# cassiusfive/balatro-gym

Hardware: AMD Instinct MI355X
Metric: env-steps/sec at 65536 envs, random policy; achieved HBM GB/s vs peak (higher is better)
Workload: dtype int64/f64

## Files before the change

### balatro_gym_amd/csrc/bg_device.h

```cpp
#pragma once
#include <hip/hip_runtime.h>
#include <stdint.h>
#include "bg_tables.h"

#define BG_NHOT 8
#define BG_NDECK 4
#define BG_NCOLD 7
#define BG_NTMPL 2
#define BG_MT_N 624
#define BG_MT_M 397
#define BG_MTS 640
#define BG_BLOCK 64

#define BG_DEVERR_GSTREAM 1u
#define BG_DEVERR_SHOPBLK 2u
#define BG_DEVERR_DECKRING 4u
#define BG_DEVERR_SHOPRING 8u

typedef __attribute__((address_space(1))) unsigned long long g_u64;
typedef __attribute__((address_space(1))) uint32_t g_u32;
__device__ __forceinline__ unsigned long long bg_ld8a(const void* p) { return __hip_atomic_load((g_u64*)p, __ATOMIC_RELAXED, __HIP_MEMORY_SCOPE_AGENT); }
__device__ __forceinline__ uint32_t bg_ld4a(const void* p) { return __hip_atomic_load((g_u32*)p, __ATOMIC_RELAXED, __HIP_MEMORY_SCOPE_AGENT); }
__device__ __forceinline__ void bg_st8a(void* p, unsigned long long v) { __hip_atomic_store((g_u64*)p, v, __ATOMIC_RELAXED, __HIP_MEMORY_SCOPE_AGENT); }
__device__ __forceinline__ uint4 bg_ld16a(const void* p) {
  const unsigned long long a = bg_ld8a(p), b = bg_ld8a((const char*)p + 8);
  return make_uint4((uint32_t)a, (uint32_t)(a >> 32), (uint32_t)b, (uint32_t)(b >> 32));
}

struct BgDev {
  int N;
  uint32_t flags;
  int max_ante;
  int KG, KS, KD;
  uint4* hot;
  uint4* deck;
  uint4* cold;
  uint4* tmpl;
  uint4* ndeck;
  uint32_t* gblk;
  uint32_t* sblk;
  uint32_t* sovf;
  uint32_t* deckmt;
  uint32_t* shopgenmt;
  uint32_t* err;
  uint32_t* wl_count;
  uint32_t* wl;
  uint32_t* wl_shop;
  uint32_t* sseed;
  uint32_t* smeta;
  const uint32_t* prod_view;
  const uint32_t* prod_in;
  uint32_t* prod_out;
  unsigned long long* dbg;
  uint4* cstate;
  uint4* ctmpl;
  uint32_t* cardmt;
  uint32_t* sealmt;
  const uint32_t* jtab;
};

struct Env {
  int64_t chips_scored, round_chips;
  int64_t best_hand;
  int32_t chips_needed, money;
  int32_t hp_total, hp_ante, jokers_sold, shop_reroll_state, shop_reroll_base;
  int32_t ante, round, phase, hands_left, discards_left, hand_size, nhand, nsel, njokers, ncons, n_magic, n_minim,
      boss_type, boss_req, bflags, shop_n;
  uint64_t hand, sel;
  uint32_t highlighted, face_down, boss_hp, boss_types, cons0, cons1;
  uint64_t jokers;
  int32_t shop_ante, d_head, d_cons, d_ready;
  uint64_t boss_cards;
  uint64_t levels;
  int32_t g_cur, g_cons, g_valid;
  int32_t g_idx, s_idx, s_cur, s_cons, s_ready;
  int32_t ndrop, nfo;
  uint64_t excess;
  int32_t max_ante;
};

#define BG_BF_FIRST_HAND 1
#define BG_BF_SHOP_EXISTS 2

__device__ __forceinline__ uint32_t bg_b(uint32_t w, int i) { return (w >> (8 * i)) & 0xffu; }

__device__ __forceinline__ void bg_unpack(const uint4 c[BG_NHOT], Env& e) {
  e.chips_scored = (int64_t)(((uint64_t)c[0].y << 32) | c[0].x);
  e.round_chips = (int64_t)(((uint64_t)c[0].w << 32) | c[0].z);
  e.best_hand = (int64_t)(((uint64_t)c[1].y << 32) | c[1].x);
  e.chips_needed = (int32_t)c[1].z;
  e.money = (int32_t)c[1].w;
  e.hp_total = (int32_t)c[2].x;
  e.hp_ante = (int32_t)(c[2].y & 0xffffu);
  e.jokers_sold = (int32_t)(c[2].y >> 16);
  e.shop_reroll_state = (int32_t)c[2].z;
  e.shop_reroll_base = (int32_t)c[2].w;
  e.ante = bg_b(c[3].x, 0); e.round = bg_b(c[3].x, 1); e.phase = bg_b(c[3].x, 2); e.hands_left = bg_b(c[3].x, 3);
  e.discards_left = bg_b(c[3].y, 0); e.hand_size = (int)(int8_t)bg_b(c[3].y, 1);  e.nhand = bg_b(c[3].y, 2); e.nsel = bg_b(c[3].y, 3);
  e.njokers = bg_b(c[3].z, 0); e.ncons = bg_b(c[3].z, 1); e.n_magic = bg_b(c[3].z, 2); e.n_minim = bg_b(c[3].z, 3);
  e.boss_type = bg_b(c[3].w, 0); e.boss_req = bg_b(c[3].w, 1); e.bflags = bg_b(c[3].w, 2); e.shop_n = bg_b(c[3].w, 3);
  e.hand = ((uint64_t)c[4].y << 32) | c[4].x;
  e.sel = ((uint64_t)c[4].w << 32) | c[4].z;
  e.highlighted = c[5].x & 0xffffu; e.face_down = bg_b(c[5].x, 2); e.boss_hp = bg_b(c[5].x, 3);
  e.boss_types = c[5].y & 0xffffu; e.cons0 = bg_b(c[5].y, 2); e.cons1 = bg_b(c[5].y, 3);
  e.jokers = (uint64_t)c[5].z | ((uint64_t)(c[5].w & 0xffu) << 32);
  e.shop_ante = bg_b(c[5].w, 1); e.d_head = bg_b(c[5].w, 2); e.d_cons = bg_b(c[5].w, 3); e.d_ready = 0;
  e.boss_cards = ((uint64_t)c[6].y << 32) | c[6].x;
  e.levels = (uint64_t)c[6].z | ((uint64_t)(c[6].w & 0xffffu) << 32);
  e.g_cur = bg_b(c[6].w, 2); e.g_cons = bg_b(c[6].w, 3); e.g_valid = 0;
  e.g_idx = (int32_t)(c[7].x & 0xffffu); e.s_idx = (int32_t)(c[7].x >> 16);
  e.s_cur = bg_b(c[7].y, 0); e.s_cons = bg_b(c[7].y, 1); e.s_ready = 0; e.ndrop = bg_b(c[7].y, 2); e.nfo = bg_b(c[7].y, 3);
  e.excess = (uint64_t)c[7].z | ((uint64_t)(c[7].w & 0xffffu) << 32);
  e.max_ante = (int32_t)(c[7].w >> 16) & 0xff;
}

__device__ __forceinline__ uint32_t bg_p4(int a, int b, int c, int d) {
  return (uint32_t)(a & 0xff) | ((uint32_t)(b & 0xff) << 8) | ((uint32_t)(c & 0xff) << 16) | ((uint32_t)(d & 0xff) << 24);
}

__device__ __forceinline__ void bg_pack(const Env& e, uint4 c[BG_NHOT]) {
  c[0] = make_uint4((uint32_t)e.chips_scored, (uint32_t)((uint64_t)e.chips_scored >> 32), (uint32_t)e.round_chips,
                    (uint32_t)((uint64_t)e.round_chips >> 32));
  c[1] = make_uint4((uint32_t)e.best_hand, (uint32_t)((uint64_t)e.best_hand >> 32), (uint32_t)e.chips_needed, (uint32_t)e.money);
  c[2] = make_uint4((uint32_t)e.hp_total, ((uint32_t)e.hp_ante & 0xffffu) | ((uint32_t)e.jokers_sold << 16),
                    (uint32_t)e.shop_reroll_state, (uint32_t)e.shop_reroll_base);
  c[3] = make_uint4(bg_p4(e.ante, e.round, e.phase, e.hands_left), bg_p4(e.discards_left, e.hand_size, e.nhand, e.nsel),
                    bg_p4(e.njokers, e.ncons, e.n_magic, e.n_minim), bg_p4(e.boss_type, e.boss_req, e.bflags, e.shop_n));
  c[4] = make_uint4((uint32_t)e.hand, (uint32_t)(e.hand >> 32), (uint32_t)e.sel, (uint32_t)(e.sel >> 32));
  c[5] = make_uint4((e.highlighted & 0xffffu) | ((e.face_down & 0xffu) << 16) | ((e.boss_hp & 0xffu) << 24),
                    (e.boss_types & 0xffffu) | ((e.cons0 & 0xffu) << 16) | ((e.cons1 & 0xffu) << 24), (uint32_t)e.jokers,
                    bg_p4((int)(e.jokers >> 32), e.shop_ante, e.d_head, e.d_cons));
  c[6] = make_uint4((uint32_t)e.boss_cards, (uint32_t)(e.boss_cards >> 32), (uint32_t)e.levels,
                    ((uint32_t)(e.levels >> 32) & 0xffffu) | ((uint32_t)(e.g_cur & 0xff) << 16) | ((uint32_t)(e.g_cons & 0xff) << 24));
  c[7] = make_uint4(((uint32_t)e.g_idx & 0xffffu) | ((uint32_t)e.s_idx << 16), bg_p4(e.s_cur, e.s_cons, e.ndrop, e.nfo),
                    (uint32_t)e.excess, ((uint32_t)(e.excess >> 32) & 0xffffu) | ((uint32_t)(e.max_ante & 0xff) << 16));
}

__device__ __forceinline__ void bg_derive_ready(Env& e, uint32_t prod) {
  e.d_ready = (int)((prod - (uint32_t)e.d_cons) & 0xffu);
  e.s_ready = (int)(((prod >> 8) - (uint32_t)e.s_cons) & 0xffu);
  e.g_valid = (int)(((prod >> 16) - (uint32_t)e.g_cons) & 0xffu);
}
__device__ __forceinline__ void bg_load_env(const BgDev& d, int env, Env& e) {
  uint4 c[BG_NHOT];
#pragma unroll
  for (int k = 0; k < BG_NHOT; k++) c[k] = d.hot[(size_t)k * d.N + env];
  bg_unpack(c, e);
  bg_derive_ready(e, d.prod_view ? d.prod_view[env] : 0u);
}
__device__ __forceinline__ void bg_store_env(const BgDev& d, int env, const Env& e) {
  uint4 c[BG_NHOT];
  bg_pack(e, c);
#pragma unroll
  for (int k = 0; k < BG_NHOT; k++) d.hot[(size_t)k * d.N + env] = c[k];
}

__device__ __forceinline__ int bg_get8(uint64_t v, int i) { return (int)((v >> (8 * i)) & 0xffull); }
__device__ __forceinline__ uint64_t bg_set8(uint64_t v, int i, int x) {
  return (v & ~(0xffull << (8 * i))) | ((uint64_t)(x & 0xff) << (8 * i));
}
__device__ __forceinline__ uint64_t bg_del8(uint64_t v, int i) {
  uint64_t lowmask = i ? ((1ull << (8 * i)) - 1) : 0ull;
  uint64_t lo = v & lowmask;
  uint64_t hi = (i < 7) ? (v >> (8 * (i + 1))) << (8 * i) : 0ull;
  return lo | hi;
}
__device__ __forceinline__ int bg_level(const Env& e, int ht) { return (int)((e.levels >> (4 * ht)) & 0xf); }

__device__ __forceinline__ uint32_t* bg_gblock(const BgDev& d, int env, int slot) { return d.gblk + ((size_t)env * d.KG + slot) * BG_MTS; }
#define BG_SW_T 56
#define BG_SW_PK 56
#define BG_SW_SEED 62
#define BG_SLOT_WORDS 64
#define BG_S_FASTMAX (BG_SW_T - 1)
static_assert(BG_SW_T >= 28 && BG_SW_PK == BG_SW_T && BG_SW_PK % 4 == 0 && BG_SW_PK + 6 == BG_SW_SEED && BG_SW_SEED + 2 == BG_SLOT_WORDS, "shop slot");
#define BG_BF_SHOP_OVF 4
__device__ __forceinline__ uint32_t* bg_sblock(const BgDev& d, int env, int slot) { return d.sblk + ((size_t)env * d.KS + slot) * BG_SLOT_WORDS; }
__device__ __forceinline__ uint32_t* bg_sovf(const BgDev& d, int env) { return d.sovf + (size_t)env * BG_MTS; }
__device__ __forceinline__ void bg_mt_seed_rolled(uint32_t* p, uint32_t key) {
  uint32_t g = 19650218u, a = g;
#pragma unroll 1
  for (uint32_t i = 1; i < 624u; i++) {
    g = 1812433253u * (g ^ (g >> 30)) + i;
    a = (g ^ ((a ^ (a >> 30)) * 1664525u)) + key;
    p[i] = a;
  }
  __builtin_amdgcn_fence(__ATOMIC_RELEASE, "agent");
  __builtin_amdgcn_fence(__ATOMIC_ACQUIRE, "agent");
  const uint32_t m1 = (p[1] ^ ((a ^ (a >> 30)) * 1664525u)) + key;
  uint32_t b = m1;
#pragma unroll 1
  for (uint32_t i = 2; i < 624u; i++) {
    b = (p[i] ^ ((b ^ (b >> 30)) * 1566083941u)) - i;
    p[i] = b;
  }
  p[1] = (m1 ^ ((b ^ (b >> 30)) * 1566083941u)) - 1u;
  p[0] = 0x80000000u;
}
__device__ __forceinline__ uint32_t* bg_deckmt(const BgDev& d, int env) { return d.deckmt + (size_t)env * BG_MTS; }
__device__ __forceinline__ uint32_t* bg_shopgenmt(const BgDev& d, int env) { return d.shopgenmt + (size_t)env * BG_MTS; }

#ifdef BG_TIMING
__shared__ unsigned long long bg_probe_lds[32];
#define BG_PROBE_BEGIN() unsigned long long _pt = __builtin_readcyclecounter()
#define BG_PROBE(k) do { unsigned long long _n = __builtin_readcyclecounter(); \
    if ((int)threadIdx.x == __ffsll((long long)__ballot(1)) - 1 + (int)(threadIdx.x & ~63u)) atomicAdd(&bg_probe_lds[k], _n - _pt); \
    _pt = __builtin_readcyclecounter(); } while (0)
#define BG_PROBE_INIT() do { if (threadIdx.x < 32) bg_probe_lds[threadIdx.x] = 0; __syncthreads(); } while (0)
#define BG_PROBE_FLUSH(d) do { __syncthreads(); if (threadIdx.x < 32 && (d).dbg && bg_probe_lds[threadIdx.x]) atomicAdd(&(d).dbg[threadIdx.x], bg_probe_lds[threadIdx.x]); } while (0)
#else
#define BG_PROBE_BEGIN() do {} while (0)
#define BG_PROBE(k) do {} while (0)
#define BG_PROBE_INIT() do {} while (0)
#define BG_PROBE_FLUSH(d) do {} while (0)
#endif

#define BG_RB 128
typedef __attribute__((address_space(3))) uint8_t lds_u8;
typedef __attribute__((address_space(3))) uint32_t lds_u32;
struct Deck0 { uint64_t lo, hi; static constexpr bool kCards = false; };
struct DeckLds { lds_u32* col; static constexpr bool kCards = false; };
struct Deck0C : Deck0 { static constexpr bool kCards = true; };
struct DeckLdsC : DeckLds { static constexpr bool kCards = true; };
#define BG_NCST 7
__device__ __forceinline__ uint32_t bg_cstate(const BgDev& d, int env, int ci) {
  return (uint32_t)((const uint16_t*)&d.cstate[(size_t)(ci >> 3) * d.N + env])[ci & 7];
}
__device__ __forceinline__ Deck0 bg_load_deck0(const BgDev& d, int env) {
  uint4 c = d.deck[env];
  Deck0 r;
  r.lo = ((uint64_t)c.y << 32) | c.x;
  r.hi = ((uint64_t)c.w << 32) | c.z;
  return r;
}
__device__ __forceinline__ void bg_deck_set(Deck0& dk, int k, uint4 c) {
  if (k == 0) { dk.lo = ((uint64_t)c.y << 32) | c.x; dk.hi = ((uint64_t)c.w << 32) | c.z; }
}
__device__ __forceinline__ void bg_deck_set(DeckLds& dk, int k, uint4 c) {
  dk.col[(4 * k) * BG_RB] = c.x; dk.col[(4 * k + 1) * BG_RB] = c.y; dk.col[(4 * k + 2) * BG_RB] = c.z; dk.col[(4 * k + 3) * BG_RB] = c.w;
}
__device__ __forceinline__ int bg_card(const BgDev& d, int env, const Deck0& k, int idx) {
  if (idx < 16) return (int)(((idx < 8 ? k.lo : k.hi) >> (8 * (idx & 7))) & 0xffull);
  const uint32_t* p = (const uint32_t*)&d.deck[(size_t)(idx >> 4) * d.N + env];
  return (int)((bg_ld4a(p + ((idx & 15) >> 2)) >> (8 * (idx & 3))) & 0xffu);
}
template <int S, bool C> struct DeckLdsS { lds_u32* col; static constexpr bool kCards = C; };
template <int S, bool C>
__device__ __forceinline__ void bg_deck_set(DeckLdsS<S, C>& dk, int k, uint4 c) {
  dk.col[(4 * k) * S] = c.x; dk.col[(4 * k + 1) * S] = c.y; dk.col[(4 * k + 2) * S] = c.z; dk.col[(4 * k + 3) * S] = c.w;
}
template <int S, bool C>
__device__ __forceinline__ int bg_card(const BgDev& d, int env, const DeckLdsS<S, C>& k, int idx) {
  return (int)((const lds_u8*)k.col)[(idx >> 2) * (S * 4) + (idx & 3)];
}
__device__ __forceinline__ int bg_card(const BgDev& d, int env, const DeckLds& k, int idx) {
  return (int)((const lds_u8*)k.col)[(idx >> 2) * (BG_RB * 4) + (idx & 3)];
}

struct DeckHead { uint64_t lo, hi; };
__device__ __forceinline__ DeckHead bg_deck_head(const BgDev& d, int env, const Deck0& k) { return DeckHead{k.lo, k.hi}; }
template <int S, bool C>
__device__ __forceinline__ DeckHead bg_deck_head(const BgDev& d, int env, const DeckLdsS<S, C>& k) {
  const uint32_t a = k.col[0], b = k.col[S], c = k.col[2 * S], e = k.col[3 * S];
  return DeckHead{((uint64_t)b << 32) | a, ((uint64_t)e << 32) | c};
}
template <class DK>
__device__ __forceinline__ int bg_card_h(const BgDev& d, int env, const DK& k, const DeckHead& h, int idx) {
  if (idx < 16) return (int)(((idx < 8 ? h.lo : h.hi) >> (8 * (idx & 7))) & 0xffull);
  return bg_card(d, env, k, idx);
}

__device__ __forceinline__ uint32_t bg_temper(uint32_t y) {
  y ^= (y >> 11);
  y ^= (y << 7) & 0x9d2c5680u;
  y ^= (y << 15) & 0xefc60000u;
  y ^= (y >> 18);
  return y;
}
__device__ __forceinline__ uint32_t bg_twist(uint32_t a, uint32_t b, uint32_t far) {
  uint32_t y = (a & 0x80000000u) | (b & 0x7fffffffu);
  return far ^ (y >> 1) ^ ((y & 1u) ? 0x9908b0dfu : 0u);
}

__device__ __forceinline__ uint32_t bg_lazy_next(uint32_t* S) {
  uint32_t c = S[BG_MT_N] & 0x3ffu;
  const uint32_t c1 = c + 1 == BG_MT_N ? 0u : c + 1, cf = c + BG_MT_M >= BG_MT_N ? c + BG_MT_M - BG_MT_N : c + BG_MT_M;
  const uint32_t y = bg_twist(S[c], S[c1], S[cf]);
  S[c] = y;
  S[BG_MT_N] = c1 | 0x80000000u;
  return bg_temper(y);
}
__device__ __forceinline__ double bg_lazy_random(uint32_t* S) {
  const uint32_t a = bg_lazy_next(S) >> 5, b = bg_lazy_next(S) >> 6;
  return ((double)a * 67108864.0 + (double)b) * (1.0 / 9007199254740992.0);
}

#define BG_WIN 16
struct JTables {
  uint64_t jd[152];
  uint32_t jm[152];
  uint64_t jr[152];
  uint8_t jf[152];
  uint8_t cost[152];
  double pow115[101];
  double pow15[16];
  double pow08[16];
  uint32_t inv[64];
};
typedef __attribute__((address_space(3))) const JTables lds_JTables;
struct RngWin {
  lds_JTables* jt;
  lds_u32* lds;
  int g_blk, g_start, g_len;
  int s_start, s_len;
  bool defer_adv;
  bool need_inv;
};
__device__ __forceinline__ void bg_win_init(RngWin& w, uint32_t* lds_lane, const JTables* jt = nullptr) {
  w.jt = (lds_JTables*)jt; w.lds = (lds_u32*)lds_lane; w.g_blk = -1; w.g_start = 0; w.g_len = 0; w.s_start = 0; w.s_len = 0; w.defer_adv = false; w.need_inv = false;
}
__device__ __noinline__ void bg_win_fill(lds_u32* lds, const uint32_t* src, int len) {
#pragma unroll 1
  for (int base = 0; base < len; base += BG_WIN) {
    uint32_t v[BG_WIN];
#pragma unroll
    for (int j = 0; j < BG_WIN; j++) v[j] = (base + j < len) ? src[base + j] : 0u;
// ... 257 lines not shown
```

### balatro_gym_amd/csrc/bg_engine.h

```cpp
#pragma once

#define BG_Q_RUN 0
#define BG_Q_PLAY 1
#define BG_Q_OTHER 2
#define BG_ITEM_VALID 0x80000000u
#define BG_SPIN_LIMIT (1u << 24)
#define BG_DEVERR_SPIN 16u
#define BG_ENG_LNE 8
static_assert(BG_ENG_LNE == 8, "only 256 envs per workgroup are supported: items carry the env lane in 8 bits, copy-queue generations in 7, and the epilogue assumes NE = 256");
#define BG_ENG_NE (1 << BG_ENG_LNE)
#define BG_ENG_NW 7
#define BG_ENG_OCC 2
#define BG_ENG_IMG_PIECES 22
#define BG_ENG_NSV 4
#define BG_ENG_SMASK_DEFAULT (((1u << BG_ENG_NSV) - 1u) << (BG_ENG_NW - BG_ENG_NSV))

struct EngineArgs {
  int T;
  int policy;
  uint64_t policy_seed, env_index0, t0;
  ObsPtrs obs;
  int obs_stride_steps;
  double* reward; uint8_t* term; uint8_t* trunc; int32_t* actions_out;
  const int32_t* actions_in;
// ... 9 lines not shown
  uint32_t epw;
  uint8_t* const* gpeer;
  uint32_t gworld, grank;
};

__device__ __forceinline__ uint32_t bg_lds_ld(uint32_t* p) {
  uint32_t v = __hip_atomic_load(p, __ATOMIC_RELAXED, __HIP_MEMORY_SCOPE_WORKGROUP);
  asm volatile("" ::: "memory");
  return v;
}
__device__ __forceinline__ void bg_lds_st(uint32_t* p, uint32_t v) {
  asm volatile("" ::: "memory");
  __hip_atomic_store(p, v, __ATOMIC_RELAXED, __HIP_MEMORY_SCOPE_WORKGROUP);
}
__device__ __forceinline__ uint32_t bg_lds_ld(uint16_t* p) {
  uint16_t v = __hip_atomic_load(p, __ATOMIC_RELAXED, __HIP_MEMORY_SCOPE_WORKGROUP);
  asm volatile("" ::: "memory");
  return (uint32_t)v;
}
__device__ __forceinline__ void bg_lds_st(uint16_t* p, uint32_t v) {
  asm volatile("" ::: "memory");
  __hip_atomic_store(p, (uint16_t)v, __ATOMIC_RELAXED, __HIP_MEMORY_SCOPE_WORKGROUP);
}
__device__ __forceinline__ void bg_vm_drain() { asm volatile("s_waitcnt vmcnt(0)" ::: "memory"); }
#ifdef BG_ENG_TL
constexpr bool kEngTl = true;
#else
constexpr bool kEngTl = false;
#endif
#define BG_TL(k) do { if constexpr (kEngTl) __hip_atomic_fetch_add(&s_tl[k], wall_clock64() - tl_k0, __ATOMIC_RELAXED, __HIP_MEMORY_SCOPE_WORKGROUP); } while (0)


template <bool HASH, bool CARDS, bool INFO>
__global__ __launch_bounds__(BG_ENG_NW * BG_BLOCK, BG_ENG_OCC) void bg_engine_kernel(BgDev d, EngineArgs a) {
  constexpr int NE = BG_ENG_NE, NW = BG_ENG_NW, NSV = BG_ENG_NSV;
  __shared__ bg_u32x4 s_img[NE][BG_ENG_IMG_PIECES];
  __shared__ uint4 s_c34[2][NE];
  __shared__ uint32_t s_deck[16][NE];
  __shared__ unsigned long long s_mask[NE];
  __shared__ uint32_t s_t[NE], s_prod[NE];
  __shared__ uint32_t s_q[3][NE];
  __shared__ __attribute__((aligned(16))) uint32_t s_ctl[8];
  uint32_t* const s_tail = &s_ctl[0];
  uint32_t* const s_head = &s_ctl[4];
#define s_done s_ctl[3]
#define s_busy s_ctl[7]
  __shared__ uint32_t s_win[NSV][BG_WIN][BG_BLOCK];
  __shared__ uint2 s_cq[NE];
  __shared__ uint32_t s_cqt;
  __shared__ bg_u32x4 s_zero;
  __shared__ unsigned long long s_stats[6];
  __shared__ JTables jt;
  __shared__ unsigned long long s_tl[kEngTl ? 32 : 1];
  const unsigned long long tl_k0 = kEngTl ? wall_clock64() : 0ull;
  if constexpr (kEngTl) { if (threadIdx.x < 32) s_tl[threadIdx.x] = 0ull; __syncthreads(); }
  __builtin_amdgcn_s_setprio(3);
  BG_PROBE_INIT();
  const int tid = threadIdx.x, wave = tid >> 6, lane = tid & 63;
  const int env0 = blockIdx.x * NE;
  const int n_live = d.N - env0 < NE ? d.N - env0 : NE;
  const bool can_serve = ((a.serve_mask >> wave) & 1u) != 0;
  const int serve_idx = __popc(a.serve_mask & ((1u << wave) - 1u));
  using DeckT = DeckLdsS<NE, CARDS>;
  const size_t N = (size_t)d.N;
  const bool keys_at_end = !a.obs.rows && a.obs_stride_steps == 0;
  if (tid < 3) { s_tail[tid] = 0u; s_head[tid] = 0; }
  if (tid == 0) { s_done = 0; s_busy = 0; s_cqt = 0; s_zero = bg_u32x4{0u, 0u, 0u, 0u}; }
  if (tid < 6) s_stats[tid] = 0ull;
  const bool mine = tid < NE && tid < n_live;
  const int l0 = tid, envp = env0 + tid;
  if (tid < NE) { s_q[BG_Q_RUN][l0] = 0; s_q[BG_Q_PLAY][l0] = 0; s_q[BG_Q_OTHER][l0] = 0; s_cq[l0] = make_uint2(0u, 0u); s_t[l0] = 0; }
  constexpr int JW = (int)(sizeof(JTables) / 4), JPT = (JW + NW * BG_BLOCK - 1) / (NW * BG_BLOCK);
  uint32_t jv[JPT];
#pragma unroll
  for (int k = 0; k < JPT; k++) { const int i = tid + k * NW * BG_BLOCK; jv[k] = i < JW ? d.jtab[i] : 0u; }
  bool svc = false;
  {
    uint4 c[BG_NHOT];
    uint4 dw[BG_NDECK];
    uint32_t prod = 0u;
    int act0 = 0;
    if (mine) {
#pragma unroll
      for (int k = 0; k < BG_NHOT; k++) c[k] = d.hot[(size_t)k * N + envp];
#pragma unroll
      for (int k = 0; k < BG_NDECK; k++) dw[k] = d.deck[(size_t)k * N + envp];
      prod = d.prod_view ? d.prod_view[envp] : 0u;
      if (a.actions_in) act0 = a.actions_in[envp];
    }
    __syncthreads();
    if (tid == 0) BG_TL(1);
#pragma unroll
    for (int k = 0; k < JPT; k++) { const int i = tid + k * NW * BG_BLOCK; if (i < JW) ((uint32_t*)&jt)[i] = jv[k]; }
    if (mine) {
      s_c34[0][l0] = c[3]; s_c34[1][l0] = c[4];
      DeckT dk; dk.col = (lds_u32*)&s_deck[0][l0];
#pragma unroll
      for (int k = 0; k < BG_NDECK; k++) bg_deck_set(dk, k, dw[k]);
      s_prod[l0] = prod;
      Env pe;
      ShopRegs psr; psr.valid = false;
      bg_unpack(c, pe);
      bg_derive_ready(pe, prod);
      const uint64_t pmask = bg_action_mask(d, envp, pe, psr);
      s_mask[l0] = pmask;
      if (a.actions_in) {
        const bool valid = act0 >= 0 && act0 < 60 && ((pmask >> (act0 & 63)) & 1ull);
        const bool terminal = pe.ante > 100 || pe.chips_scored > 1000000000ll;
        const bool cheap = !terminal && (!valid || (pe.phase == 0 && act0 >= 2 && act0 < 10) || (pe.phase == 1 && act0 == 31 && pe.hand_size <= pe.nhand));
        svc = !cheap;
        if (svc) {
          const int q = (!terminal && pe.phase == 0 && act0 == 0) ? BG_Q_PLAY : BG_Q_OTHER;
          const uint32_t slot = __hip_atomic_fetch_add(&s_tail[q], 1u, __ATOMIC_RELAXED, __HIP_MEMORY_SCOPE_WORKGROUP);
          bg_lds_st(&s_q[q][slot & (NE - 1)], (uint32_t)l0 | (((slot >> BG_ENG_LNE) & 0xffu) << 8) | (((uint32_t)act0 & 0x7fffu) << 16) | BG_ITEM_VALID);
        }
      }
    }
  }
  if (tid == 0) BG_TL(2);
  __syncthreads();
  if (tid == 0) BG_TL(3);
  {
    if (mine && !svc) {
      __builtin_amdgcn_s_setprio(1);
      uint4 c[BG_NHOT];
#pragma unroll
      for (int k = 0; k < BG_NHOT; k++) if (k != 3 && k != 4) c[k] = d.hot[(size_t)k * N + envp];
      c[3] = s_c34[0][l0]; c[4] = s_c34[1][l0];
      Env pe;
      ShopRegs psr; psr.valid = false;
      bg_unpack(c, pe);
      bg_derive_ready(pe, s_prod[l0]);
      const uint64_t pmask = s_mask[l0];
      DeckT dk; dk.col = (lds_u32*)&s_deck[0][l0];
      const ObsPtrs none{};
      bg_write_obs_impl<false, 3>(d, envp, 0, pe, dk, none, pmask, psr, RowExtra{0.0, 0, 0u}, RowStage{(lds_u4*)&s_img[l0][0], nullptr});
      const uint32_t slot = __hip_atomic_fetch_add(&s_tail[BG_Q_RUN], 1u, __ATOMIC_RELAXED, __HIP_MEMORY_SCOPE_WORKGROUP);
      bg_lds_st(&s_q[BG_Q_RUN][slot & (NE - 1)], (uint32_t)l0 | (((slot >> BG_ENG_LNE) & 0xffu) << 8) | BG_ITEM_VALID);
    }
  }
  if (tid == 0) BG_TL(4);
  if (wave >= (int)(a.n_waves + a.copier)) return;
  if (a.copier && wave >= (int)a.n_waves) {
    __builtin_amdgcn_s_setprio(2);
    const uint32_t cid = (uint32_t)wave - a.n_waves, two = a.copier > 1u ? 1u : 0u;
    uint32_t head = two ? 32u * cid : 0u, cpolls = 0;
    const bool whole = a.obs.row_stride == 384u;
    const uint32_t PR = 22u, rcp = 2979u;
    for (;;) {
      const uint32_t tail = __builtin_amdgcn_readfirstlane(bg_lds_ld(&s_cqt));
      uint32_t navail = (int32_t)(tail - head) > 0 ? tail - head : 0u;
      if (two) { const uint32_t left = 32u - (head & 31u); navail = navail > left ? left : navail; }
      if (navail == 0u) {
        if (__builtin_amdgcn_readfirstlane(bg_lds_ld(&s_done)) >= (uint32_t)n_live) break;
        __builtin_amdgcn_s_sleep(2);
        if (++cpolls > BG_SPIN_LIMIT) { if (lane == 0) atomicOr(d.err, BG_DEVERR_SPIN); break; }
        continue;
      }
      cpolls = 0;
      const uint32_t nb = navail > BG_BLOCK ? BG_BLOCK : navail;
      uint2 ent = make_uint2(0u, 0u);
      if ((uint32_t)lane < nb) {
        const uint32_t pos = head + (uint32_t)lane, want = BG_ITEM_VALID | (((pos >> BG_ENG_LNE) & 0x7fu) << 16);
        lds_u32* ep = (lds_u32*)&s_cq[pos & (NE - 1)];
        uint32_t spin = 0, y = ep[1];
        while ((y & (BG_ITEM_VALID | 0x7f0000u)) != want && ++spin < BG_SPIN_LIMIT) { __builtin_amdgcn_s_sleep(1); asm volatile("" ::: "memory"); y = ep[1]; }
        asm volatile("" ::: "memory");
        if ((y & (BG_ITEM_VALID | 0x7f0000u)) != want) atomicOr(d.err, BG_DEVERR_SPIN);
        else ent = make_uint2(ep[0], y);
      }
      BG_WAVE_SYNC();
      typedef __attribute__((address_space(3))) const char lds_cc;
      typedef uint32_t bg_u32x2 __attribute__((ext_vector_type(2)));
      if (whole) {
        uint32_t rsel[3], mul[3], ib[3], gl[3];
        lds_cc* const imgb = (lds_cc*)&s_img[0][0];
        lds_cc* const cqb = (lds_cc*)&s_cq[0];
#pragma unroll
        for (int j = 0; j < 3; j++) {
          const uint32_t pidx = (uint32_t)j * BG_BLOCK + (uint32_t)lane, rs = (pidx * 2731u) >> 16, c = pidx - 24u * rs;
          rsel[j] = rs; gl[j] = 16u * c;
          mul[j] = c < 22u ? 16u * BG_ENG_IMG_PIECES : 0u;
          ib[j] = c < 22u ? 16u * c : (uint32_t)((lds_cc*)&s_zero - imgb);
        }
        for (uint32_t g0 = 0; g0 < nb; g0 += 32u) {
          bg_u32x2 ce[4][3];
          bg_u32x4 v[4][3];
#pragma unroll
          for (int u = 0; u < 4; u++)
#pragma unroll
            for (int j = 0; j < 3; j++)
              ce[u][j] = *(__attribute__((address_space(3))) const bg_u32x2*)(cqb + (((head + g0 + 8u * (uint32_t)u + rsel[j]) & (NE - 1)) << 3));
#pragma unroll
          for (int u = 0; u < 4; u++)
#pragma unroll
            for (int j = 0; j < 3; j++)
              v[u][j] = *(__attribute__((address_space(3))) const bg_u32x4*)(imgb + __umul24(ce[u][j].y & 0xffu, mul[j]) + ib[j]);
#pragma unroll
          for (int u = 0; u < 4; u++)
#pragma unroll
            for (int j = 0; j < 3; j++)
              if (g0 + 8u * (uint32_t)u + rsel[j] < nb)
                __builtin_nontemporal_store(v[u][j], (__attribute__((address_space(1))) bg_u32x4*)(a.obs.rows + ((size_t)ce[u][j].x * 384u + gl[j])));
        }
      } else {
      const uint32_t total = PR * nb;
#define BG_COPIER_KU 12
      constexpr int KU = BG_COPIER_KU;
      for (uint32_t q0 = (uint32_t)lane; q0 < total; q0 += (uint32_t)KU * BG_BLOCK) {
        uint2 ce[KU];
// ... 135 lines not shown
          const uint32_t play = te.nsel > 0 ? 1u : 0u, disc = (te.nsel > 0 && discards_left > 0u) ? 1u : 0u;
          mask = (mask & ~3ull) | play | ((uint64_t)disc << 1);
          s_mask[l] = mask;
          *(__attribute__((address_space(3))) uint16_t*)&img8[BG_ROW_ACTION_MASK] = (uint16_t)(play | (disc << 8));
        }
        fin = true;
      } else if (!terminal && valid && phase == 1u && action == 31 && (int)(int8_t)bg_b(c3.y, 1) <= (int)bg_b(c3.y, 2)) {
        const uint32_t nhand = bg_b(c3.y, 2), ncons = bg_b(c3.z, 1);
        ((lds_u8*)&s_c34[0][l])[2] = 0;
        uint64_t m = (((1ull << (nhand < 8u ? nhand : 8u)) - 1ull) << 2) | (((1ull << ncons) - 1ull) << 10);
        if (nsel0 > 0u) m |= 1ull | (discards_left > 0u ? 2ull : 0ull);
        mask = m;
        s_mask[l] = mask;
#pragma unroll
        for (int wq = 0; wq < 15; wq++) img32[44 + wq] = __umul24((uint32_t)(mask >> (4 * wq)) & 0xfu, 0x204081u) & 0x01010101u;
#pragma unroll
        for (int wq = 64; wq < 74; wq++) img32[wq] = 0u;
        img8[BG_ROW_PHASE] = 0;
        fin = true;
      } else if (!terminal && !valid) { reward = -1.0; fin = true; }
      else {
        const int q = (!terminal && phase == 0u && action == 0) ? BG_Q_PLAY : BG_Q_OTHER;
        const uint32_t slot = __hip_atomic_fetch_add(&s_tail[q], 1u, __ATOMIC_RELAXED, __HIP_MEMORY_SCOPE_WORKGROUP);
        bg_lds_st(&s_q[q][slot & (NE - 1)], (uint32_t)l | (((slot >> BG_ENG_LNE) & 0xffu) << 8) | (((uint32_t)action & 0x7fffu) << 16) | BG_ITEM_VALID);
        active = false;
      }
      if (fin) {
        *(__attribute__((address_space(3))) double*)&img32[34] = reward;
        img32[43] = (uint32_t)action;
        img8[BG_ROW_TERMINATED] = 0;
        if constexpr (INFO) { bg_step_init(o); o.reward = reward; o.error = valid ? 0 : 1; }
      }
      return fin;
    };
    auto finish = [&](bool cheap, size_t row, int action, double reward, bool terminated, const StepOut& o) __attribute__((always_inline)) {
      if (!a.obs.rows && !keys_at_end) bg_emit_keys_from_image((const lds_u4*)&s_img[l][0], a.obs, row);
      if (a.reward) a.reward[row] = reward;
      if (a.term) a.term[row] = terminated ? 1 : 0;
      if (a.actions_out) a.actions_out[row] = action;
      if constexpr (INFO) bg_emit_info(row, o, a.trunc, a.info);
      if (HASH) ohash ^= bg_hash_image((const lds_u4*)&s_img[l][0]) * (0x9E3779B97F4A7C15ull + 2 * (uint64_t)(a.t0 + t)) + (a.env_index0 + (uint64_t)env);
      n_steps++;
      rbits ^= (uint64_t)__double_as_longlong(reward) * (2 * (uint64_t)(a.t0 + t) + 1);
      t++;
      s_t[l] = t;
    };
    auto copy_out = [&](bool fin, size_t row) __attribute__((always_inline)) {
    if (a.copier) {
      const unsigned long long fm = __ballot(fin);
      if (fm) {
        uint32_t base = 0;
        if (lane == (int)(__ffsll((long long)fm) - 1)) base = __hip_atomic_fetch_add(&s_cqt, (uint32_t)__popcll(fm), __ATOMIC_RELAXED, __HIP_MEMORY_SCOPE_WORKGROUP);
        base = __builtin_amdgcn_readlane(base, __ffsll((long long)fm) - 1);
        if (fin) {
          const uint32_t pos = base + __builtin_amdgcn_mbcnt_hi((uint32_t)(fm >> 32), __builtin_amdgcn_mbcnt_lo((uint32_t)fm, 0u));
          lds_u32* ep = (lds_u32*)&s_cq[pos & (NE - 1)];
          ep[0] = (uint32_t)row;
          asm volatile("" ::: "memory");
          ep[1] = (uint32_t)l | (t >= (uint32_t)a.T ? 0x100u : 0u) | (((pos >> BG_ENG_LNE) & 0x7fu) << 16) | BG_ITEM_VALID;
          asm volatile("" ::: "memory");
          active = false;
        }
      }
      return;
    }
      if (active && t >= (uint32_t)a.T) { __hip_atomic_fetch_add(&s_done, 1u, __ATOMIC_RELAXED, __HIP_MEMORY_SCOPE_WORKGROUP); active = false; }
    };
    {
      bool fin = false;
      size_t row = 0;
      if (active) {
        row = (size_t)env + (a.obs_stride_steps ? (size_t)t * N : 0);
        int action = 0;
        double reward = 0.0;
        bool terminated = false;
        StepOut o;
        if (cls == BG_Q_RUN) fin = cheap_step(action, reward, o);
        else {
          uint64_t mask = s_mask[l];
        action = a.actions_in ? a.actions_in[(size_t)t * N + env] : (int)((item >> 16) & 0x7fffu);
        BG_PROBE_BEGIN();
        uint4 c[BG_NHOT];
#pragma unroll
        for (int k = 0; k < BG_NHOT; k++) if (k != 3 && k != 4) c[k] = d.hot[(size_t)k * N + env];
        c[3] = s_c34[0][l]; c[4] = s_c34[1][l];
        Env e;
        bg_unpack(c, e);
        BG_PROBE(23);
        bg_derive_ready(e, s_prod[l]);
        DeckT dk; dk.col = (lds_u32*)&s_deck[0][l];
        ShopRegs sr; sr.valid = false;
        RngWin w;
        bg_win_init(w, &s_win[serve_idx][0][lane], &jt);
        bg_step_init(o);
        if constexpr (INFO) if (a.info.score_breakdown) o.bd_dst = a.info.score_breakdown + row * 8;
        if (bg_step_guards(e, mask, action, o)) bg_env_dispatch(d, env, e, w, sr, dk, action, o);
        BG_PROBE(cls == BG_Q_PLAY ? 20 : 21);
        if (e.max_ante > 0 && e.ante > e.max_ante) { o.terminated = true; o.flags |= 256; }
        if (o.terminated) n_eps++;
        if (o.terminated && a.autoreset) { bg_env_reset(d, env, e, dk); if (INFO) o.flags |= BG_INFO_AUTORESET; }
        if constexpr (CARDS) bg_vm_drain();
        BG_PROBE(24);
        mask = bg_action_mask(d, env, e, sr);
        BG_PROBE(25);
        {
          const ObsPtrs none{};
          bg_write_obs_impl<false, 3>(d, env, row, e, dk, none, mask, sr, RowExtra{o.reward, action, o.terminated ? 1u : 0u}, RowStage{(lds_u4*)&s_img[l][0], nullptr});
        }
        BG_PROBE(26);
        bg_pack(e, c);
#pragma unroll
        for (int k = 0; k < BG_NHOT; k++) if (k != 3 && k != 4) d.hot[(size_t)k * N + env] = c[k];
        s_c34[0][l] = c[3]; s_c34[1][l] = c[4];
        s_mask[l] = mask;
        BG_PROBE(27);
        reward = o.reward; terminated = o.terminated;
        if (o.hand_type >= 0) { n_plays++; ssum += o.final_score; }
        fin = true;
        }
        if (fin) finish(cls == BG_Q_RUN, row, action, reward, terminated, o);
      }
      copy_out(fin, row);
    }
    for (uint32_t sub = 0; cls == BG_Q_RUN && !a.copier && sub < a.th_more && __ballot(active) != 0ull; sub++) {
      bool fin = false;
      size_t row = 0;
      if (active) {
        row = (size_t)env + (a.obs_stride_steps ? (size_t)t * N : 0);
        int action = 0;
        double reward = 0.0;
        StepOut o;
        fin = cheap_step(action, reward, o);
        if (fin) finish(true, row, action, reward, false, o);
      }
      copy_out(fin, row);
    }
    if (active) {
      const uint32_t slot = __hip_atomic_fetch_add(&s_tail[BG_Q_RUN], 1u, __ATOMIC_RELAXED, __HIP_MEMORY_SCOPE_WORKGROUP);
      bg_lds_st(&s_q[BG_Q_RUN][slot & (NE - 1)], (uint32_t)l | (((slot >> BG_ENG_LNE) & 0xffu) << 8) | BG_ITEM_VALID);
    }
    if (lane == 0) __hip_atomic_fetch_sub(&s_busy, 1u, __ATOMIC_RELAXED, __HIP_MEMORY_SCOPE_WORKGROUP);
    if constexpr (kEngTl) if (lane == 0) {
      const int b = cls == BG_Q_RUN ? 5 : (cls == BG_Q_PLAY ? 16 : 20);
      __hip_atomic_fetch_add(&s_tl[b], tl_b0 - tl_k0, __ATOMIC_RELAXED, __HIP_MEMORY_SCOPE_WORKGROUP);
      __hip_atomic_fetch_add(&s_tl[b + 1], 1ull, __ATOMIC_RELAXED, __HIP_MEMORY_SCOPE_WORKGROUP);
      __hip_atomic_fetch_add(&s_tl[b + 2], wall_clock64() - tl_b0, __ATOMIC_RELAXED, __HIP_MEMORY_SCOPE_WORKGROUP);
      __hip_atomic_fetch_add(&s_tl[b + 3], (unsigned long long)nb, __ATOMIC_RELAXED, __HIP_MEMORY_SCOPE_WORKGROUP);
    }
  }
  if (lane == 0 && wave == 0) BG_TL(9);
  if (lane == 0 && wave == (int)a.n_waves - 1) BG_TL(10);
  BG_PROBE_FLUSH(d);
  __syncthreads();
  if (tid == 0) BG_TL(12);
  if (tid < n_live) {
    d.hot[(size_t)3 * N + env0 + tid] = s_c34[0][tid];
    d.hot[(size_t)4 * N + env0 + tid] = s_c34[1][tid];
    if (keys_at_end) bg_emit_keys_from_image((const lds_u4*)&s_img[tid][0], a.obs, (size_t)(env0 + tid));
  }
  if (a.stats) {
    bg_stats_wave(s_stats, n_steps, n_eps, n_plays, ssum, rbits, ohash);
    __syncthreads();
    bg_stats_flush(a.stats, s_stats, tid);
  }
  if constexpr (kEngTl) if (d.dbg) {
    if (tid == 0) { BG_TL(13); s_tl[0] = 1ull; }
    __syncthreads();
    if (tid < 32 && tid != 14 && tid != 15 && s_tl[tid]) atomicAdd(&d.dbg[tid], s_tl[tid]);
    if (tid == 14) atomicMax(&d.dbg[14], ~tl_k0);
    if (tid == 15) atomicMax(&d.dbg[15], wall_clock64());
  }
}
```

### balatro_gym_amd/csrc/bg_engine3.h

```cpp
#pragma once

#ifdef BG_E3_TIMING
#define E3T_DECL() unsigned long long e3t_[8] = {0,0,0,0,0,0,0,0}, e3t0_ = __builtin_readcyclecounter()
#define E3T(k) do { const unsigned long long n_ = __builtin_readcyclecounter(); e3t_[k] += n_ - e3t0_; e3t0_ = n_; } while (0)
#define E3T_CNT(k, v) do { e3t_[k] += (v); } while (0)
#define E3T_FLUSH(base) do { if (lane == 0 && d.dbg) for (int k_ = 0; k_ < 8; k_++) atomicAdd(&d.dbg[(base) + k_], e3t_[k_]); } while (0)
constexpr bool kE3Timing = true, kE3Tl = true;
#else
#define E3T_DECL() const unsigned long long e3t_[8] = {0,0,0,0,0,0,0,0}; (void)e3t_
#define E3T(k) do {} while (0)
#define E3T_CNT(k, v) do {} while (0)
#define E3T_FLUSH(base) do {} while (0)
constexpr bool kE3Timing = false;
#ifdef BG_E3_TL
constexpr bool kE3Tl = true;
#else
constexpr bool kE3Tl = false;
#endif
#endif

#define BG_E3_REC_STORE(v, p) __builtin_nontemporal_store(v, p)
#define BG_E3_SPARSE 8u
#define BG_E3_SPARSE2 16u
#define BG_E3_ACTB 8
template <int NOW, int KS, int NSV>
struct E3Lds {
  static constexpr int NE = NOW * KS * BG_BLOCK;
  bg_u32x4 s_img[NE][22];
  uint4 s_c34[2][NE];
  unsigned long long s_mask[NE];
  uint32_t s_prod[NE];
  uint16_t s_ans[NE];
  uint32_t s_q[2][NE];
  __attribute__((aligned(16))) uint32_t s_ctl[8];
  uint32_t s_win[NSV][BG_WIN][BG_BLOCK];
  uint2 s_list[NOW][KS * BG_BLOCK];
  uint4 s_nd[BG_NDECK][NE];
  uint32_t s_ndst[NE];
  bg_u32x4 s_zero;
  unsigned long long s_stats[6];
  uint32_t s_owners_left;
  JTables jt;
};
template <bool HASH, bool CARDS, int NOW, int KS, int NSV, bool ACT = false>
__global__ __launch_bounds__((NOW + NSV) * BG_BLOCK, 2) void bg_engine3_kernel(BgDev d, EngineArgs a) {
  constexpr int NE = NOW * KS * BG_BLOCK, LNE = NE == 256 ? 8 : (NE == 128 ? 7 : 6);
  static_assert(NE == 64 || NE == 128 || NE == 256, "envs per workgroup (a request carries the env's lane in 8 bits)");
  __shared__ E3Lds<NOW, KS, NSV> L;
  auto& s_img = L.s_img; auto& s_c34 = L.s_c34; auto& s_mask = L.s_mask; auto& s_prod = L.s_prod; auto& s_ans = L.s_ans; auto& s_q = L.s_q;
  auto& s_ctl = L.s_ctl; auto& s_win = L.s_win; auto& s_list = L.s_list; auto& s_zero = L.s_zero; auto& s_owners_left = L.s_owners_left; auto& jt = L.jt;
  auto& s_nd = L.s_nd; auto& s_ndst = L.s_ndst;
  __shared__ int s_actb[ACT ? BG_E3_ACTB : 1][ACT ? NE : 1];
  __builtin_amdgcn_s_setprio(2);
  const unsigned long long e3_k0 = kE3Tl ? wall_clock64() : 0ull;
  BG_PROBE_INIT();
  bg_tables_load(&jt, d.jtab);
  const int tid = threadIdx.x, lane = tid & 63;
  const int wave = tid >> 6;
  const int epw = (NE == 64 && a.epw >= 1u && a.epw < 64u) ? (int)a.epw : NE;
  const int env0 = blockIdx.x * epw;
  const int n_live = d.N - env0 < epw ? d.N - env0 : epw;
  using DeckT = typename std::conditional<CARDS, Deck0C, Deck0>::type;
  const size_t N = (size_t)d.N;
  typedef __attribute__((address_space(3))) const char lds_cc;
  if (tid < 8) s_ctl[tid] = 0;
  if (tid == 0) { s_zero = bg_u32x4{0u, 0u, 0u, 0u}; s_owners_left = NOW; }
  if (tid < 6) L.s_stats[tid] = 0ull;
  for (int l = tid; l < NE; l += (NOW + NSV) * BG_BLOCK) {
    const int env = env0 + l;
    s_q[0][l] = 0; s_q[1][l] = 0; s_ans[l] = 0; s_ndst[l] = 0;
    if (l < n_live) {
      uint4 c[BG_NHOT];
#pragma unroll
      for (int k = 0; k < BG_NHOT; k++) c[k] = d.hot[(size_t)k * N + env];
      s_c34[0][l] = c[3]; s_c34[1][l] = c[4];
      DeckT dk; static_cast<Deck0&>(dk) = bg_load_deck0(d, env);
      const uint32_t prod = d.prod_view ? d.prod_view[env] : 0u;
      s_prod[l] = prod;
      Env e;
      bg_unpack(c, e);
      bg_derive_ready(e, prod);
      s_ndst[l] = e.d_ready > 0 ? 1u : 0u;
      if (e.d_ready > 0) {
#pragma unroll
        for (int k = 0; k < BG_NDECK; k++) s_nd[k][l] = d.ndeck[((size_t)e.d_head * BG_NDECK + k) * N + env];
      }
      ShopRegs sr; sr.valid = false;
      const uint64_t mask = bg_action_mask(d, env, e, sr);
      s_mask[l] = mask;
      const ObsPtrs none{};
      bg_write_obs_impl<false, 3>(d, env, 0, e, dk, none, mask, sr, RowExtra{0.0, 0, 0u}, RowStage{(lds_u4*)&s_img[l][0], nullptr});
    }
  }
  __syncthreads();
  if constexpr (kE3Timing) if (lane == 0) { uint32_t hw; asm volatile("s_getreg_b32 %0, hwreg(HW_REG_HW_ID)" : "=s"(hw)); atomicOr(&s_ctl[2], ((hw >> 4) & 3u) << (2 * wave)); }
  const unsigned long long e3_w0 = kE3Tl ? wall_clock64() : 0ull;
  if constexpr (kE3Tl) {
    if (tid == 0 && d.dbg) atomicAdd(&d.dbg[28], e3_w0 - e3_k0);
    __syncthreads();
  }
  const uint32_t T = (uint32_t)a.T;
  if (wave < NOW) {
    const uint32_t bmod3 = (uint32_t)(a.env_index0 % 3ull);
    lds_cc* const imgb = (lds_cc*)&s_img[0][0];
    const bool whole = a.obs.row_stride == 384u;
    uint32_t rsel[3], cmul[3], cib[3], cgl[3];
#pragma unroll
    for (int j = 0; j < 3; j++) {
      const uint32_t pidx = (uint32_t)j * BG_BLOCK + (uint32_t)lane, rs = (pidx * 2731u) >> 16, c = pidx - 24u * rs;
      rsel[j] = rs; cgl[j] = 16u * c;
      cmul[j] = c < 22u ? 16u * 22u : 0u;
      cib[j] = c < 22u ? 16u * c : (uint32_t)((lds_cc*)&s_zero - imgb);
    }
    uint32_t t[KS], nreq[KS];
    bool waiting[KS], terminal[KS];
    uint4 rc3[KS], rc4[KS];
    uint64_t rmask[KS];
    uint64_t px[KS];
    size_t prow[KS];
    int pblind[KS];
    uint32_t abase[KS];
    uint32_t athr[KS];
#pragma unroll
    for (int s = 0; s < KS; s++) {
      t[s] = 0; nreq[s] = 0; waiting[s] = false;
      const int l = (wave * KS + s) * BG_BLOCK + lane;
      if constexpr (ACT) {
        abase[s] = 0; athr[s] = 100u;
        prow[s] = (size_t)(env0 + l);
        if (l < n_live) {
          const uint32_t cap = (d.hot[(size_t)7 * N + (size_t)(env0 + l)].w >> 16) & 0xffu;
          if (cap > 0u && cap < 100u) athr[s] = cap;
        }
      } else {
        const int env = env0 + l;
        const uint64_t gi0 = a.env_index0 + (uint64_t)env;
        px[s] = a.policy_seed + 0x9E3779B97F4A7C15ull * (gi0 + 1) + BG_POLICY_PSI * (a.t0 + 1);
        prow[s] = (size_t)env;
        pblind[s] = a.policy == 2 ? 45 + (int)((bmod3 + (uint32_t)env % 3u) % 3u) : 45;
      }
      rc3[s] = s_c34[0][l]; rc4[s] = s_c34[1][l]; rmask[s] = s_mask[l];
      const lds_u32* im = (const lds_u32*)&s_img[l][0];
      terminal[s] = bg_b(rc3[s].x, 0) > (ACT ? athr[s] : 100u) || (int64_t)(((uint64_t)im[33] << 32) | im[32]) > 1000000000ll;
    }
    uint64_t n_steps = 0, rbits = 0, ohash = 0;
    uint32_t idle = 0, aiter = 0;
    E3T_DECL();
    for (;;) {
      bg_u32x4 ndv[KS][BG_NDECK];
      bool ndp[KS];
#pragma unroll
      for (int s = 0; s < KS; s++) ndp[s] = false;
      bool busy = false;
#pragma unroll
      for (int s = 0; s < KS; s++) busy = busy || ((wave * KS + s) * BG_BLOCK + lane < n_live && (t[s] < T || waiting[s]));
      if (__ballot(busy) == 0ull) break;
      E3T_CNT(4, 1);
      if constexpr (ACT) {
        if ((aiter++ & (BG_E3_ACTB - 1u)) == 0u) {
#pragma unroll
          for (int s = 0; s < KS; s++) {
            const int l = (wave * KS + s) * BG_BLOCK + lane;
            const uint32_t nt = t[s] + (waiting[s] ? 1u : 0u);
            abase[s] = nt;
            int av[BG_E3_ACTB];
#pragma unroll
            for (int j = 0; j < BG_E3_ACTB; j++) {
              av[j] = 0;
              if (l < n_live && nt + (uint32_t)j < T) av[j] = a.actions_in[(size_t)(nt + (uint32_t)j) * N + (size_t)(env0 + l)];
            }
#pragma unroll
            for (int j = 0; j < BG_E3_ACTB; j++) s_actb[j][l] = av[j];
          }
        }
      }
      uint32_t nb = 0;
      bool glast = false;
#pragma unroll
      for (int s = 0; s < KS; s++) {
        const int l = (wave * KS + s) * BG_BLOCK + lane, env = env0 + l;
        const bool live = l < n_live;
        lds_u32* const img32 = (lds_u32*)&s_img[l][0];
        lds_u8* const img8 = (lds_u8*)&s_img[l][0];
        const size_t row = prow[s];
        bool fin = false;
        if (waiting[s] && bg_lds_ld(&s_ans[l]) == (nreq[s] & 0xffffu)) {
          waiting[s] = false; fin = true;
          const uint32_t nds = bg_lds_ld(&s_ndst[l]);
          if ((nds & 0xffu) == 2u) {
#pragma unroll
            for (int k = 0; k < BG_NDECK; k++) ndv[s][k] = *(const __attribute__((address_space(1))) bg_u32x4*)&d.ndeck[((size_t)(nds >> 8) * BG_NDECK + k) * N + env];
            bg_lds_st(&s_ndst[l], 0u);
            ndp[s] = true;
          }
          rc3[s] = s_c34[0][l]; rc4[s] = s_c34[1][l]; rmask[s] = s_mask[l];
          terminal[s] = bg_b(rc3[s].x, 0) > (ACT ? athr[s] : 100u) || (int64_t)(((uint64_t)img32[33] << 32) | img32[32]) > 1000000000ll;
        }
        else if (live && !waiting[s] && t[s] < T) {
          uint64_t mask = rmask[s];
          const uint4 c3 = rc3[s];
          const uint32_t phase = bg_b(c3.x, 2), discards_left = bg_b(c3.y, 0), nsel0 = bg_b(c3.y, 3);
          int action;
          if constexpr (ACT) action = s_actb[(t[s] - abase[s]) & (BG_E3_ACTB - 1u)][l];
          else {
            Env pe; pe.phase = (int)phase;
            PolicyLane pl; pl.seed_env = 0; pl.blind = pblind[s];
            action = bg_policy_action_fast(pe, mask, a.policy, pl, px[s], (lds_JTables*)&jt);
          }
          double reward = 0.0;
          const bool valid = action >= 0 && action < 60 && ((mask >> (action & 63)) & 1ull);
          const bool term = terminal[s];
          if (!term && valid && phase == 0u && action >= 2 && action < 10) {
            const int pos = action - 2;
            Env te; te.sel = ((uint64_t)rc4[s].w << 32) | rc4[s].z; te.nsel = (int)nsel0;
            bg_toggle_select(te, pos);
            rc4[s].z = (uint32_t)te.sel; rc4[s].w = (uint32_t)(te.sel >> 32);
            rc3[s].y = (rc3[s].y & 0x00ffffffu) | ((uint32_t)te.nsel << 24);
            *(lds_u64*)&img32[2 * pos] = te.nsel > (int)nsel0 ? 1ull : 0ull;
            if ((te.nsel > 0) != (nsel0 > 0u)) {
              const uint32_t play = te.nsel > 0 ? 1u : 0u, disc = (te.nsel > 0 && discards_left > 0u) ? 1u : 0u;
              mask = (mask & ~3ull) | play | ((uint64_t)disc << 1);
              rmask[s] = mask;
              *(__attribute__((address_space(3))) uint16_t*)&img8[BG_ROW_ACTION_MASK] = (uint16_t)(play | (disc << 8));
            }
            fin = true;
          } else if (!term && valid && phase == 1u && action == 31 && (int)(int8_t)bg_b(c3.y, 1) <= (int)bg_b(c3.y, 2)) {
            const uint32_t nhand = bg_b(c3.y, 2), ncons = bg_b(c3.z, 1);
            rc3[s].x &= 0xff00ffffu;
            uint64_t m = (((1ull << (nhand < 8u ? nhand : 8u)) - 1ull) << 2) | (((1ull << ncons) - 1ull) << 10);
            if (nsel0 > 0u) m |= 1ull | (discards_left > 0u ? 2ull : 0ull);
            mask = m;
            rmask[s] = mask;
#pragma unroll
            for (int wq = 0; wq < 15; wq++) img32[44 + wq] = __umul24((uint32_t)(mask >> (4 * wq)) & 0xfu, 0x204081u) & 0x01010101u;
#pragma unroll
            for (int wq = 64; wq < 74; wq++) img32[wq] = 0u;
            img8[BG_ROW_PHASE] = 0;
            fin = true;
          } else if (!term && !valid) { reward = -1.0; fin = true; }
          else {
            s_c34[0][l] = rc3[s]; s_c34[1][l] = rc4[s]; s_mask[l] = mask;
            if constexpr (ACT) img32[43] = (uint32_t)action;
            const int q = (!term && phase == 0u && action == 0) ? 0 : 1;
            const uint32_t slot = __hip_atomic_fetch_add(&s_ctl[q], 1u, __ATOMIC_RELAXED, __HIP_MEMORY_SCOPE_WORKGROUP);
            bg_lds_st(&s_q[q][slot & (NE - 1)], (uint32_t)l | (((slot >> LNE) & 0xffu) << 8) | (((uint32_t)action & 0x7fffu) << 16) | BG_ITEM_VALID);
            nreq[s]++;
            waiting[s] = true;
          }
          if (fin) {
            *(__attribute__((address_space(3))) double*)&img32[34] = reward;
            img32[43] = (uint32_t)action;
            img8[BG_ROW_TERMINATED] = 0;
          }
        }
        if (fin) {
          const uint64_t rb = ((uint64_t)img32[35] << 32) | img32[34];
          if (HASH) ohash ^= bg_hash_image((const lds_u4*)&s_img[l][0]) * (0x9E3779B97F4A7C15ull + 2 * (uint64_t)(a.t0 + t[s])) + (a.env_index0 + (uint64_t)env);
          n_steps++;
          rbits ^= rb * (2 * (uint64_t)(a.t0 + t[s]) + 1);
          t[s]++;
          if constexpr (!ACT) px[s] += BG_POLICY_PSI;
          if (a.obs_stride_steps) prow[s] += N;
        }
        const unsigned long long fms = __ballot(fin);
        const bool lastrec = fin && a.gworld != 0u && t[s] == T;
        if (fin) s_list[wave][nb + __builtin_amdgcn_mbcnt_hi((uint32_t)(fms >> 32), __builtin_amdgcn_mbcnt_lo((uint32_t)fms, 0u))] = make_uint2((uint32_t)row, (uint32_t)l | (lastrec ? 0x100u : 0u));
        nb += (uint32_t)__popcll(fms);
        glast = glast || lastrec;
      }
      E3T(0);
      if (nb) {
        idle = 0;
        BG_WAVE_SYNC();
        typedef uint32_t bg_u32x2 __attribute__((ext_vector_type(2)));
// ... 62 lines not shown
        }
        E3T(1); E3T_CNT(5, nb);
      } else {
        __builtin_amdgcn_s_sleep(2);
        if (++idle > BG_SPIN_LIMIT) { if (lane == 0) atomicOr(d.err, BG_DEVERR_SPIN); break; }
        E3T(2);
      }
    }
    E3T_FLUSH(0);
    if constexpr (kE3Timing) if (lane == 0 && d.dbg) {
      uint32_t hw; asm volatile("s_getreg_b32 %0, hwreg(HW_REG_HW_ID)" : "=s"(hw));
      const uint32_t my = (hw >> 4) & 3u;
      int same = 0;
      const uint32_t simds = bg_lds_ld(&s_ctl[2]);
      for (int k = 0; k < NOW + NSV; k++) same += (((simds >> (2 * k)) & 3u) == my) ? 1 : 0;
      const int key = same >= 3 ? 3 : same;
      atomicAdd(&d.dbg[16 + 4 * (key - 1) + 0], wall_clock64() - e3_w0);
      atomicAdd(&d.dbg[16 + 4 * (key - 1) + 1], e3t_[4]);
      atomicAdd(&d.dbg[16 + 4 * (key - 1) + 2], 1ull);
    }
    if constexpr (kE3Tl) if (lane == 0 && d.dbg) atomicAdd(&d.dbg[29], wall_clock64() - e3_k0);
#pragma unroll
    for (int s = 0; s < KS; s++) { const int l = (wave * KS + s) * BG_BLOCK + lane; s_c34[0][l] = rc3[s]; s_c34[1][l] = rc4[s]; }
    if (lane == 0) __hip_atomic_fetch_sub(&s_owners_left, 1u, __ATOMIC_RELAXED, __HIP_MEMORY_SCOPE_WORKGROUP);
    if (a.stats) bg_stats_wave(L.s_stats, n_steps, 0, 0, 0, rbits, ohash);
  } else {
    __builtin_amdgcn_s_setprio(3);
    const int sidx = wave - NOW;
    uint64_t n_eps = 0, n_plays = 0;
    int64_t ssum = 0;
    uint32_t polls = 0;
    bool seen = false;
    unsigned long long t_seen = 0;
    E3T_DECL();
    for (;;) {
      asm volatile("" ::: "memory");
      const bg_u32x4 ch = *(volatile __attribute__((address_space(3))) bg_u32x4*)&s_ctl[4];
      asm volatile("" ::: "memory");
      const bg_u32x4 ct = *(volatile __attribute__((address_space(3))) bg_u32x4*)&s_ctl[0];
      asm volatile("" ::: "memory");
      const uint32_t hp = __builtin_amdgcn_readfirstlane(ch.x), ho = __builtin_amdgcn_readfirstlane(ch.y);
      auto queued = [&](uint32_t tail, uint32_t head) -> uint32_t { const uint32_t k = tail - head; return k <= (uint32_t)NE ? k : 0u; };
      const uint32_t np = queued(__builtin_amdgcn_readfirstlane(ct.x), hp), no = queued(__builtin_amdgcn_readfirstlane(ct.y), ho);
      if ((np | no) == 0u) {
        if (__builtin_amdgcn_readfirstlane(bg_lds_ld(&s_owners_left)) == 0u) break;
        __builtin_amdgcn_s_sleep(2);
        if (++polls > BG_SPIN_LIMIT) { if (lane == 0) atomicOr(d.err, BG_DEVERR_SPIN); break; }
        continue;
      }
      int cls;
      if (np >= a.th_play) cls = 0;
      else if (no >= a.th_other) cls = 1;
      else {
        const unsigned long long now = wall_clock64();
        if (!seen) { seen = true; t_seen = now; }
        if (now - t_seen < (unsigned long long)a.th_more) { __builtin_amdgcn_s_sleep(1); continue; }
        cls = np >= no ? 0 : 1;
      }
      seen = false;
      const uint32_t head = cls ? ho : hp, navail = cls ? no : np;
      const uint32_t nb = navail > BG_BLOCK ? BG_BLOCK : navail;
      uint32_t item = 0;
      uint32_t* const slotp = &s_q[cls][(head + (uint32_t)lane) & (NE - 1)];
      {
        uint32_t got = 0;
        if ((uint32_t)lane < nb) item = bg_lds_ld(slotp);
        if (lane == 0) got = atomicCAS(&s_ctl[4 + cls], head, head + nb) == head ? 1u : 0u;
        if (__builtin_amdgcn_readfirstlane(got) == 0u) continue;
      }
      polls = 0;
      E3T(0);
      if ((uint32_t)lane < nb) {
        uint32_t spin = 0;
        const uint32_t want = BG_ITEM_VALID | ((((head + (uint32_t)lane) >> LNE) & 0xffu) << 8);
        while ((item & (BG_ITEM_VALID | 0xff00u)) != want && ++spin < BG_SPIN_LIMIT) { __builtin_amdgcn_s_sleep(1); item = bg_lds_ld(slotp); }
        if ((item & (BG_ITEM_VALID | 0xff00u)) != want) atomicOr(d.err, BG_DEVERR_SPIN);
        else {
          const int l = (int)(item & 0xffu), env = env0 + l;
          const int action = ACT ? (int)((const lds_u32*)&s_img[l][0])[43] : (int)((item >> 16) & 0x7fffu);
          uint64_t mask = s_mask[l];
          BG_PROBE_BEGIN();
          uint4 c[BG_NHOT];
#pragma unroll
          for (int k = 0; k < BG_NHOT; k++) if (k != 3 && k != 4) c[k] = d.hot[(size_t)k * N + env];
          c[3] = s_c34[0][l]; c[4] = s_c34[1][l];
          DeckT dk; static_cast<Deck0&>(dk) = bg_load_deck0(d, env);
          RngWin w;
          bg_win_init(w, &s_win[sidx][0][lane], &jt);
          Env e;
          bg_unpack(c, e);
          BG_PROBE(23);
          bg_derive_ready(e, s_prod[l]);
          ShopRegs sr; sr.valid = false;
          StepOut o;
          bg_step_init(o);
          o.bd_dst = nullptr;
          if (bg_step_guards(e, mask, action, o)) bg_env_dispatch(d, env, e, w, sr, dk, action, o);
          BG_PROBE(cls == 0 ? 20 : 21);
          if (e.max_ante > 0 && e.ante > e.max_ante) { o.terminated = true; o.flags |= 256; }
          if (o.terminated) n_eps++;
          if (o.terminated && a.autoreset) {
            const bool have = bg_lds_ld(&s_ndst[l]) == 1u;
            bg_env_reset(d, env, e, dk, nullptr, have ? (lds_cu4*)&s_nd[0][l] : (lds_cu4*)nullptr, NE);
            bg_lds_st(&s_ndst[l], e.d_ready > 0 ? (2u | ((uint32_t)e.d_head << 8)) : 0u);
          }
          if constexpr (CARDS) bg_vm_drain();
          BG_PROBE(24);
          mask = bg_action_mask(d, env, e, sr);
          BG_PROBE(25);
          const ObsPtrs none{};
          bg_write_obs_impl<false, 3>(d, env, 0, e, dk, none, mask, sr, RowExtra{o.reward, action, o.terminated ? 1u : 0u}, RowStage{(lds_u4*)&s_img[l][0], nullptr});
          BG_PROBE(26);
          bg_pack(e, c);
#pragma unroll
          for (int k = 0; k < BG_NHOT; k++) if (k != 3 && k != 4) d.hot[(size_t)k * N + env] = c[k];
          s_c34[0][l] = c[3]; s_c34[1][l] = c[4];
          s_mask[l] = mask;
          if (o.hand_type >= 0) { n_plays++; ssum += o.final_score; }
          bg_lds_st(&s_ans[l], bg_lds_ld(&s_ans[l]) + 1u);
          BG_PROBE(27);
        }
      }
      E3T(1 + cls); E3T_CNT(4 + cls, 1); E3T_CNT(6 + cls, nb);
    }
    E3T_FLUSH(8);
    if constexpr (kE3Tl) if (lane == 0 && d.dbg) atomicAdd(&d.dbg[30], wall_clock64() - e3_k0);
    if (a.stats) bg_stats_wave(L.s_stats, 0, n_eps, n_plays, ssum, 0, 0);
  }
  BG_PROBE_FLUSH(d);
  __syncthreads();
  for (int l = tid; l < n_live; l += (NOW + NSV) * BG_BLOCK) {
    d.hot[(size_t)3 * N + env0 + l] = s_c34[0][l];
    d.hot[(size_t)4 * N + env0 + l] = s_c34[1][l];
  }
  if (a.stats) bg_stats_flush(a.stats, L.s_stats, tid);
  if constexpr (kE3Tl) if (tid == 0 && d.dbg) atomicAdd(&d.dbg[31], wall_clock64() - e3_k0);
}
```

### balatro_gym_amd/csrc/bg_lib.hip

```cpp
#include "../../include/balatro_mi355x.h"
#include "bg_step.h"
#include <hip/hip_ext.h>
#include <stdio.h>
#include <stdlib.h>
#include <string.h>
#include <type_traits>
#include <string>
#include <vector>


struct InfoPtrs {
  int64_t* final_score; int32_t* error; int32_t* flags; int32_t* aux; int8_t* hand_type; int8_t* cards_played;
  double* reward_terms;
  double* score_breakdown;
};

static_assert(offsetof(ObsPtrs, rows) == sizeof(bg_obs_ptrs), "the first 31 members of ObsPtrs must mirror bg_obs_ptrs");
static_assert(sizeof(InfoPtrs) == sizeof(bg_info_ptrs), "InfoPtrs must mirror bg_info_ptrs");

__device__ __forceinline__ void bg_emit_info(size_t row, const StepOut& o, uint8_t* trunc, const InfoPtrs& info) {
  if (trunc) trunc[row] = 0;
  if (info.final_score) info.final_score[row] = o.final_score;
  if (info.error) info.error[row] = o.error;
  if (info.flags) info.flags[row] = o.flags;
// ... 246 lines not shown
      for (int g = 0; g < BG_MTB / 4 + 1; g++) { uint4 v = f4[g]; fr[4 * g] = v.x; fr[4 * g + 1] = v.y; fr[4 * g + 2] = v.z; fr[4 * g + 3] = v.w; }
    }
    uint32_t v[BG_MTB];
#pragma unroll
    for (int j = 0; j < BG_MTB; j++) {
      uint32_t nxt = (base + j == BG_MT_N - 1) ? first_new : nx[j + 1];
      v[j] = bg_twist(cur, nxt, fr[j + 1]);
      if (base + j == 0) first_new = v[j];
      cur = nxt;
    }
#pragma unroll
    for (int j = 0; j < BG_MTB / 4; j++) d4[base / 4 + j] = make_uint4(v[4 * j], v[4 * j + 1], v[4 * j + 2], v[4 * j + 3]);
  }
}

#include "bg_ops.h"
#include "bg_sim.h"
#include "bg_encode.h"
#include "bg_gae.h"
#include "bg_norm.h"
#include "bg_head.h"
#include "bg_ppo.h"

__global__ __launch_bounds__(BG_BLOCK) void bg_seed_kernel(BgDev d, const int64_t* __restrict__ seeds,
                                                          const uint8_t* __restrict__ mask_in, int reseed_global) {
  int env = blockIdx.x * BG_BLOCK + threadIdx.x;
  if (env >= d.N) return;
  if (mask_in && !mask_in[env]) return;
  RngWin w;
  bg_win_init(w, nullptr);
  Env e;
  bg_load_env(d, env, e);
  int64_t seed = seeds[env];
  if (reseed_global) {
    uint32_t gs = (uint32_t)((uint64_t)seed + 16000ull);
    uint32_t* g = bg_gblock(d, env, 0);
    bg_mt_seed(g, gs);
    bg_mt_twist(g, g);
    e.g_cur = 0; e.g_idx = 0; e.g_cons = 0; e.g_valid = 1;
  }
  if (seed == 0) {
    uint64_t r;
    int guard = 0;
    do {
      uint64_t lo = bg_gdraw(d, env, e, w);
      uint64_t hi = bg_gdraw(d, env, e, w) >> 31;
      r = lo | (hi << 32);
    } while (r >= 4294967296ull && ++guard < 4096);
    seed = (int64_t)(r & 0xffffffffull);
  }
  uint32_t base = (uint32_t)(uint64_t)seed;
  bg_mt_seed(bg_deckmt(d, env), base);
  bg_deckmt(d, env)[BG_MT_N] = BG_LAZY_SEEDED;
  bg_mt_seed(bg_shopgenmt(d, env), base + 2000u);
  bg_shopgenmt(d, env)[BG_MT_N] = BG_LAZY_SEEDED;
  if (d.cardmt) {
    bg_mt_seed(d.cardmt + (size_t)env * BG_MTS, base + 11000u);
    d.cardmt[(size_t)env * BG_MTS + BG_MT_N] = BG_LAZY_SEEDED;
    bg_mt_seed(d.sealmt + (size_t)env * BG_MTS, base + 13000u);
    d.sealmt[(size_t)env * BG_MTS + BG_MT_N] = BG_LAZY_SEEDED;
  }
  e.d_head = 0; e.d_cons = 0; e.d_ready = 0;
  e.s_cons = 0; e.s_ready = 0;
  d.smeta[env] = 0;
  {
    uint32_t gp = reseed_global ? 1u : (uint32_t)((e.g_cons + e.g_valid) & 0xff);
    uint32_t pv = 0u | (0u << 8) | (gp << 16) | 0x80000000u;
    d.prod_out[env] = pv;
    ((uint32_t*)d.prod_in)[env] = pv;
  }
  bg_store_env(d, env, e);
}

__global__ __launch_bounds__(BG_BLOCK) void bg_refill_zero_kernel(BgDev d) { if (threadIdx.x < BG_WL_COUNTERS) d.wl_count[threadIdx.x] = 0; }

struct BgPart { uint32_t p, q; };
__device__ __forceinline__ uint32_t bg_part_lo(uint32_t count, BgPart pt) { return (uint32_t)(((uint64_t)count * pt.p) / pt.q); }
__device__ __forceinline__ uint32_t bg_part_hi(uint32_t count, BgPart pt) { return (uint32_t)(((uint64_t)count * (pt.p + 1u)) / pt.q); }

__global__ __launch_bounds__(BG_BLOCK) void bg_refill_scan_kernel(BgDev d) {
  int env = blockIdx.x * BG_BLOCK + threadIdx.x;
  if (env >= d.N) return;
  size_t N = d.N;
  uint32_t w5 = ((const uint32_t*)&d.hot[(size_t)5 * N + env])[3];
  uint32_t w6 = ((const uint32_t*)&d.hot[(size_t)6 * N + env])[3];
  uint2 w7 = *((const uint2*)&d.hot[(size_t)7 * N + env]);
  uint32_t prod = d.prod_in[env];
  int d_cons = bg_b(w5, 3), g_cons = bg_b(w6, 3), s_cur = bg_b(w7.y, 0), s_cons = bg_b(w7.y, 1);
  int d_ready = (int)((prod - (uint32_t)d_cons) & 0xffu);
  int s_ready = (int)(((prod >> 8) - (uint32_t)s_cons) & 0xffu);
  int g_valid = (int)(((prod >> 16) - (uint32_t)g_cons) & 0xffu);
  const bool seeded = (prod >> 31) != 0;
  if (!seeded) { d.prod_out[env] = prod; return; }
  if (s_ready < d.KS - 1) {
    uint32_t sm = d.smeta[env];
    int head = (int)(sm & 0xffu), cnt = (int)((sm >> 8) & 0xffu);
    int emitted = d.KS - 1 - s_ready;
    if (emitted > cnt) emitted = cnt;
    if (emitted > 0) {
      const uint32_t base = atomicAdd(&d.wl_count[3], (uint32_t)emitted);
#pragma unroll 1
      for (int k = 0; k < emitted; k++) {
        int slot = s_cur + 1 + s_ready + k; while (slot >= d.KS) slot -= d.KS;
        d.wl_shop[2 * (size_t)(base + k)] = (uint32_t)env | ((uint32_t)slot << 24);
        d.wl_shop[2 * (size_t)(base + k) + 1] = d.sseed[(size_t)env * BG_SSEED + ((head + k) & (BG_SSEED - 1))];
      }
      head = (head + emitted) & (BG_SSEED - 1); cnt -= emitted;
    } else emitted = 0;
    if (emitted) {
      d.smeta[env] = (uint32_t)head | ((uint32_t)cnt << 8);
      prod = (prod & 0xffff00ffu) | ((((prod >> 8) + (uint32_t)emitted) & 0xffu) << 8);
    }
    if (cnt < BG_SSEED - 8) { uint32_t i = atomicAdd(&d.wl_count[1], 1u); d.wl[N + i] = (uint32_t)env; }
  }
  d.prod_out[env] = prod;
  if (d_ready < d.KD) { uint32_t i = atomicAdd(&d.wl_count[0], 1u); d.wl[i] = (uint32_t)env; }
  if (g_valid > 0 && g_valid < d.KG) { uint32_t i = atomicAdd(&d.wl_count[2], 1u); d.wl[2 * N + i] = (uint32_t)env; }
}

typedef uint32_t bg_cp_u32x4 __attribute__((ext_vector_type(4)));
__global__ __launch_bounds__(BG_BLOCK) __attribute__((amdgpu_waves_per_eu(4, 4))) void bg_refill_deck_kernel(BgDev d, BgPart pt, uint32_t cursor_idx, uint32_t max_made) {
  __builtin_amdgcn_s_setprio(BG_REFILL_WAVE_PRIO);
  __shared__ uint8_t sdeck[52][BG_BLOCK];
  const size_t N = d.N;
  const int tid = threadIdx.x;
  const uint32_t count0 = d.wl_count[0], lo = bg_part_lo(count0, pt), count = bg_part_hi(count0, pt);
  uint32_t* const cursor = &d.wl_count[cursor_idx];
  const int cap = max_made ? (int)max_made : 1 << 30;
  int env = 0, d_head = 0, d_ready = 0, made = 0;
  uint32_t prod = 0, cur = 0;
  uint32_t* mt = bg_deckmt(d, 0);
  bool have = false, need = false, dry = false;
#pragma unroll 1
  while (true) {
    if (!dry) {
      const unsigned long long freem = __ballot(!have);
      if (freem != 0ull) {
        const int leader = __ffsll(freem) - 1, nfree = __popcll(freem);
        uint32_t base = 0;
        if (tid == leader) base = atomicAdd(cursor, (uint32_t)nfree);
        base = lo + (uint32_t)__shfl((int)base, leader);
        dry = base + (uint32_t)nfree >= count;
        const uint32_t my = base + (uint32_t)__popcll(freem & ((1ull << tid) - 1ull));
        if (!have && my < count) {
          env = (int)d.wl[my];
          mt = bg_deckmt(d, env);
          const uint32_t w5 = ((const uint32_t*)&d.hot[(size_t)5 * N + env])[3];
          prod = d.prod_out[env];
          d_head = bg_b(w5, 2);
          d_ready = (int)((prod - (uint32_t)bg_b(w5, 3)) & 0xffu);
          cur = mt[BG_MT_N] & 0x3ffu;
          made = 0;
          need = d_ready < d.KD;
          have = need;
        }
      }
    }
    if (__ballot(need) == 0ull) { if (dry) break; continue; }
    if (need) { int p = 0; for (int s = 0; s < 4; s++) for (int r = 0; r < 13; r++) sdeck[p++][tid] = (uint8_t)(r * 4 + s); }
    int i = 51;
    cur = bg_lazy_stream(mt, cur, need, [&](uint32_t y) {
      const int k = 32 - __clz((uint32_t)(i + 1));
      const uint32_t j = bg_temper(y) >> (32 - k);
      if (j <= (uint32_t)i) {
        const uint8_t a = sdeck[i][tid], b = sdeck[j][tid];
        sdeck[i][tid] = b; sdeck[j][tid] = a;
        i--;
      }
      return i >= 1;
    });
    if (need) {
      const int slot = (d_head + d_ready) % d.KD;
#pragma unroll
      for (int k = 0; k < BG_NDECK; k++) {
        uint32_t wv[4] = {0, 0, 0, 0};
#pragma unroll
        for (int b = 0; b < 16; b++) { int i2 = k * 16 + b; if (i2 < 52) wv[b >> 2] |= (uint32_t)sdeck[i2][tid] << (8 * (b & 3)); }
        bg_cp_u32x4 nv; nv.x = wv[0]; nv.y = wv[1]; nv.z = wv[2]; nv.w = wv[3];
        __builtin_nontemporal_store(nv, (bg_cp_u32x4*)&d.ndeck[((size_t)slot * BG_NDECK + k) * N + env]);
      }
      d_ready++; made++;
      need = d_ready < d.KD && made < cap;
      if (!need) {
        mt[BG_MT_N] = cur | BG_LAZY_SEEDED;
        ((uint8_t*)&d.prod_out[env])[0] = (uint8_t)((prod + (uint32_t)made) & 0xffu);
        have = false;
      }
    }
  }
}

__global__ __launch_bounds__(BG_BLOCK) void bg_refill_seedring_kernel(BgDev d, BgPart pt) {
  __builtin_amdgcn_s_setprio(BG_REFILL_WAVE_PRIO);
  size_t N = d.N;
  const uint32_t count0 = d.wl_count[1], lo = bg_part_lo(count0, pt), count = bg_part_hi(count0, pt);
  for (uint32_t base = lo + blockIdx.x * BG_BLOCK; base < count; base += gridDim.x * BG_BLOCK) {
    const bool valid = base + threadIdx.x < count;
    const int env = valid ? (int)d.wl[N + base + threadIdx.x] : 0;
    uint32_t* mt = bg_shopgenmt(d, env);
    int head = 0, cnt = BG_SSEED;
    uint32_t cur = 0;
    if (valid) {
      const uint32_t sm = d.smeta[env];
      head = (int)(sm & 0xffu); cnt = (int)((sm >> 8) & 0xffu);
      cur = mt[BG_MT_N] & 0x3ffu;
    }
    const bool need = valid && cnt < BG_SSEED;
    cur = bg_lazy_stream<BG_LAZY_U_SEEDRING>(mt, cur, need, [&](uint32_t y) {
      const uint32_t r = bg_temper(y);
      if (r < 2147483648u) { d.sseed[(size_t)env * BG_SSEED + ((head + cnt) & (BG_SSEED - 1))] = r; cnt++; }
      return cnt < BG_SSEED;
    });
    if (need) {
      mt[BG_MT_N] = cur | BG_LAZY_SEEDED;
      d.smeta[env] = (uint32_t)head | ((uint32_t)cnt << 8);
    }
  }
}

__global__ __launch_bounds__(BG_BLOCK, 8) void bg_refill_shop_kernel(BgDev d, BgPart pt) {
  const uint32_t count0 = d.wl_count[3], lo = bg_part_lo(count0, pt), count = bg_part_hi(count0, pt);
  for (uint32_t item = lo + blockIdx.x * BG_BLOCK + threadIdx.x; item < count; item += gridDim.x * BG_BLOCK) {
    const uint2 it = ((const uint2*)d.wl_shop)[item];
    bg_mt_seed_slot(bg_sblock(d, (int)(it.x & 0xffffffu), (int)(it.x >> 24)), it.y);
  }
}
__global__ __launch_bounds__(BG_BLOCK) void bg_refill_gblk_kernel(BgDev d, BgPart pt) {
  __builtin_amdgcn_s_setprio(BG_REFILL_WAVE_PRIO);
  const size_t N = d.N;
  const uint32_t count0 = d.wl_count[2], lo = bg_part_lo(count0, pt), count = bg_part_hi(count0, pt);
  const int l = threadIdx.x;
  constexpr int NR = (BG_MT_N + 63) / 64;
  for (uint32_t item = lo + blockIdx.x; item < count; item += gridDim.x) {
    const int env = (int)d.wl[2 * N + item];
    const uint32_t w6 = ((const uint32_t*)&d.hot[(size_t)6 * N + env])[3];
    const uint32_t prod = d.prod_out[env];
    const int g_cur = bg_b(w6, 2), g_cons = bg_b(w6, 3);
    int g_valid = (int)(((prod >> 16) - (uint32_t)g_cons) & 0xffu);
    if (g_valid <= 0 || g_valid >= d.KG) continue;
    int last = (g_cur + g_valid - 1) % d.KG, made = 0;
    uint32_t o[NR + 1];
    {
      const uint32_t* src = bg_gblock(d, env, last);
#pragma unroll
      for (int r = 0; r < NR; r++) o[r] = (64 * r + l < BG_MT_N) ? __builtin_nontemporal_load(&src[64 * r + l]) : 0u;
      o[NR] = 0u;
    }
#pragma unroll 1
    while (g_valid < d.KG) {
      const int nxt = last + 1 == d.KG ? 0 : last + 1;
      uint32_t* dst = bg_gblock(d, env, nxt);
      uint32_t n[NR];
#pragma unroll
      for (int r = 0; r < NR; r++) {
        const int k = 64 * r + l;
        const uint32_t up_same = __shfl(o[r], (l + 1) & 63), up_next = __shfl(o[r + 1], 0);
        uint32_t up = l == 63 ? up_next : up_same;
        if (r == NR - 1) { const uint32_t new0 = __shfl(n[0], 0); if (k == BG_MT_N - 1) up = new0; }
        uint32_t far = 0u;
        if (64 * r < BG_MT_N - BG_MT_M) {
          const uint32_t a = r + 6 < NR ? __shfl(o[r + 6], (l + 13) & 63) : 0u, b2 = r + 7 < NR ? __shfl(o[r + 7], (l + 13) & 63) : 0u;
          far = l + 13 < 64 ? a : b2;
        }
        if (64 * r + 63 >= BG_MT_N - BG_MT_M) {
          const uint32_t a = r >= 4 ? __shfl(n[r >= 4 ? r - 4 : 0], (l + 29) & 63) : 0u, b2 = r >= 3 ? __shfl(n[r >= 3 ? r - 3 : 0], (l + 29) & 63) : 0u;
          const uint32_t fn = l + 29 < 64 ? a : b2;
          if (k >= BG_MT_N - BG_MT_M) far = fn;
        }
        n[r] = bg_twist(o[r], up, far);
        if (k < BG_MT_N) __builtin_nontemporal_store(n[r], &dst[k]);
      }
      if (l < 16) bg_gblock(d, env, last)[BG_MT_N + l] = n[0];
#pragma unroll
      for (int r = 0; r < NR; r++) o[r] = n[r];
      last = nxt; g_valid++; made++;
    }
    if (made && l == 0) {
      const uint32_t g = ((prod >> 16) + (uint32_t)made) & 0xffu;
      ((uint8_t*)&d.prod_out[env])[2] = (uint8_t)g;
    }
  }
}

__global__ __launch_bounds__(BG_BLOCK) void bg_inject_kernel(BgDev d, const uint8_t* __restrict__ mask_in) {
  int env = blockIdx.x * BG_BLOCK + threadIdx.x;
  if (env >= d.N) return;
  if (mask_in && !mask_in[env]) return;
  Env e;
  bg_load_env(d, env, e);
  uint4 t0 = d.tmpl[env], t1 = d.tmpl[(size_t)d.N + env];
  if (t0.y & 0x80000000u) { e.njokers = (int)bg_b(t0.y, 1); e.jokers = (uint64_t)t0.x | ((uint64_t)(t0.y & 0xffu) << 32); }
  if (t0.y & 0x40000000u) e.money = (int32_t)t0.z;
  if (t0.y & 0x20000000u) e.ante = (int)bg_b(t0.y, 2);
  if (t0.y & 0x10000000u) { e.levels = (uint64_t)t1.x | ((uint64_t)(t1.y & 0xffffu) << 32); e.excess = 0; }
  if (t1.z & 0x80000000u) { e.ncons = (int)bg_b(t1.z, 0); e.cons0 = bg_b(t1.z, 1); e.cons1 = bg_b(t1.z, 2); }
  bg_store_env(d, env, e);
}

__global__ __launch_bounds__(256) void bg_tables_build_kernel(uint32_t* out) {
  __shared__ JTables jt;
  { uint32_t* w = (uint32_t*)&jt; for (int i = threadIdx.x; i < (int)(sizeof(JTables) / 4); i += blockDim.x) w[i] = 0u; }
  __syncthreads();
  bg_tables_init(&jt);
  const uint32_t* w = (const uint32_t*)&jt;
  for (int i = threadIdx.x; i < (int)(sizeof(JTables) / 4); i += blockDim.x) out[i] = w[i];
}

__global__ __launch_bounds__(BG_BLOCK) void bg_inject_deck_kernel(BgDev d, const uint4* __restrict__ decks, const uint8_t* __restrict__ mask_in) {
  int env = blockIdx.x * BG_BLOCK + threadIdx.x;
  if (env >= d.N) return;
  if (mask_in && !mask_in[env]) return;
#pragma unroll
  for (int k = 0; k < BG_NDECK; k++) d.deck[(size_t)k * d.N + env] = decks[(size_t)env * BG_NDECK + k];
}
__global__ __launch_bounds__(BG_BLOCK) void bg_set_cap_kernel(BgDev d, const int32_t* __restrict__ caps, int scalar, const uint8_t* __restrict__ mask_in) {
  int env = blockIdx.x * BG_BLOCK + threadIdx.x;
  if (env >= d.N) return;
  if (mask_in && !mask_in[env]) return;
  uint32_t* w = ((uint32_t*)&d.hot[(size_t)7 * d.N + env]) + 3;
  const int cap = caps ? caps[env] : scalar;
  *w = (*w & 0xffffu) | ((uint32_t)(cap & 0xff) << 16);
}

struct bg_handle {
  BgDev dev;
  int device_id;
  bool seeded;
  int64_t* d_seeds;
  uint8_t* d_mask;
  uint32_t* d_jtab;
  int steps_since_refill;
  std::vector<uint4> h_tmpl;
  std::vector<hipEvent_t> ev_pool;
  std::vector<uint8_t> h_cap;
  uint64_t bytes;
  std::string err;
  bool profiling;
  uint32_t* d_prod[2];
  long refill_seq;
  long refill_done;
  long view_min;
  bool async_refill;
  hipStream_t side;
  hipEvent_t ev_refill[2];
  hipEvent_t ev_rollout;
  std::vector<hipEvent_t> ev_rollout_t, ev_refill_t, ev_step_t;
  std::vector<int> rollout_steps;
  struct RefillPiece { int kind; uint32_t part, nparts; int grid; uint32_t cursor, max_made; };
  std::vector<RefillPiece> pieces;
  size_t piece_next;
  BgDev piece_dev;
  int refill_sliced, piece_parts[4], deck_passes;
  uint32_t eng_smask; int eng_copiers;
  int engine;
  int e3_cfg, e3_epw;
  uint8_t* gpeer[8]; uint8_t** d_gpeer; int gworld, grank;
};

static std::string g_create_err;

struct BgDeviceGuard {
  int prev = -1;
  bool switched = false;
  explicit BgDeviceGuard(int dev) {
    if (hipGetDevice(&prev) == hipSuccess && prev != dev) switched = hipSetDevice(dev) == hipSuccess;
  }
  ~BgDeviceGuard() { if (switched) (void)hipSetDevice(prev); }
};
#define BG_GUARD(h) BgDeviceGuard _guard((h)->device_id)

#define BG_HIP(call)                                                                                   \
  do {                                                                                                 \
    hipError_t _e = (call);                                                                            \
    if (_e != hipSuccess) {                                                                            \
      h->err = std::string(#call) + ": " + hipGetErrorString(_e);                                      \
      return BG_E_HIP;                                                                                 \
    }                                                                                                  \
  } while (0)

template <typename T>
static hipError_t bg_alloc(bg_handle* h, T** p, size_t count) {
  size_t bytes = count * sizeof(T);
  hipError_t e = hipMalloc((void**)p, bytes);
  if (e != hipSuccess) return e;
  h->bytes += bytes;
  return hipMemset(*p, 0, bytes);
}

static int bg_grid(const bg_handle* h) { return (h->dev.N + BG_BLOCK - 1) / BG_BLOCK; }

static hipEvent_t bg_ev_take(bg_handle* h) {
  if (!h->ev_pool.empty()) { hipEvent_t e = h->ev_pool.back(); h->ev_pool.pop_back(); return e; }
  hipEvent_t e = nullptr;
  return hipEventCreate(&e) == hipSuccess ? e : nullptr;
}
static void bg_ev_begin(bg_handle* h, std::vector<hipEvent_t>& v, hipStream_t s) {
  if (!h->profiling) return;
  hipEvent_t a = bg_ev_take(h), b = bg_ev_take(h);
  if (!a || !b) { if (a) h->ev_pool.push_back(a); if (b) h->ev_pool.push_back(b); return; }
  v.push_back(a); v.push_back(b);
  (void)hipEventRecord(a, s);
}
// ... 49 lines not shown
  BG_GUARD(h);
  BG_HIP(hipDeviceSynchronize());
  BG_HIP(hipMemcpy(out4, h->dev.wl_count, 4 * sizeof(unsigned int), hipMemcpyDeviceToHost));
  return 0;
}

int bg_set_profiling(bg_handle* h, int enable) {
  if (!h) return BG_E_ARG;
  h->profiling = enable != 0;
  if (h->profiling) { BG_GUARD(h); while (h->ev_pool.size() < 128) { hipEvent_t e = nullptr; if (hipEventCreate(&e) != hipSuccess) break; h->ev_pool.push_back(e); } }
  return 0;
}

int bg_get_profile(bg_handle* h, double* out8) {
  if (!h || !out8) return BG_E_ARG;
  BG_GUARD(h);
  BG_HIP(hipDeviceSynchronize());
  double nr = (double)(h->ev_rollout_t.size() / 2), nf = (double)(h->ev_refill_t.size() / 2), ns = (double)(h->ev_step_t.size() / 2);
  double steps = 0;
  for (int t : h->rollout_steps) steps += t;
  h->rollout_steps.clear();
  out8[0] = bg_ev_sum(h, h->ev_rollout_t); out8[1] = nr; out8[2] = steps;
  out8[3] = bg_ev_sum(h, h->ev_refill_t); out8[4] = nf;
  out8[5] = bg_ev_sum(h, h->ev_step_t); out8[6] = ns; out8[7] = 0;
  return 0;
}

int bg_create(int n_envs, int device_id, uint32_t flags, int max_ante, bg_handle** out) { return bg_create_ex(n_envs, device_id, flags, max_ante, 0, out); }

int bg_create_ex(int n_envs, int device_id, uint32_t flags, int max_ante, int fused_steps_hint, bg_handle** out) {
  if (!out || n_envs <= 0) { g_create_err = "bg_create: bad arguments"; return BG_E_ARG; }
  int ndev = 0;
  if (hipGetDeviceCount(&ndev) != hipSuccess || ndev <= 0) {
    g_create_err = "bg_create: no HIP device visible (this library has no CPU fallback)";
    return BG_E_NODEVICE;
  }
  if (device_id < 0 || device_id >= ndev) { g_create_err = "bg_create: device_id out of range"; return BG_E_ARG; }
  bg_handle* h = new bg_handle();
  h->device_id = device_id; h->seeded = false; h->bytes = 0; h->profiling = false;
  { const char* av = getenv("BG_ASYNC_REFILL"); h->async_refill = av ? atoi(av) != 0 : true; }
  {
    auto geti = [](const char* k, int dflt) { const char* v = getenv(k); return v ? atoi(v) : dflt; };
    h->refill_sliced = geti("BG_REFILL_SLICED", 1);
    { const int dp[4] = {2, 1, 2, 8};
      for (int k = 0; k < 4; k++) h->piece_parts[k] = dp[k];
      auto get4 = [](const char* k, int* out, int lo, int hi) { const char* v = getenv(k); if (!v) return; int a[4]; if (sscanf(v, "%d,%d,%d,%d", &a[0], &a[1], &a[2], &a[3]) == 4) for (int i = 0; i < 4; i++) out[i] = a[i] < lo ? lo : a[i] > hi ? hi : a[i]; };
      get4("BG_REFILL_PARTS", h->piece_parts, 1, 16); }
    h->piece_next = 0;
    h->deck_passes = 3;
    while (h->deck_passes * h->piece_parts[0] > BG_WL_COUNTERS - 8) { if (h->deck_passes > 1) h->deck_passes--; else h->piece_parts[0]--; }
    h->eng_smask = (uint32_t)geti("BG_ENG_SMASK", BG_ENG_SMASK_DEFAULT); h->eng_copiers = geti("BG_ENG_COPIERS", 0); if (h->eng_copiers < 0 || h->eng_copiers > 3) h->eng_copiers = 0;
    if (h->eng_smask == 0 || h->eng_smask >= (1u << BG_ENG_NW) || __builtin_popcount(h->eng_smask) > BG_ENG_NSV) h->eng_smask = BG_ENG_SMASK_DEFAULT;
    h->engine = geti("BG_ENGINE", 3);
    if (h->engine != 1 && h->engine != 3) { delete h; g_create_err = "bg_create: BG_ENGINE must be 3 (bg_engine3.h, the default) or 1 (bg_engine.h); the two-kernel engine 2 was retired in round 5"; return BG_E_ARG; }
    h->e3_cfg = geti("BG_E3_CFG", 0);
    if (h->e3_cfg != 0 && h->e3_cfg != 113 && h->e3_cfg != 213 && h->e3_cfg != 413) { delete h; g_create_err = "bg_create: BG_E3_CFG must be 113, 213 or 413 (100 x owner waves + 10 x slices + service waves)"; return BG_E_ARG; }
    for (int g = 0; g < 8; g++) h->gpeer[g] = nullptr;
    h->d_gpeer = nullptr;
    h->gworld = 0; h->grank = 0;
    h->e3_epw = geti("BG_E3_EPW", 0);
    if (h->e3_epw != 0 && (h->e3_epw < 1 || h->e3_epw > 64)) { delete h; g_create_err = "bg_create: BG_E3_EPW must be in [1, 64]"; return BG_E_ARG; }
  }
  h->d_prod[0] = h->d_prod[1] = nullptr; h->refill_seq = 0; h->view_min = 0; h->refill_done = -1; h->side = nullptr;
  h->ev_refill[0] = h->ev_refill[1] = nullptr; h->ev_rollout = nullptr;
  h->d_seeds = nullptr; h->d_mask = nullptr; h->d_jtab = nullptr; h->steps_since_refill = 0;
  memset(&h->dev, 0, sizeof(h->dev));
  BgDev& d = h->dev;
  d.N = n_envs; d.flags = flags; d.max_ante = max_ante;
  const char* kg = getenv("BG_KG"); const char* ks = getenv("BG_KS"); const char* kd = getenv("BG_KD");
  int dsd = n_envs <= 131072 ? 248 : (n_envs <= 262144 ? 124 : (n_envs <= 1048576 ? 24 : 12));
  int dg = 2 * (int)((bg_gwords(flags, 3 * (dsd / 2)) + BG_MT_N - 1) / BG_MT_N) + 1; if (dg < 5) dg = 5;
  if (fused_steps_hint > 0) {
    const int hint = fused_steps_hint > 372 ? 372 : fused_steps_hint;
    int ring = 2 * ((hint + 2) / 3); if (ring < 4) ring = 4;
    int gb = 2 * (int)((bg_gwords(flags, hint) + BG_MT_N - 1) / BG_MT_N) + 1; if (gb < 5) gb = 5;
    if (ring < dsd) dsd = ring;
    if (gb < dg) dg = gb;
  }
  d.KG = kg ? atoi(kg) : dg; d.KS = ks ? atoi(ks) : dsd + 1; d.KD = kd ? atoi(kd) : dsd;
  if (d.KG < 2 || d.KS < 2 || d.KD < 1 || d.KG > 250 || d.KS > 250 || d.KD > 250) { delete h; g_create_err = "bg_create: bad ring depths"; return BG_E_ARG; }
  size_t N = (size_t)n_envs;
  BG_GUARD(h);
  hipError_t e = hipSuccess;
  if (e == hipSuccess) e = bg_alloc(h, &d.hot, BG_NHOT * N);
  if (e == hipSuccess) e = bg_alloc(h, &d.deck, BG_NDECK * N);
  if (e == hipSuccess) e = bg_alloc(h, &d.cold, BG_NCOLD * N);
  if (e == hipSuccess) e = bg_alloc(h, &d.tmpl, BG_NTMPL * N);
  if (e == hipSuccess) e = bg_alloc(h, &d.ndeck, (size_t)d.KD * BG_NDECK * N);
  if (e == hipSuccess) e = bg_alloc(h, &d.gblk, (size_t)d.KG * BG_MTS * N);
  if (e == hipSuccess) e = bg_alloc(h, &d.sblk, (size_t)d.KS * BG_SLOT_WORDS * N);
  if (e == hipSuccess) e = bg_alloc(h, &d.sovf, (size_t)BG_MTS * N);
  if (e == hipSuccess && (flags & BG_FLAG_CARD_STATES)) {
    e = bg_alloc(h, &d.cstate, (size_t)BG_NCST * N);
    if (e == hipSuccess) e = bg_alloc(h, &d.ctmpl, (size_t)BG_NCST * N);
    if (e == hipSuccess) e = bg_alloc(h, &d.cardmt, (size_t)BG_MTS * N);
    if (e == hipSuccess) e = bg_alloc(h, &d.sealmt, (size_t)BG_MTS * N);
  }
  if (e == hipSuccess) e = bg_alloc(h, &d.deckmt, (size_t)BG_MTS * N);
  if (e == hipSuccess) e = bg_alloc(h, &d.shopgenmt, (size_t)BG_MTS * N);
  if (e == hipSuccess) e = bg_alloc(h, &d.wl_count, BG_WL_COUNTERS);
  if (e == hipSuccess) e = bg_alloc(h, &d.wl, 3 * N);
  if (e == hipSuccess) e = bg_alloc(h, &d.wl_shop, 2 * N * (size_t)(d.KS - 1));
  if (e == hipSuccess) e = bg_alloc(h, &d.sseed, (size_t)BG_SSEED * N);
  if (e == hipSuccess) e = bg_alloc(h, &d.smeta, N);
  if (e == hipSuccess) e = bg_alloc(h, &h->d_prod[0], N);
  if (e == hipSuccess) e = bg_alloc(h, &h->d_prod[1], N);
  int prio_least = 0, prio_greatest = 0;
  if (e == hipSuccess) e = hipDeviceGetStreamPriorityRange(&prio_least, &prio_greatest);
  if (e == hipSuccess) e = hipStreamCreateWithPriority(&h->side, hipStreamNonBlocking, prio_least);
  if (e == hipSuccess) e = hipEventCreateWithFlags(&h->ev_refill[0], hipEventDisableTiming);
  if (e == hipSuccess) e = hipEventCreateWithFlags(&h->ev_refill[1], hipEventDisableTiming);
  if (e == hipSuccess) e = hipEventCreateWithFlags(&h->ev_rollout, hipEventDisableTiming);
  if (e == hipSuccess) e = bg_alloc(h, &h->d_jtab, (sizeof(JTables) + 3) / 4);
  if (e == hipSuccess) e = bg_alloc(h, &d.dbg, 32);
  if (e == hipSuccess) e = bg_alloc(h, &d.err, 4);
  if (e == hipSuccess) e = bg_alloc(h, &h->d_seeds, N);
  if (e == hipSuccess) e = bg_alloc(h, &h->d_mask, N);
  if (e != hipSuccess) {
    g_create_err = std::string("bg_create: ") + hipGetErrorString(e);
    bg_destroy(h);
    return BG_E_HIP;
  }
  d.prod_view = h->d_prod[0]; d.prod_in = h->d_prod[0]; d.prod_out = h->d_prod[1];
  d.jtab = h->d_jtab;
  hipLaunchKernelGGL(bg_tables_build_kernel, dim3(1), dim3(256), 0, 0, h->d_jtab);
  if (hipGetLastError() != hipSuccess || hipDeviceSynchronize() != hipSuccess) { g_create_err = "bg_create: table kernel failed"; bg_destroy(h); return BG_E_HIP; }
  h->h_tmpl.assign(BG_NTMPL * N, make_uint4(0, 0, 0, 0));
  h->h_cap.assign(N, (uint8_t)(max_ante > 0 && max_ante < 256 ? max_ante : 0));
  if (max_ante < 0 || max_ante > 255) { g_create_err = "bg_create: max_ante must be in [0, 255]"; bg_destroy(h); return BG_E_ARG; }
  if (max_ante > 0) {
    hipLaunchKernelGGL(bg_set_cap_kernel, dim3(bg_grid(h)), dim3(BG_BLOCK), 0, 0, d, (const int32_t*)nullptr, max_ante, (const uint8_t*)nullptr);
    if (hipGetLastError() != hipSuccess || hipDeviceSynchronize() != hipSuccess) { g_create_err = "bg_create: cap kernel failed"; bg_destroy(h); return BG_E_HIP; }
  }
  *out = h;
  return 0;
}

int bg_destroy(bg_handle* h) {
  if (!h) return 0;
  { BG_GUARD(h);
  BgDev& d = h->dev;
  (void)hipDeviceSynchronize();
  if (h->side) (void)hipStreamDestroy(h->side);
  for (int i = 0; i < 2; i++) if (h->ev_refill[i]) (void)hipEventDestroy(h->ev_refill[i]);
  if (h->ev_rollout) (void)hipEventDestroy(h->ev_rollout);
  for (hipEvent_t e : h->ev_pool) (void)hipEventDestroy(e);
  for (auto* v : {&h->ev_rollout_t, &h->ev_refill_t, &h->ev_step_t}) for (hipEvent_t e : *v) (void)hipEventDestroy(e);
  hipFree(h->d_prod[0]); hipFree(h->d_prod[1]);
  hipFree(d.hot); hipFree(d.deck); hipFree(d.cold); hipFree(d.tmpl); hipFree(d.ndeck); hipFree(d.gblk); hipFree(d.sblk); hipFree(d.sovf);
  hipFree(d.deckmt); hipFree(d.shopgenmt); hipFree(d.err); hipFree(h->d_seeds); hipFree(h->d_mask); hipFree(d.wl_count); hipFree(d.wl); hipFree(d.wl_shop); hipFree(d.sseed); hipFree(d.smeta); hipFree(d.dbg); hipFree(h->d_jtab); hipFree(h->d_gpeer); hipFree(d.cstate); hipFree(d.ctmpl); hipFree(d.cardmt); hipFree(d.sealmt);
  }
  delete h;
  return 0;
}

const char* bg_last_error(const bg_handle* h) { return h ? h->err.c_str() : g_create_err.c_str(); }
int bg_num_envs(const bg_handle* h) { return h ? h->dev.N : 0; }

static int bg_chunk_limit(const bg_handle* h, bool* async_out) {
  int ring = h->dev.KD < h->dev.KS - 1 ? h->dev.KD : h->dev.KS - 1;
  int gblocks = h->dev.KG - 1;
  const bool async = h->async_refill && ring >= 2 && gblocks >= 2;
  if (async) { ring /= 2; gblocks /= 2; }
  int max_chunk = 3 * ring;
  int gchunk = bg_gsteps(h->dev.flags, gblocks);
  if (gchunk < max_chunk) max_chunk = gchunk;
  if (max_chunk < 1) max_chunk = 1;
  if (async_out) *async_out = async;
  return max_chunk;
}
int bg_max_fused_steps(const bg_handle* h) { return h ? bg_chunk_limit(h, nullptr) : 0; }
uint64_t bg_state_bytes(const bg_handle* h) { return h ? h->bytes : 0; }

static uint32_t* bg_prod_latest(bg_handle* h) { return h->d_prod[(h->refill_seq + 1) & 1]; }

static BgDev bg_dev_view(bg_handle* h, const uint32_t* view) {
  BgDev d = h->dev;
  d.prod_view = view;
  return d;
}

static int bg_refill_pieces(bg_handle* h, int n);
static int bg_wait_refill(bg_handle* h, hipStream_t s, int back) {
  long i = h->refill_seq - 1 - back;
  if (i < 0) return 0;
  if (back == 0 && h->piece_next < h->pieces.size()) { int rc = bg_refill_pieces(h, 1 << 30); if (rc) return rc; }
  BG_HIP(hipStreamWaitEvent(s, h->ev_refill[i & 1], 0));
  return 0;
}

static int bg_refill_pieces(bg_handle* h, int n) {
  const BgDev& d = h->piece_dev;
  hipStream_t s = h->side;
  while (n-- > 0 && h->piece_next < h->pieces.size()) {
    const bg_handle::RefillPiece& pc = h->pieces[h->piece_next++];
    const BgPart pt{pc.part, pc.nparts};
    hipEvent_t ea = nullptr, eb = nullptr;
    bg_ev_pair(h, h->ev_refill_t, ea, eb);
    const dim3 g(pc.grid), b(BG_BLOCK);
    if (ea) {
      if (pc.kind == 0) hipExtLaunchKernelGGL(bg_refill_deck_kernel, g, b, 0, s, ea, eb, 0, d, pt, pc.cursor, pc.max_made);
      else if (pc.kind == 1) hipExtLaunchKernelGGL(bg_refill_seedring_kernel, g, b, 0, s, ea, eb, 0, d, pt);
      else if (pc.kind == 2) hipExtLaunchKernelGGL(bg_refill_gblk_kernel, g, b, 0, s, ea, eb, 0, d, pt);
      else hipExtLaunchKernelGGL(bg_refill_shop_kernel, g, b, 0, s, ea, eb, 0, d, pt);
    } else {
      if (pc.kind == 0) hipLaunchKernelGGL(bg_refill_deck_kernel, g, b, 0, s, d, pt, pc.cursor, pc.max_made);
      else if (pc.kind == 1) hipLaunchKernelGGL(bg_refill_seedring_kernel, g, b, 0, s, d, pt);
      else if (pc.kind == 2) hipLaunchKernelGGL(bg_refill_gblk_kernel, g, b, 0, s, d, pt);
      else hipLaunchKernelGGL(bg_refill_shop_kernel, g, b, 0, s, d, pt);
    }
// ... 426 lines not shown
  BG_HIP(hipDeviceSynchronize());
  BG_HIP(hipMemcpy(h->d_gpeer, h->gpeer, sizeof(h->gpeer), hipMemcpyHostToDevice));
  h->gworld = world; h->grank = rank;
  return 0;
}

int bg_rollout(bg_handle* h, int T, int policy, uint64_t policy_seed, uint64_t env_index0, uint64_t t0,
               const bg_obs_ptrs* obs, int obs_stride_steps, double* reward_dev, uint8_t* terminated_dev,
               int32_t* actions_out_dev, bg_rollout_stats* stats_dev, void* stream) {
  return bg_rollout_impl(h, T, policy, policy_seed, env_index0, t0, obs, nullptr, 0, obs_stride_steps, reward_dev,
                         terminated_dev, actions_out_dev, stats_dev, stream);
}

int bg_rollout_rows(bg_handle* h, int T, int policy, uint64_t policy_seed, uint64_t env_index0, uint64_t t0,
                    uint8_t* rows_dev, uint64_t row_stride_bytes, int rows_stride_steps, bg_rollout_stats* stats_dev,
                    void* stream) {
  if (!h) return BG_E_ARG;
  if ((uint64_t)h->dev.N * (uint64_t)bg_max_fused_steps(h) > 0xffffffffull) { h->err = "bg_rollout_rows: more than 2**32 records per launch (envs x fused steps)"; return BG_E_ARG; }
  if (!rows_dev || row_stride_bytes < BG_ROW_BYTES || (row_stride_bytes & 15) || ((uintptr_t)rows_dev & 15) || row_stride_bytes > 0xffffffffull) {
    h->err = "bg_rollout_rows: rows_dev must be 16-byte aligned and row_stride_bytes a multiple of 16, >= BG_ROW_BYTES";
    return BG_E_ARG;
  }
  return bg_rollout_impl(h, T, policy, policy_seed, env_index0, t0, nullptr, rows_dev, (size_t)row_stride_bytes,
                         rows_stride_steps, nullptr, nullptr, nullptr, stats_dev, stream);
}

int bg_step_many_rows(bg_handle* h, int K, const int32_t* actions_dev, uint8_t* rows_dev, uint64_t row_stride_bytes,
                      int rows_stride_steps, bg_rollout_stats* stats_dev, void* stream) {
  if (!h) return BG_E_ARG;
  if (!actions_dev || K <= 0) { h->err = "bg_step_many_rows: actions_dev must be a device pointer to [K, N] int32 actions, K > 0"; return BG_E_ARG; }
  if ((uint64_t)h->dev.N * (uint64_t)bg_max_fused_steps(h) > 0xffffffffull) { h->err = "bg_step_many_rows: more than 2**32 records per launch (envs x fused steps)"; return BG_E_ARG; }
  if (const char* m = bg_rows_args(rows_dev, row_stride_bytes)) { h->err = std::string("bg_step_many_rows: ") + m; return BG_E_ARG; }
  return bg_rollout_impl(h, K, 0, 0, 0, 0, nullptr, rows_dev, (size_t)row_stride_bytes, rows_stride_steps, nullptr, nullptr, nullptr, stats_dev,
                         stream, actions_dev, (h->dev.flags & BG_FLAG_AUTORESET) != 0);
}

__global__ __launch_bounds__(BG_BLOCK) void bg_inject_cards_kernel(BgDev d, const uint16_t* __restrict__ cs, const uint8_t* __restrict__ mask_in, int apply_now) {
  int env = blockIdx.x * BG_BLOCK + threadIdx.x;
  if (env >= d.N) return;
  if (mask_in && !mask_in[env]) return;
  const uint4* src = (const uint4*)(cs + (size_t)env * 56);
#pragma unroll
  for (int k = 0; k < BG_NCST; k++) {
    uint4 v = src[k];
    d.ctmpl[(size_t)k * d.N + env] = v;
    if (apply_now) d.cstate[(size_t)k * d.N + env] = v;
  }
}

int bg_inject_cards(bg_handle* h, const uint8_t* enh_host, const uint8_t* edition_host, const uint8_t* seal_host,
                    const uint8_t* mask_host, int apply_now, void* stream) {
  if (!h) return BG_E_ARG;
  if (!h->dev.cstate) { h->err = "bg_inject_cards: the handle was created without BG_FLAG_CARD_STATES"; return BG_E_ARG; }
  BG_GUARD(h);
  hipStream_t s = (hipStream_t)stream;
  const size_t N = h->dev.N;
  std::vector<uint16_t> packed(N * 56, 0);
  for (size_t i = 0; i < N; i++)
    for (int c = 0; c < 52; c++) {
      const uint32_t e = enh_host ? enh_host[i * 52 + c] : 0, d = edition_host ? edition_host[i * 52 + c] : 0, sl = seal_host ? seal_host[i * 52 + c] : 0;
      if (e > 15 || d > 15 || sl > 15) { h->err = "bg_inject_cards: state codes are 0..15"; return BG_E_ARG; }
      packed[i * 56 + c] = (uint16_t)(e | (d << 4) | (sl << 8));
    }
  uint16_t* dcs = nullptr;
  BG_HIP(hipMalloc(&dcs, packed.size() * sizeof(uint16_t)));
  BG_HIP(hipMemcpyAsync(dcs, packed.data(), packed.size() * sizeof(uint16_t), hipMemcpyHostToDevice, s));
  if (mask_host) BG_HIP(hipMemcpyAsync(h->d_mask, mask_host, N, hipMemcpyHostToDevice, s));
  hipLaunchKernelGGL(bg_inject_cards_kernel, dim3(bg_grid(h)), dim3(BG_BLOCK), 0, s, h->dev, (const uint16_t*)dcs,
                     mask_host ? (const uint8_t*)h->d_mask : (const uint8_t*)nullptr, apply_now);
  BG_HIP(hipGetLastError());
  BG_HIP(hipStreamSynchronize(s));
  BG_HIP(hipFree(dcs));
  return 0;
}

int bg_inject(bg_handle* h, const int32_t* jokers_host, const int32_t* njokers_host, const int64_t* money_host,
              const int32_t* ante_host, const uint8_t* levels_host, const uint8_t* mask_host, int apply_now, void* stream) {
  if (!h) return BG_E_ARG;
  BG_GUARD(h);
  hipStream_t s = (hipStream_t)stream;
  size_t N = h->dev.N;
  for (size_t i = 0; i < N; i++) {
    if (mask_host && !mask_host[i]) continue;
    uint4& t0 = h->h_tmpl[i];
    uint4& t1 = h->h_tmpl[N + i];
    uint32_t fl = t0.y >> 24;
    uint32_t j4 = t0.y & 0xffu, nj = (t0.y >> 8) & 0xffu, an = (t0.y >> 16) & 0xffu;
    if (jokers_host && njokers_host) {
      int n = njokers_host[i];
      if (n < 0 || n > 5) { h->err = "bg_inject: njokers must be in [0,5]"; return BG_E_ARG; }
      uint32_t lo = 0; j4 = 0;
      for (int k = 0; k < n; k++) {
        int id = jokers_host[i * 5 + k];
        if (id < 1 || id > 150) { h->err = "bg_inject: joker id out of range"; return BG_E_ARG; }
        if (k < 4) lo |= (uint32_t)id << (8 * k); else j4 = (uint32_t)id;
      }
      t0.x = lo; nj = (uint32_t)n; fl |= 0x80u;
    }
    if (money_host) { if (money_host[i] >= 0) { t0.z = (uint32_t)(int32_t)money_host[i]; fl |= 0x40u; } else fl &= ~0x40u; }
    if (ante_host) {
      if (ante_host[i] > 255 || (h->h_cap[i] > 0 && ante_host[i] > (int)h->h_cap[i])) { h->err = "bg_inject: template ante above the env's curriculum cap (max_ante)"; return BG_E_ARG; }
      if (ante_host[i] > 0) { an = (uint32_t)ante_host[i] & 0xffu; fl |= 0x20u; } else fl &= ~0x20u;
    }
    if (levels_host) {
      uint64_t lv = 0; bool any = false;
      for (int k = 0; k < 12; k++) { int l = levels_host[i * 12 + k]; if (l) any = true; if (l < 1) l = 1; if (l > 15) l = 15; lv |= (uint64_t)l << (4 * k); }
      if (any) { t1.x = (uint32_t)lv; t1.y = (uint32_t)(lv >> 32); fl |= 0x10u; } else fl &= ~0x10u;
    }
    t0.y = j4 | (nj << 8) | (an << 16) | (fl << 24);
  }
  BG_HIP(hipMemcpyAsync(h->dev.tmpl, h->h_tmpl.data(), BG_NTMPL * N * sizeof(uint4), hipMemcpyHostToDevice, s));
  if (apply_now) {
    if (mask_host) BG_HIP(hipMemcpyAsync(h->d_mask, mask_host, N, hipMemcpyHostToDevice, s));
    { const int rcw = bg_wait_refill(h, s, 0); if (rcw) return rcw; }
    hipLaunchKernelGGL(bg_inject_kernel, dim3(bg_grid(h)), dim3(BG_BLOCK), 0, s, bg_dev_view(h, bg_prod_latest(h)),
                       mask_host ? (const uint8_t*)h->d_mask : (const uint8_t*)nullptr);
    BG_HIP(hipGetLastError());
  }
  BG_HIP(hipStreamSynchronize(s));
  return 0;
}

int bg_inject_consumables(bg_handle* h, const int32_t* ids_host, const int32_t* n_host, const uint8_t* mask_host, int apply_now,
                          void* stream) {
  if (!h || !ids_host || !n_host) return BG_E_ARG;
  BG_GUARD(h);
  hipStream_t s = (hipStream_t)stream;
  size_t N = h->dev.N;
  for (size_t i = 0; i < N; i++) {
    if (mask_host && !mask_host[i]) continue;
    int n = n_host[i];
    if (n < 0) { h->h_tmpl[N + i].z = 0; continue; }
    if (n > 2) { h->err = "bg_inject_consumables: an env holds at most consumable_slots = 2"; return BG_E_ARG; }
    uint32_t v = 0x80000000u | (uint32_t)n;
    for (int k = 0; k < n; k++) {
      int id = ids_host[i * 2 + k];
      bool planet = id >= 30 && id <= 41, other = (id >= 1 && id <= 22) || (id >= 50 && id <= 67);
      if (!planet && !other) { h->err = "bg_inject_consumables: ids are 1-22 (tarots), 30-41 (planets), 50-67 (spectrals)"; return BG_E_ARG; }
      if (other && !h->dev.cstate) { h->err = "bg_inject_consumables: tarot / spectral cards need BG_FLAG_CARD_STATES"; return BG_E_ARG; }
      v |= (uint32_t)id << (8 * (k + 1));
    }
    h->h_tmpl[N + i].z = v;
  }
  BG_HIP(hipMemcpyAsync(h->dev.tmpl, h->h_tmpl.data(), BG_NTMPL * N * sizeof(uint4), hipMemcpyHostToDevice, s));
  if (apply_now) {
    if (mask_host) BG_HIP(hipMemcpyAsync(h->d_mask, mask_host, N, hipMemcpyHostToDevice, s));
    { const int rcw = bg_wait_refill(h, s, 0); if (rcw) return rcw; }
    hipLaunchKernelGGL(bg_inject_kernel, dim3(bg_grid(h)), dim3(BG_BLOCK), 0, s, bg_dev_view(h, bg_prod_latest(h)),
                       mask_host ? (const uint8_t*)h->d_mask : (const uint8_t*)nullptr);
    BG_HIP(hipGetLastError());
  }
  BG_HIP(hipStreamSynchronize(s));
  return 0;
}

struct BgSlice { void* base; size_t rows; size_t elem; };
static void bg_slices(bg_handle* h, std::vector<BgSlice>& v) {
  BgDev& d = h->dev;
  v.push_back({d.hot, BG_NHOT, 16}); v.push_back({d.deck, BG_NDECK, 16}); v.push_back({d.cold, BG_NCOLD, 16});
  v.push_back({d.tmpl, BG_NTMPL, 16}); v.push_back({d.ndeck, (size_t)d.KD * BG_NDECK, 16});
  v.push_back({d.gblk, 1, (size_t)d.KG * BG_MTS * 4}); v.push_back({d.sblk, 1, (size_t)d.KS * BG_SLOT_WORDS * 4}); v.push_back({d.sovf, 1, (size_t)BG_MTS * 4});
  v.push_back({d.deckmt, 1, (size_t)BG_MTS * 4}); v.push_back({d.shopgenmt, 1, (size_t)BG_MTS * 4});
  v.push_back({d.sseed, 1, BG_SSEED * 4}); v.push_back({d.smeta, 1, 4});
  v.push_back({bg_prod_latest(h), 1, 4});
  if (d.cstate) { v.push_back({d.cstate, BG_NCST, 16}); v.push_back({d.ctmpl, BG_NCST, 16}); v.push_back({d.cardmt, 1, (size_t)BG_MTS * 4}); v.push_back({d.sealmt, 1, (size_t)BG_MTS * 4}); }
}
uint64_t bg_state_blob_bytes(const bg_handle* h) {
  if (!h) return 0;
  std::vector<BgSlice> v;
  bg_slices(const_cast<bg_handle*>(h), v);
  uint64_t b = 16;
  for (auto& s : v) b += s.rows * s.elem;
  return b;
}
#define BG_BLOB_MAGIC 0x42474d58u
#define BG_BLOB_VERSION 7u
static int bg_blob_args(bg_handle* h, const char* fn, int env_index, const void* blob, uint64_t blob_bytes) {
  if (!h) return BG_E_ARG;
  char buf[200];
  if (!blob) { h->err = std::string(fn) + ": null blob"; return BG_E_ARG; }
  if (env_index < 0 || env_index >= h->dev.N) { snprintf(buf, sizeof(buf), "%s: env_index %d out of range [0, %d)", fn, env_index, h->dev.N); h->err = buf; return BG_E_ARG; }
  const uint64_t want = bg_state_blob_bytes(h);
  if (blob_bytes < want) {
    snprintf(buf, sizeof(buf), "%s: blob of %llu bytes, this handle's blobs are %llu bytes (ring depths and card-state flag decide the size)", fn,
             (unsigned long long)blob_bytes, (unsigned long long)want);
    h->err = buf; return BG_E_ARG;
  }
  return 0;
}
int bg_get_state(bg_handle* h, int env_index, void* blob_host, uint64_t blob_bytes) {
  int rc = bg_blob_args(h, "bg_get_state", env_index, blob_host, blob_bytes);
  if (rc) return rc;
  BG_GUARD(h);
  rc = bg_refill_pieces(h, 1 << 30);
  if (rc) return rc;
  BG_HIP(hipDeviceSynchronize());
  uint8_t* out = (uint8_t*)blob_host;
  uint32_t hdr[4] = {BG_BLOB_MAGIC, BG_BLOB_VERSION, (uint32_t)h->dev.KG | (h->dev.cstate ? 0x10000u : 0u), (uint32_t)h->dev.KS | ((uint32_t)h->dev.KD << 16)};
  memcpy(out, hdr, 16); out += 16;
  std::vector<BgSlice> v;
  bg_slices(h, v);
  size_t N = h->dev.N;
  for (auto& s : v) {
    BG_HIP(hipMemcpy2D(out, s.elem, (uint8_t*)s.base + (size_t)env_index * s.elem, N * s.elem, s.elem, s.rows, hipMemcpyDeviceToHost));
    out += s.rows * s.elem;
  }
  return 0;
}
int bg_set_state(bg_handle* h, int env_index, const void* blob_host, uint64_t blob_bytes) {
  int rc = bg_blob_args(h, "bg_set_state", env_index, blob_host, blob_bytes);
  if (rc) return rc;
  BG_GUARD(h);
  const uint8_t* in = (const uint8_t*)blob_host;
  uint32_t hdr[4];
  memcpy(hdr, in, 16); in += 16;
  char buf[200];
  if (hdr[0] != BG_BLOB_MAGIC) { h->err = "bg_set_state: not a state blob (bad magic)"; return BG_E_ARG; }
  if (hdr[1] != BG_BLOB_VERSION) { snprintf(buf, sizeof(buf), "bg_set_state: blob version %u, this library reads version %u", hdr[1], BG_BLOB_VERSION); h->err = buf; return BG_E_ARG; }
  if (hdr[2] != ((uint32_t)h->dev.KG | (h->dev.cstate ? 0x10000u : 0u)) || hdr[3] != ((uint32_t)h->dev.KS | ((uint32_t)h->dev.KD << 16))) {
    snprintf(buf, sizeof(buf), "bg_set_state: the blob was saved with ring depths %u/%u/%u%s, this handle has %d/%d/%d%s", hdr[2] & 0xffffu, hdr[3] & 0xffffu, hdr[3] >> 16,
             (hdr[2] & 0x10000u) ? " + card states" : "", h->dev.KG, h->dev.KS, h->dev.KD, h->dev.cstate ? " + card states" : "");
    h->err = buf; return BG_E_ARG;
  }
  rc = bg_refill_pieces(h, 1 << 30);
  if (rc) return rc;
  BG_HIP(hipDeviceSynchronize());
  std::vector<BgSlice> v;
  bg_slices(h, v);
  size_t N = h->dev.N;
  for (auto& s : v) {
    BG_HIP(hipMemcpy2D((uint8_t*)s.base + (size_t)env_index * s.elem, N * s.elem, in, s.elem, s.elem, s.rows, hipMemcpyHostToDevice));
    if (s.base == (void*)h->dev.tmpl)
      for (size_t r = 0; r < s.rows; r++) memcpy(&h->h_tmpl[r * N + (size_t)env_index], in + r * s.elem, sizeof(uint4));
    if (s.base == (void*)h->dev.hot) { uint4 c7; memcpy(&c7, in + 7 * s.elem, sizeof(uint4)); h->h_cap[env_index] = (uint8_t)((c7.w >> 16) & 0xffu); }
    in += s.rows * s.elem;
  }
  {
    uint32_t w = 0;
    BG_HIP(hipMemcpy(&w, bg_prod_latest(h) + env_index, 4, hipMemcpyDeviceToHost));
    BG_HIP(hipMemcpy(h->d_prod[0] + env_index, &w, 4, hipMemcpyHostToDevice));
    BG_HIP(hipMemcpy(h->d_prod[1] + env_index, &w, 4, hipMemcpyHostToDevice));
  }
  h->seeded = true;
  h->steps_since_refill = 1 << 30;
  return 0;
}

int bg_inject_deck(bg_handle* h, const uint8_t* decks_host, const uint8_t* mask_host, void* stream) {
  if (!h || !decks_host) return BG_E_ARG;
  BG_GUARD(h);
  hipStream_t s = (hipStream_t)stream;
  const size_t N = h->dev.N;
  std::vector<uint8_t> packed(N * 64, 0);
  for (size_t i = 0; i < N; i++) {
    if (mask_host && !mask_host[i]) continue;
    uint64_t seen = 0;
    for (int c = 0; c < 52; c++) {
      const uint8_t v = decks_host[i * 52 + c];
      if (v >= 52 || ((seen >> v) & 1ull)) { h->err = "bg_inject_deck: every deck must be a permutation of the 52 card codes (rank-2)*4+suit"; return BG_E_ARG; }
      seen |= 1ull << v;
      packed[i * 64 + c] = v;
    }
  }
  uint4* dd = nullptr;
  BG_HIP(hipMalloc((void**)&dd, packed.size()));
  BG_HIP(hipMemcpyAsync(dd, packed.data(), packed.size(), hipMemcpyHostToDevice, s));
  if (mask_host) BG_HIP(hipMemcpyAsync(h->d_mask, mask_host, N, hipMemcpyHostToDevice, s));
  { int rcw = bg_wait_refill(h, s, 0); if (rcw) { (void)hipFree(dd); return rcw; } }
  hipLaunchKernelGGL(bg_inject_deck_kernel, dim3(bg_grid(h)), dim3(BG_BLOCK), 0, s, h->dev, (const uint4*)dd,
                     mask_host ? (const uint8_t*)h->d_mask : (const uint8_t*)nullptr);
  BG_HIP(hipGetLastError());
  BG_HIP(hipStreamSynchronize(s));
  BG_HIP(hipFree(dd));
  return 0;
}

int bg_set_max_ante(bg_handle* h, int max_ante, const int32_t* per_env_host, const uint8_t* mask_host, void* stream) {
  if (!h) return BG_E_ARG;
  BG_GUARD(h);
  hipStream_t s = (hipStream_t)stream;
  const size_t N = h->dev.N;
  if (!per_env_host && (max_ante < 0 || max_ante > 255)) { h->err = "bg_set_max_ante: the cap must be in [0, 255] (0 = none)"; return BG_E_ARG; }
  int32_t* dc = nullptr;
  for (size_t i = 0; i < N; i++) {
    if (mask_host && !mask_host[i]) continue;
    const int c = per_env_host ? per_env_host[i] : max_ante;
    if (c < 0 || c > 255) { h->err = "bg_set_max_ante: every cap must be in [0, 255] (0 = none)"; return BG_E_ARG; }
    const uint32_t ty = h->h_tmpl[i].y;
    if (c > 0 && ((ty >> 24) & 0x20u) && (int)((ty >> 16) & 0xffu) > c) { h->err = "bg_set_max_ante: a cap below the env's template ante (bg_inject)"; return BG_E_ARG; }
  }
  for (size_t i = 0; i < N; i++)
    if (!mask_host || mask_host[i]) h->h_cap[i] = (uint8_t)(per_env_host ? per_env_host[i] : max_ante);
  if (per_env_host) {
    BG_HIP(hipMalloc((void**)&dc, N * sizeof(int32_t)));
    BG_HIP(hipMemcpyAsync(dc, per_env_host, N * sizeof(int32_t), hipMemcpyHostToDevice, s));
  }
  if (mask_host) BG_HIP(hipMemcpyAsync(h->d_mask, mask_host, N, hipMemcpyHostToDevice, s));
  hipLaunchKernelGGL(bg_set_cap_kernel, dim3(bg_grid(h)), dim3(BG_BLOCK), 0, s, h->dev, (const int32_t*)dc, max_ante,
                     mask_host ? (const uint8_t*)h->d_mask : (const uint8_t*)nullptr);
  BG_HIP(hipGetLastError());
  BG_HIP(hipStreamSynchronize(s));
  if (dc) BG_HIP(hipFree(dc));
  if (!per_env_host && !mask_host) h->dev.max_ante = max_ante;
  return 0;
}

#define BG_HIP0(call)                                                                                  \
  do {                                                                                                 \
    hipError_t _e = (call);                                                                            \
    if (_e != hipSuccess) {                                                                            \
      g_create_err = std::string(#call) + ": " + hipGetErrorString(_e);                                \
      return BG_E_HIP;                                                                                 \
    }                                                                                                  \
  } while (0)

__global__ __launch_bounds__(256) void bg_stream_copy_kernel(const bg_cp_u32x4* __restrict__ src, bg_cp_u32x4* __restrict__ dst, size_t n16) {
  const size_t i = (size_t)blockIdx.x * 256 * 4 + threadIdx.x;
  bg_cp_u32x4 v[4];
#pragma unroll
  for (int k = 0; k < 4; k++) if (i + (size_t)k * 256 < n16) v[k] = __builtin_nontemporal_load(&src[i + (size_t)k * 256]);
#pragma unroll
  for (int k = 0; k < 4; k++) if (i + (size_t)k * 256 < n16) __builtin_nontemporal_store(v[k], &dst[i + (size_t)k * 256]);
}
int bg_bench_copy(const void* src_dev, void* dst_dev, uint64_t bytes, int iters, double* gbps_out, void* stream) {
  if (!src_dev || !dst_dev || !gbps_out || bytes < 16 || iters < 1 || ((uintptr_t)src_dev & 15) || ((uintptr_t)dst_dev & 15)) { g_create_err = "bg_bench_copy: bad arguments"; return BG_E_ARG; }
  hipStream_t s = (hipStream_t)stream;
  const size_t n16 = bytes / 16;
  const unsigned grid = (unsigned)((n16 + 1023) / 1024);
  hipEvent_t a, b;
  BG_HIP0(hipEventCreate(&a)); BG_HIP0(hipEventCreate(&b));
  for (int i = 0; i < 2; i++) hipLaunchKernelGGL(bg_stream_copy_kernel, dim3(grid), dim3(256), 0, s, (const bg_cp_u32x4*)src_dev, (bg_cp_u32x4*)dst_dev, n16);
  BG_HIP0(hipEventRecord(a, s));
  for (int i = 0; i < iters; i++) hipLaunchKernelGGL(bg_stream_copy_kernel, dim3(grid), dim3(256), 0, s, (const bg_cp_u32x4*)src_dev, (bg_cp_u32x4*)dst_dev, n16);
  BG_HIP0(hipEventRecord(b, s));
  BG_HIP0(hipGetLastError());
  BG_HIP0(hipEventSynchronize(b));
  float ms = 0;
  BG_HIP0(hipEventElapsedTime(&ms, a, b));
  (void)hipEventDestroy(a); (void)hipEventDestroy(b);
  *gbps_out = ms > 0 ? 2.0 * (double)(n16 * 16) * iters / (ms * 1e-3) / 1e9 : 0.0;
  return 0;
}

__global__ __launch_bounds__(256) void bg_stream_fill_kernel(uint4* __restrict__ dst, size_t n16, uint32_t seed) {
  const size_t i = (size_t)blockIdx.x * 256 + threadIdx.x;
  if (i < n16) dst[i] = make_uint4(seed, (uint32_t)i, 0u, seed ^ (uint32_t)i);
}
int bg_bench_fill(void* dst_dev, uint64_t bytes, int iters, double* gbps_out, void* stream) {
  if (!dst_dev || !gbps_out || bytes < 16 || iters < 1 || ((uintptr_t)dst_dev & 15)) { g_create_err = "bg_bench_fill: bad arguments"; return BG_E_ARG; }
  hipStream_t s = (hipStream_t)stream;
  const size_t n16 = bytes / 16;
  const unsigned grid = (unsigned)((n16 + 255) / 256);
  hipEvent_t a, b;
  BG_HIP0(hipEventCreate(&a)); BG_HIP0(hipEventCreate(&b));
  for (int i = 0; i < 2; i++) hipLaunchKernelGGL(bg_stream_fill_kernel, dim3(grid), dim3(256), 0, s, (uint4*)dst_dev, n16, 0u);
  BG_HIP0(hipEventRecord(a, s));
  for (int i = 0; i < iters; i++) hipLaunchKernelGGL(bg_stream_fill_kernel, dim3(grid), dim3(256), 0, s, (uint4*)dst_dev, n16, (uint32_t)i + 1u);
  BG_HIP0(hipEventRecord(b, s));
  BG_HIP0(hipGetLastError());
  BG_HIP0(hipEventSynchronize(b));
  float ms = 0;
  BG_HIP0(hipEventElapsedTime(&ms, a, b));
  (void)hipEventDestroy(a); (void)hipEventDestroy(b);
  *gbps_out = ms > 0 ? (double)(n16 * 16) * iters / (ms * 1e-3) / 1e9 : 0.0;
  return 0;
}

struct BgOpTimer {
  hipEvent_t a = nullptr, b = nullptr;
  bool on = false;
  int begin(float* out, hipStream_t s) { on = out != nullptr; if (!on) return 0; BG_HIP0(hipEventCreate(&a)); BG_HIP0(hipEventCreate(&b)); BG_HIP0(hipEventRecord(a, s)); return 0; }
// ... 489 lines not shown
```

### balatro_gym_amd/csrc/bg_step.h

```cpp
#pragma once
#include "bg_device.h"

struct StepOut {
  double reward;
  int64_t final_score;
  double terms[8];
  int32_t error, flags, aux;
  int32_t hand_type, cards_played;
  bool terminated;
  double* bd_dst;
};

struct ShopRegs { uint4 c3, c4, c5, c6; bool valid; };
__device__ __forceinline__ void bg_shop_load(const BgDev& d, int env, ShopRegs& sr) {
  if (sr.valid) return;
  size_t N = d.N;
  sr.c3 = bg_ld16a(&d.cold[3 * N + env]); sr.c4 = bg_ld16a(&d.cold[4 * N + env]); sr.c5 = bg_ld16a(&d.cold[5 * N + env]); sr.c6 = bg_ld16a(&d.cold[6 * N + env]);
  sr.valid = true;
}
__device__ __forceinline__ void bg_shop_store(const BgDev& d, int env, const ShopRegs& sr) {
  size_t N = d.N;
  d.cold[3 * N + env] = sr.c3; d.cold[4 * N + env] = sr.c4; d.cold[5 * N + env] = sr.c5; d.cold[6 * N + env] = sr.c6;
}
__device__ __forceinline__ void bg_shop_unpack(const ShopRegs& sr, int32_t cost[9], uint32_t tp[9]) {
  cost[0] = sr.c3.x; cost[1] = sr.c3.y; cost[2] = sr.c3.z; cost[3] = sr.c3.w;
  cost[4] = sr.c4.x; cost[5] = sr.c4.y; cost[6] = sr.c4.z; cost[7] = sr.c4.w; cost[8] = sr.c5.x;
  tp[0] = sr.c5.y & 0xffffu; tp[1] = sr.c5.y >> 16; tp[2] = sr.c5.z & 0xffffu; tp[3] = sr.c5.z >> 16;
  tp[4] = sr.c5.w & 0xffffu; tp[5] = sr.c5.w >> 16; tp[6] = sr.c6.x & 0xffffu; tp[7] = sr.c6.x >> 16; tp[8] = sr.c6.y & 0xffffu;
}
__device__ __forceinline__ void bg_shop_pack(ShopRegs& sr, const int32_t cost[9], const uint32_t tp[9]) {
  sr.c3 = make_uint4(cost[0], cost[1], cost[2], cost[3]);
  sr.c4 = make_uint4(cost[4], cost[5], cost[6], cost[7]);
  sr.c5 = make_uint4(cost[8], tp[0] | (tp[1] << 16), tp[2] | (tp[3] << 16), tp[4] | (tp[5] << 16));
  sr.c6 = make_uint4(tp[6] | (tp[7] << 16), tp[8], 0, 0);
  sr.valid = true;
}
enum { IT_PACK = 1, IT_CARD = 2, IT_JOKER = 3, IT_VOUCHER = 4 };
enum { PK_STANDARD = 0, PK_JOKER = 1, PK_TAROT = 2, PK_PLANET = 3, PK_SPECTRAL = 4 };

__device__ __forceinline__ uint64_t bg_action_mask(const BgDev& d, int env, const Env& e, ShopRegs& sr) {
  uint64_t m = 0;
  if (e.phase == 0) {
    int n = e.nhand < 8 ? e.nhand : 8;
    m |= ((1ull << n) - 1) << 2;
    if (e.nsel > 0) { m |= 1ull; if (e.discards_left > 0) m |= 2ull; }
    m |= ((1ull << e.ncons) - 1) << 10;
  } else if (e.phase == 1) {
    if (e.bflags & BG_BF_SHOP_EXISTS) {
      bg_shop_load(d, env, sr);
      int32_t cost[9]; uint32_t tp[9];
      bg_shop_unpack(sr, cost, tp);
#pragma unroll
      for (int i = 0; i < 9; i++)
        if (i < e.shop_n && e.money >= cost[i]) m |= 1ull << (20 + i);
      if (e.money >= e.shop_reroll_state) m |= 1ull << 30;
    }
    m |= 1ull << 31;
    m |= ((1ull << e.njokers) - 1) << 32;
  } else if (e.phase == 2) {
    m |= 0xfull << 45;
  }
  return m;
}

typedef uint32_t bg_pv_u32x4 __attribute__((ext_vector_type(4)));
typedef __attribute__((address_space(3))) const bg_pv_u32x4 lds_cu4;
template <class DK>
__device__ __forceinline__ void bg_env_reset(const BgDev& d, int env, Env& e, DK& dk, const uint4* pre = nullptr, lds_cu4* pv = nullptr, int pv_stride = 0) {
  const uint4 t0 = d.tmpl[env], t1 = d.tmpl[(size_t)d.N + env];
  e.ante = 1; e.round = 1; e.phase = 2; e.chips_needed = 300; e.chips_scored = 0; e.round_chips = 0; e.money = 4;
  e.hand = 0; e.nhand = 0; e.sel = 0; e.nsel = 0; e.hands_left = 4; e.discards_left = 3; e.hand_size = 8;
  e.njokers = 0; e.jokers = 0; e.ncons = 0; e.cons0 = 0; e.cons1 = 0; e.n_magic = 0; e.n_minim = 0;
  e.shop_reroll_state = 5; e.hp_total = 0; e.hp_ante = 0; e.best_hand = 0; e.jokers_sold = 0;
  e.boss_type = 0; e.boss_types = 0; e.boss_cards = 0; e.boss_hp = 0; e.boss_req = 5; e.face_down = 0;
  e.bflags = (e.bflags & BG_BF_SHOP_EXISTS) | BG_BF_FIRST_HAND;
  e.highlighted = 0;
  e.ndrop = 0; e.nfo = 0;
  e.levels = 0x111111111111ull;
  e.excess = 0;
#pragma unroll
  for (int k = 0; k < 3; k++) d.cold[(size_t)k * d.N + env] = make_uint4(0, 0, 0, 0);
  if (e.d_ready <= 0) atomicOr(d.err, BG_DEVERR_DECKRING);
  else {
#pragma unroll
    for (int k = 0; k < BG_NDECK; k++) {
      uint4 c;
      if (pv) { const bg_pv_u32x4 v = pv[k * pv_stride]; c = make_uint4(v.x, v.y, v.z, v.w); }
      else c = pre ? pre[k] : d.ndeck[((size_t)e.d_head * BG_NDECK + k) * d.N + env];
      d.deck[(size_t)k * d.N + env] = c;
      bg_deck_set(dk, k, c);
    }
    e.d_head = (e.d_head + 1 == d.KD) ? 0 : e.d_head + 1;
    e.d_ready--; e.d_cons = (e.d_cons + 1) & 0xff;
  }
  int tnj = (int)bg_b(t0.y, 1);
  if (t0.y & 0x80000000u) { e.njokers = tnj; e.jokers = (uint64_t)t0.x | ((uint64_t)(t0.y & 0xffu) << 32); }
  if (t0.y & 0x40000000u) e.money = (int32_t)t0.z;
  if (t0.y & 0x20000000u) e.ante = (int)bg_b(t0.y, 2);
  if (t0.y & 0x10000000u) e.levels = (uint64_t)t1.x | ((uint64_t)(t1.y & 0xffffu) << 32);
  if (t1.z & 0x80000000u) { e.ncons = (int)bg_b(t1.z, 0); e.cons0 = bg_b(t1.z, 1); e.cons1 = bg_b(t1.z, 2); }
  if constexpr (DK::kCards) {
#pragma unroll
    for (int k = 0; k < BG_NCST; k++) d.cstate[(size_t)k * d.N + env] = d.ctmpl[(size_t)k * d.N + env];
  }
}

__device__ __forceinline__ double bg_shop_cost_mult(const Env& e, lds_JTables* jt) {
  int k = e.shop_ante - 1;
  k = k < 0 ? 0 : (k > 100 ? 100 : k);
  double m = jt->pow115[k];
  if (e.n_magic > 0) m *= 0.9;
  return m;
}

__device__ __forceinline__ uint64_t bg_sorted_jokers(const Env& e) {
  uint64_t v = e.jokers | (e.njokers < 8 ? (~0ull << (8 * e.njokers)) : 0ull);
#pragma unroll 1
  for (int pass = 0; pass < 4; pass++) {
#pragma unroll
    for (int i = 0; i < 4; i++) {
      uint32_t a = (uint32_t)(v >> (8 * i)) & 0xffu, b2 = (uint32_t)(v >> (8 * (i + 1))) & 0xffu;
      if (a > b2) v = (v & ~(0xffffull << (8 * i))) | ((uint64_t)b2 << (8 * i)) | ((uint64_t)a << (8 * (i + 1)));
    }
  }
#pragma unroll
  for (int i = 4; i >= 1; i--)
    if (((v >> (8 * i)) & 0xffull) == ((v >> (8 * (i - 1))) & 0xffull)) v |= 0xffull << (8 * i);
  return v;
}
__device__ __forceinline__ int bg_candidate(uint64_t sorted, int j) {
  int id = j + 1;
#pragma unroll
  for (int q = 0; q < 5; q++) { int o = (int)((sorted >> (8 * q)) & 0xff); if (o <= id && o <= 145) id++; }
  return id;
}

struct BgPk6 { uint32_t a, b, c, d, e, f; };
__device__ __forceinline__ uint32_t bg_pk_byte(const BgPk6 pk, int i) {
  const int g = i >> 2;
  uint32_t wv = pk.a;
  wv = g == 1 ? pk.b : wv; wv = g == 2 ? pk.c : wv; wv = g == 3 ? pk.d : wv; wv = g == 4 ? pk.e : wv; wv = g == 5 ? pk.f : wv;
  return (wv >> (8 * (i & 3))) & 0xffu;
}
__device__ __forceinline__ uint32_t bg_movemask4(uint32_t f) { return (((f >> 7) & 0x01010101u) * 0x01020408u) >> 24; }

__device__ __forceinline__ void bg_shop_inventory(const BgDev& d, int env, Env& e, RngWin& w, ShopRegs& sr) {
  BG_PROBE_BEGIN();
  bool full_state;
  const uint32_t* S = bg_sbase(d, env, e, full_state);
  const bool fresh = e.s_idx == 0 && !full_state;
  uint4 q0 = make_uint4(0, 0, 0, 0), q1 = q0;
  if (fresh) { const uint4* S4 = (const uint4*)(S + BG_SW_PK); q0 = S4[0]; q1 = S4[1]; }
  double mult = bg_shop_cost_mult(e, w.jt);
  const uint64_t sj = bg_sorted_jokers(e);
  int owned145 = 0;
#pragma unroll
  for (int q = 0; q < 5; q++) owned145 += bg_get8(sj, q) <= 145 ? 1 : 0;
  const uint32_t nc = (uint32_t)(145 - owned145);
  int third_r = 0, p0 = 0, p1 = 0, p2 = 0, v = 0, ca = 0, cb = 0;
  bool fast = false;
  if (fresh) {
    const BgPk6 pk{q0.x, q0.y, q0.z, q0.w, q1.x, q1.y};
    BG_PROBE(18);
    const uint32_t H = 0x80808080u;
    const uint32_t addnc = (0x80u - (nc & 0x7fu)) * 0x01010101u;
    uint32_t m3 = 0, m2 = 0, m8 = 0, m52 = 0;
#define BG_INV_CLASS(x, g) do { \
      const uint32_t ge192 = (x) & ((x) << 1);                                    \
      const uint32_t ge208 = ge192 & (((x) << 2) | ((x) << 3));                   \
      const uint32_t genc = (x) & (((x) & 0x7f7f7f7fu) + addnc);                  \
      m3 |= bg_movemask4(~ge192 & H) << (4 * (g)); \
      m2 |= bg_movemask4(~(x) & H) << (4 * (g));                                  \
// ... 495 lines not shown
    }
  }
  int level = bg_level(e, ht);
  int bchips, bmult;
  bg_hand_base(ht, level, bchips, bmult);
  int64_t chips = bchips + chip_sum, mult = bmult;
  double x_mult = 1.0;
  BG_PROBE(1);
  if ((d.flags & 1u) && e.njokers > 0) {
    ChainIn in;
    in.phist = phist; in.pcodes = pcodes; in.scnt = scnt; in.stone = stone; in.n = n; in.ht = ht; in.kings = kings; in.queens = queens;
    in.all_black = false; in.deck_len = 52; in.style = 0;
    int chain_money = 0;
    bg_joker_chain<false, DK>(d, env, e, w, in, chips, mult, x_mult, chain_money, &pre);
  }
  BG_PROBE(15);
  int64_t final_score = (int64_t)((double)(chips * mult) * x_mult);
  if (o.bd_dst) {
    int gems = 0;
    if ((d.flags & 1u) && e.njokers > 0) {
#pragma unroll
      for (int j = 0; j < 5; j++) gems += (j < e.njokers && bg_get8(e.jokers, j) == 116) ? 1 : 0;
    }
    double2* q = (double2*)o.bd_dst;
    q[0] = make_double2((double)chips, (double)mult); q[1] = make_double2(x_mult, (double)chip_sum);
    q[2] = make_double2((double)bchips, (double)bmult); q[3] = make_double2((double)(gems * (int)((scnt >> 4) & 0xfu)), 0.0);
  }
  int retriggers = 0;
  if constexpr (DK::kCards) {
    int extra_money = 0, blue = 0;
#pragma unroll 1
    for (int c = 0; c < n; c++) {
      const uint32_t b = (uint32_t)(cst >> (8 * c)) & 0xffu, enh = b & 0xfu, seal = b >> 4;
      if (enh == 4u) (void)bg_lazy_random(d.cardmt + (size_t)env * BG_MTS);
      else if (enh == 8u) {
        (void)bg_lazy_random(d.cardmt + (size_t)env * BG_MTS);
        if (bg_lazy_random(d.cardmt + (size_t)env * BG_MTS) < 0.0667) extra_money += 20;
      }
      if (seal == 1u) extra_money += 3; else if (seal == 2u) retriggers++; else if (seal == 3u) blue++;
    }
    if (blue && e.ncons < 2) {
      const int PLANET_ID[12] = {38, 30, 31, 32, 33, 34, 35, 36, 37, 39, 40, 41};
#pragma unroll 1
      for (int q = 0; q < blue; q++)
        if (e.ncons < 2) { if (e.ncons == 0) e.cons0 = PLANET_ID[ht]; else e.cons1 = PLANET_ID[ht]; e.ncons++; }
    }
    double steel = 1.0;
    uint32_t selpos = 0;
#pragma unroll 1
    for (int q = 0; q < e.nsel; q++) { int sp = bg_get8(e.sel, q); if (sp < e.nhand) selpos |= 1u << sp; }
#pragma unroll 1
    for (int i = 0; i < e.nhand; i++)
      if (!((selpos >> i) & 1u) && (bg_cstate(d, env, bg_get8(e.hand, i)) & 0xfu) == 5u) steel *= 1.5;
    final_score = (int64_t)((double)final_score * steel);
    e.money += extra_money;
  }
  BG_PROBE(16);
  if (e.boss_type) {
    int64_t mc = bchips, mm = bmult;
    if (e.boss_type == 21) { mc = mc / 2; mm = mm / 2; }
    else if (e.boss_type == 22) mc = 0;
    else if (e.boss_type == 23) { mc = (int64_t)((double)mc * 0.75); mm = (int64_t)((double)mm * 0.75); }
    int deb = 0;
    if (e.boss_type == 14) deb = djqk;
    else if (e.boss_type == 24) deb = n;
    else if (e.boss_type == 16) deb = __popcll(e.boss_cards & pmask);
    if (deb > 0) {
      double pen = w.jt->pow08[deb];
      mc = (int64_t)((double)mc * pen);
      mm = (int64_t)((double)mm * pen);
    }
    double cr = (double)mc / (double)bchips, mr = (double)mm / (double)bmult;
    final_score = (int64_t)((double)final_score * cr * mr);
  }
  if constexpr (DK::kCards) final_score = (int64_t)((double)final_score * (1.0 + (double)retriggers * 0.5));
  BG_PROBE(17);
  int64_t need1 = e.chips_needed > 1 ? e.chips_needed : 1;
  double old_progress = (double)e.round_chips / (double)need1;
  if (old_progress > 1.0) old_progress = 1.0;
  e.round_chips += final_score;
  e.chips_scored += final_score;
  e.hp_total++; e.hp_ante++;
  if (final_score > e.best_hand) e.best_hand = final_score;
  atomicAdd(((uint32_t*)&d.cold[(size_t)(ht >> 2) * d.N + env]) + (ht & 3), 1u);
  if (e.boss_type) {
    e.boss_types |= 1u << ht;
    e.bflags &= ~BG_BF_FIRST_HAND;
    e.boss_hp++;
    if (e.boss_type == 16) e.boss_cards |= pmask;
    if (e.boss_type == 25) e.boss_req = e.boss_req + 1 > 7 ? 7 : e.boss_req + 1;
  }
  e.nsel = 0; e.sel = 0;
  BG_PROBE(10);
  double new_progress = (double)e.round_chips / (double)need1;
  if (new_progress > 1.0) new_progress = 1.0;
  double progress_reward = 15.0 * new_progress;
  double milestone = 0.0;
  if (old_progress < 0.25 && 0.25 <= new_progress) milestone = 5.0;
  else if (old_progress < 0.5 && 0.5 <= new_progress) milestone = 10.0;
  else if (old_progress < 0.75 && 0.75 <= new_progress) milestone = 15.0;
  else if (old_progress < 1.0 && 1.0 <= new_progress) milestone = 25.0;
  double score_reward;
  if (e.ante <= 3) { score_reward = (double)final_score / 100.0; if (score_reward > 10.0) score_reward = 10.0; }
  else {
    int64_t s = final_score > 1 ? final_score : 1;
    score_reward = s >= BG_LOG10_N ? 10.0 : 3.0 * BG_LOG10[s];
    if (score_reward > 10.0) score_reward = 10.0;
  }
  double hq;
  switch (ht) {
    case 0: hq = 0.1; break; case 1: hq = 0.5; break; case 2: hq = 1.0; break; case 3: hq = 2.0; break;
    case 4: hq = 2.5; break; case 5: hq = 2.5; break; case 6: hq = 3.5; break; case 7: hq = 5.0; break;
    case 8: hq = 7.0; break; case 9: hq = 10.0; break; default: hq = 0.0; break;
  }
  double eff = 0.0;
  if (ht >= 3 && n <= 3) eff = 2.0;
  else if (ht >= 5 && n == 5) eff = 1.0;
  else if (n <= 4 && e.hands_left <= 2) eff = 1.5;
  double syn = 0.0;
  if (e.njokers > 0) {
    uint32_t jf = bg_joker_flags(e, w.jt);
    if (ht == 5 && (jf & 1u)) syn += 2.0;
    if ((ht == 1 || ht == 2 || ht == 3) && (jf & 2u)) syn += 1.5;
    if (faces > 0 && (jf & 4u)) syn += 0.5 * (double)faces;
  }
  double strat = 0.0;
  if (new_progress > 0.7 && e.hands_left >= 3) strat = 2.0;
  else if (new_progress < 0.3 && ht >= 5) strat = 3.0;
  double ante_bonus = 0.0;
  if (e.ante >= 4) { ante_bonus = (double)(e.ante - 3) * 0.5; if (ante_bonus > 5.0) ante_bonus = 5.0; }
  double r = progress_reward + milestone;
  r = r + score_reward;
  r = r + hq * 2.0;
  r = r + eff * 1.5;
  r = r + syn * 3.0;
  r = r + strat * 2.0;
  r = r + ante_bonus;
  if (r > 100.0) r = 100.0;
  o.terms[0] = progress_reward; o.terms[1] = milestone; o.terms[2] = score_reward; o.terms[3] = hq;
  o.terms[4] = eff; o.terms[5] = syn; o.terms[6] = strat; o.terms[7] = ante_bonus;
  o.final_score = final_score; o.hand_type = ht; o.cards_played = n;
  BG_PROBE(11);
  if (e.round_chips >= (int64_t)e.chips_needed) {
    double bonus = 25.0 + 10.0 * (double)e.ante;
    r += bonus < 50.0 ? bonus : 50.0;
    if (w.defer_adv) o.flags |= BG_FLAG_DEFER_ADV;
    else bg_advance_round<DK::kCards>(d, env, e, w, sr);
    o.flags |= 1;
  } else if (e.hands_left <= 1) {
    r += -50.0 * (1.0 - new_progress);
    o.terminated = true;
    o.flags |= 2;
  } else {
    e.hands_left -= 1;
    bg_draw_cards(e);
    if (e.boss_type) bg_boss_on_hand_drawn(d, env, e, w, dk);
  }
  BG_PROBE(12);
  o.reward = r;
  asm volatile("" ::"v"(touch0));
}

template <class DK>
__device__ __forceinline__ void bg_step_discard(const BgDev& d, int env, Env& e, const RngWin& w, const DK& dk, StepOut& o) {
  int n = 0, nfaces = 0, purple = 0;
#pragma unroll 1
  for (int i = 0; i < e.nsel; i++) {
// ... 228 lines not shown
        }
        break;
      case 13:
        raises = nt > 0;
        break;
      case 14:
        if (nt >= 2) { naff = 2; aff = tg; success = true; }
        break;
      case 15:
        money_gained = 5 * e.njokers < 50 ? 5 * e.njokers : 50; success = true;
        break;
      case 18: case 19: case 20: case 22:
        if (nt > 0) { naff = nt < 3 ? nt : 3; aff = tg; success = true; }
        break;
      case 21: {
        uint32_t p = 30u + bg_randbelow<false>(d, env, e, w, 9u);
        if (n < slots) { L |= p << (8 * n); n++; items = p; nitems = 1; }
        success = true;
        break;
      }
      case 50: case 51: case 52:
        raises = nt >= 1;
        break;
      case 53: case 61: case 63: case 64:
        if (nt >= 1) { naff = 1; aff = tg; set_seal = id == 53 ? 3 : (id == 61 ? 1 : (id == 63 ? 2 : 4)); success = true; }
        break;
      case 54:
        if (nt >= 1) { set_edi = 1 + (int)bg_randbelow<false>(d, env, e, w, 3u); naff = 1; aff = tg; success = true; }
        break;
      case 55:
        if (e.njokers < 5) {
          uint32_t k = bg_randbelow<false>(d, env, e, w, 14u);
          jc = k == 4u ? 0 : 137 + (int)k; njc = 1; hs = -1; success = true;
        }
        break;
      case 56: case 57:
        if (e.nhand > 0) { (void)bg_randbelow<false>(d, env, e, w, id == 56 ? 4u : 13u); raises = true; }
        break;
      case 58:
        if (e.njokers > 0) { hs = -1; success = true; }
        break;
      case 59: {
        const int nn = 52 - e.ndrop, n = nn + e.nfo;
        if (nn < 13) { unsupported = true; break; }
        uint64_t gone = 0; int nfgone = 0;
        if (n > 21) {
          uint32_t p0 = 0xffu, p1 = 0xffu, p2 = 0xffu, p3 = 0xffu;
#pragma unroll 1
          for (int i = 0; i < 5; i++) {
            uint32_t j; int guard = 0;
            do { j = bg_randbelow<false>(d, env, e, w, (uint32_t)n); } while ((j == p0 || j == p1 || j == p2 || j == p3) && ++guard < 4096);
            p3 = p2; p2 = p1; p1 = p0; p0 = j;
            if ((int)j < nn) gone |= 1ull << j; else nfgone++;
          }
        } else {
          uint64_t plo = 0, phi = 0;
#pragma unroll 1
          for (int i = 0; i < n; i++) { if (i < 12) plo |= (uint64_t)i << (5 * i); else phi |= (uint64_t)i << (5 * (i - 12)); }
#pragma unroll 1
          for (int i = 0; i < 5; i++) {
            const int j = (int)bg_randbelow<false>(d, env, e, w, (uint32_t)(n - i)), last = n - i - 1;
            const uint32_t pick = (uint32_t)((j < 12 ? plo >> (5 * j) : phi >> (5 * (j - 12))) & 31ull);
            const uint64_t lv = (last < 12 ? plo >> (5 * last) : phi >> (5 * (last - 12))) & 31ull;
            if (j < 12) plo = (plo & ~(31ull << (5 * j))) | (lv << (5 * j)); else phi = (phi & ~(31ull << (5 * (j - 12)))) | (lv << (5 * (j - 12)));
            if ((int)pick < nn) gone |= 1ull << pick; else nfgone++;
          }
        }
        DK& mdk = const_cast<DK&>(dk);
        uint32_t cur = 0; int wpos = 0; uint64_t played = 0;
#pragma unroll 1
        for (int i = 0; i < nn; i++)
          if (!((gone >> i) & 1ull)) {
            cur |= (uint32_t)bg_card(d, env, dk, i) << (8 * (wpos & 3));
            if ((e.boss_cards >> i) & 1ull) played |= 1ull << wpos;
            wpos++;
            if ((wpos & 3) == 0) { w.lds[((wpos >> 2) - 1) * BG_BLOCK] = cur; cur = 0; }
          }
#pragma unroll 1
        while (wpos < 64) { wpos++; if ((wpos & 3) == 0) { w.lds[((wpos >> 2) - 1) * BG_BLOCK] = cur; cur = 0; } }
        w.g_len = 0; w.s_len = 0; w.g_blk = -1;
#pragma unroll
        for (int k = 0; k < BG_NDECK; k++) {
          const uint4 c4 = make_uint4(w.lds[(4 * k) * BG_BLOCK], w.lds[(4 * k + 1) * BG_BLOCK], w.lds[(4 * k + 2) * BG_BLOCK], w.lds[(4 * k + 3) * BG_BLOCK]);
          d.deck[(size_t)k * d.N + env] = c4;
          bg_deck_set(mdk, k, c4);
        }
        e.boss_cards = played;
        e.ndrop += 5 - nfgone; e.nfo -= nfgone;
        ndestroyed = 5; money_gained = 20; success = true;
        break;
      }
      case 60:
        if (e.njokers > 0) {
          uint32_t k = bg_randbelow<false>(d, env, e, w, (uint32_t)e.njokers);
          jc = (d.flags & 1u) ? bg_get8(e.jokers, (int)k) : 0; njc = 1; success = true;
        }
        break;
      case 62:
        if (e.njokers > 0) { (void)bg_randbelow<false>(d, env, e, w, (uint32_t)e.njokers); success = true; }
        break;
      case 65:
        if (nt >= 1) { if (52 - e.ndrop + e.nfo + 2 > 127) { unsupported = true; break; } e.nfo += 2; ncreated = 2; success = true; }
        break;
      case 66:
        if (e.njokers < 5) { jc = 146 + (int)bg_randbelow<false>(d, env, e, w, 5u); njc = 1; success = true; }
        break;
      case 67:
        success = true;
        break;
      default: break;
    }
    if (raises) { o.reward = -1.0; o.error = 11; return; }
    if (unsupported) { o.reward = -1.0; o.error = 12; return; }
  }
  if (success) {
    double r = 0.0;
    L = (L & ((1u << (8 * ci)) - 1u)) | ((L >> (8 * (ci + 1))) << (8 * ci)); n--;
    if (money_gained > 0) { e.money += money_gained; r += (double)money_gained / 10.0; }
    if (planet >= 0) {
      const int ht = (int)((0xba9087654321ull >> (4 * planet)) & 0xfull);
      int lv = bg_level(e, ht);
      if (lv < 15) e.levels += 1ull << (4 * ht);
      else e.excess += 1ull << (4 * ht);
      r += 10.0;
    }
    if constexpr (DK::kCards) {
      if (naff) {
#pragma unroll 1
        for (int i = 0; i < naff; i++) {
          const int ti = bg_get8(aff, i);
          uint16_t* q = &((uint16_t*)&d.cstate[(size_t)(ti >> 3) * d.N + env])[ti & 7];
          uint32_t v = *q;
          if (set_enh >= 0) v = (v & ~0xfu) | (uint32_t)set_enh;
          if (set_edi >= 0) v = (v & ~0xf0u) | ((uint32_t)set_edi << 4);
          if (set_seal >= 0) v = (v & ~0xf00u) | ((uint32_t)set_seal << 8);
          *q = (uint16_t)v;
        }
        r += (double)naff * 2.0;
      }
      if (ncreated) r += (double)ncreated * 3.0;
      if (ndestroyed) r += (double)ndestroyed * 1.0;
      if (njc) {
        if (e.njokers < 5 && jc > 0) { e.jokers = bg_set8(e.jokers, e.njokers, jc); e.njokers++; }
        r += (double)njc * 15.0;
      }
      if (nitems) {
#pragma unroll 1
        for (int i = 0; i < nitems; i++)
          if (n < 2) { L |= ((items >> (8 * i)) & 0xffu) << (8 * n); n++; }
        r += (double)nitems * 5.0;
      }
      if (hs) e.hand_size += hs;
    }
    e.cons0 = L & 0xffu; e.cons1 = (L >> 8) & 0xffu; e.ncons = n;
    o.reward = r;
  } else { o.reward = -1.0; o.error = 8; }
  e.nsel = 0; e.sel = 0;
}

template <class DK>
__device__ __forceinline__ void bg_env_dispatch(const BgDev& d, int env, Env& e, RngWin& w, ShopRegs& sr, const DK& dk,
                                                int action, StepOut& o) {
  if (e.phase == 0) {
    if (action == 0) bg_step_play_hand(d, env, e, w, sr, dk, o);
    else if (action == 1) bg_step_discard(d, env, e, w, dk, o);
    else if (action < 10) bg_toggle_select(e, action - 2);
    else bg_use_consumable(d, env, e, w, dk, action - 10, o);
// ... 453 lines not shown
```

Before: 8.137 billion.

## Store deck and prefetched-deck rings per-env contiguously via index helpers

Adds shared host/device index helpers for every per-env state array and routes all accesses through them. The deck and ndeck arrays move from chunk-major (k*N+env) to env-major (env*4+k, and (env*KD+slot)*4+k) layouts, while hot, cold and tmpl keep their layout. Each env's 64-byte deck and each prefetched deck slot become one contiguous run, which should improve locality for the scattered per-env deck reads and the refill writes. The cost is that lanes now issue 16-byte accesses strided by 64 bytes, and the state save/load slicing is generalised with explicit env and row strides to match.

```diff
diff --git a/balatro_gym_amd/csrc/bg_device.h b/balatro_gym_amd/csrc/bg_device.h
--- a/balatro_gym_amd/csrc/bg_device.h
+++ b/balatro_gym_amd/csrc/bg_device.h
@@ -11,6 +11,18 @@
 #define BG_MT_M 397
 #define BG_MTS 640
 #define BG_BLOCK 64
+#define BG_HD __host__ __device__ __forceinline__
+
+BG_HD size_t bg_hot_at(size_t N, size_t env, int k) { return (size_t)k * N + env; }
+BG_HD size_t bg_hot_chunks(size_t N) { return N * BG_NHOT; }
+BG_HD size_t bg_cold_at(size_t N, size_t env, int k) { return (size_t)k * N + env; }
+BG_HD size_t bg_cold_chunks(size_t N) { return N * BG_NCOLD; }
+BG_HD size_t bg_tmpl_at(size_t N, size_t env, int k) { return (size_t)k * N + env; }
+BG_HD size_t bg_tmpl_chunks(size_t N) { return N * BG_NTMPL; }
+BG_HD size_t bg_deck_at(size_t N, size_t env, int k) { (void)N; return env * BG_NDECK + (size_t)k; }
+BG_HD size_t bg_ndeck_at(size_t N, size_t KD, size_t env, size_t slot, int k) { (void)N; return (env * KD + slot) * BG_NDECK + (size_t)k; }
+BG_HD size_t bg_deck_chunks(size_t N) { return N * BG_NDECK; }
+BG_HD size_t bg_ndeck_chunks(size_t N, size_t KD) { return N * KD * BG_NDECK; }
 
 #define BG_DEVERR_GSTREAM 1u
 #define BG_DEVERR_SHOPBLK 2u
@@ -59,6 +71,12 @@
   const uint32_t* jtab;
 };
 
+__device__ __forceinline__ uint4* bg_hot(const BgDev& d, int env, int k) { return d.hot + bg_hot_at((size_t)d.N, (size_t)env, k); }
+__device__ __forceinline__ uint4* bg_cold(const BgDev& d, int env, int k) { return d.cold + bg_cold_at((size_t)d.N, (size_t)env, k); }
+__device__ __forceinline__ uint4* bg_deck(const BgDev& d, int env, int k) { return d.deck + bg_deck_at((size_t)d.N, (size_t)env, k); }
+__device__ __forceinline__ uint4* bg_tmpl(const BgDev& d, int env, int k) { return d.tmpl + bg_tmpl_at((size_t)d.N, (size_t)env, k); }
+__device__ __forceinline__ uint4* bg_ndeck(const BgDev& d, int env, int slot, int k) { return d.ndeck + bg_ndeck_at((size_t)d.N, (size_t)d.KD, (size_t)env, (size_t)slot, k); }
+
 struct Env {
   int64_t chips_scored, round_chips;
   int64_t best_hand;
@@ -144,7 +162,7 @@
 __device__ __forceinline__ void bg_load_env(const BgDev& d, int env, Env& e) {
   uint4 c[BG_NHOT];
 #pragma unroll
-  for (int k = 0; k < BG_NHOT; k++) c[k] = d.hot[(size_t)k * d.N + env];
+  for (int k = 0; k < BG_NHOT; k++) c[k] = *bg_hot(d, env, k);
   bg_unpack(c, e);
   bg_derive_ready(e, d.prod_view ? d.prod_view[env] : 0u);
 }
@@ -152,7 +170,7 @@
   uint4 c[BG_NHOT];
   bg_pack(e, c);
 #pragma unroll
-  for (int k = 0; k < BG_NHOT; k++) d.hot[(size_t)k * d.N + env] = c[k];
+  for (int k = 0; k < BG_NHOT; k++) *bg_hot(d, env, k) = c[k];
 }
 
 __device__ __forceinline__ int bg_get8(uint64_t v, int i) { return (int)((v >> (8 * i)) & 0xffull); }
@@ -227,7 +245,7 @@
   return (uint32_t)((const uint16_t*)&d.cstate[(size_t)(ci >> 3) * d.N + env])[ci & 7];
 }
 __device__ __forceinline__ Deck0 bg_load_deck0(const BgDev& d, int env) {
-  uint4 c = d.deck[env];
+  uint4 c = *bg_deck(d, env, 0);
   Deck0 r;
   r.lo = ((uint64_t)c.y << 32) | c.x;
   r.hi = ((uint64_t)c.w << 32) | c.z;
@@ -241,7 +259,7 @@
 }
 __device__ __forceinline__ int bg_card(const BgDev& d, int env, const Deck0& k, int idx) {
   if (idx < 16) return (int)(((idx < 8 ? k.lo : k.hi) >> (8 * (idx & 7))) & 0xffull);
-  const uint32_t* p = (const uint32_t*)&d.deck[(size_t)(idx >> 4) * d.N + env];
+  const uint32_t* p = (const uint32_t*)bg_deck(d, env, idx >> 4);
   return (int)((bg_ld4a(p + ((idx & 15) >> 2)) >> (8 * (idx & 3))) & 0xffu);
 }
 template <int S, bool C> struct DeckLdsS { lds_u32* col; static constexpr bool kCards = C; };
diff --git a/balatro_gym_amd/csrc/bg_engine.h b/balatro_gym_amd/csrc/bg_engine.h
--- a/balatro_gym_amd/csrc/bg_engine.h
+++ b/balatro_gym_amd/csrc/bg_engine.h
@@ -115,9 +115,9 @@
     int act0 = 0;
     if (mine) {
 #pragma unroll
-      for (int k = 0; k < BG_NHOT; k++) c[k] = d.hot[(size_t)k * N + envp];
-#pragma unroll
-      for (int k = 0; k < BG_NDECK; k++) dw[k] = d.deck[(size_t)k * N + envp];
+      for (int k = 0; k < BG_NHOT; k++) c[k] = *bg_hot(d, envp, k);
+#pragma unroll
+      for (int k = 0; k < BG_NDECK; k++) dw[k] = *bg_deck(d, envp, k);
       prod = d.prod_view ? d.prod_view[envp] : 0u;
       if (a.actions_in) act0 = a.actions_in[envp];
     }
@@ -158,7 +158,7 @@
       __builtin_amdgcn_s_setprio(1);
       uint4 c[BG_NHOT];
 #pragma unroll
-      for (int k = 0; k < BG_NHOT; k++) if (k != 3 && k != 4) c[k] = d.hot[(size_t)k * N + envp];
+      for (int k = 0; k < BG_NHOT; k++) if (k != 3 && k != 4) c[k] = *bg_hot(d, envp, k);
       c[3] = s_c34[0][l0]; c[4] = s_c34[1][l0];
       Env pe;
       ShopRegs psr; psr.valid = false;
@@ -460,7 +460,7 @@
         BG_PROBE_BEGIN();
         uint4 c[BG_NHOT];
 #pragma unroll
-        for (int k = 0; k < BG_NHOT; k++) if (k != 3 && k != 4) c[k] = d.hot[(size_t)k * N + env];
+        for (int k = 0; k < BG_NHOT; k++) if (k != 3 && k != 4) c[k] = *bg_hot(d, env, k);
         c[3] = s_c34[0][l]; c[4] = s_c34[1][l];
         Env e;
         bg_unpack(c, e);
@@ -488,7 +488,7 @@
         BG_PROBE(26);
         bg_pack(e, c);
 #pragma unroll
-        for (int k = 0; k < BG_NHOT; k++) if (k != 3 && k != 4) d.hot[(size_t)k * N + env] = c[k];
+        for (int k = 0; k < BG_NHOT; k++) if (k != 3 && k != 4) *bg_hot(d, env, k) = c[k];
         s_c34[0][l] = c[3]; s_c34[1][l] = c[4];
         s_mask[l] = mask;
         BG_PROBE(27);
@@ -532,8 +532,8 @@
   __syncthreads();
   if (tid == 0) BG_TL(12);
   if (tid < n_live) {
-    d.hot[(size_t)3 * N + env0 + tid] = s_c34[0][tid];
-    d.hot[(size_t)4 * N + env0 + tid] = s_c34[1][tid];
+    *bg_hot(d, env0 + tid, 3) = s_c34[0][tid];
+    *bg_hot(d, env0 + tid, 4) = s_c34[1][tid];
     if (keys_at_end) bg_emit_keys_from_image((const lds_u4*)&s_img[tid][0], a.obs, (size_t)(env0 + tid));
   }
   if (a.stats) {
diff --git a/balatro_gym_amd/csrc/bg_engine3.h b/balatro_gym_amd/csrc/bg_engine3.h
--- a/balatro_gym_amd/csrc/bg_engine3.h
+++ b/balatro_gym_amd/csrc/bg_engine3.h
@@ -72,7 +72,7 @@
     if (l < n_live) {
       uint4 c[BG_NHOT];
 #pragma unroll
-      for (int k = 0; k < BG_NHOT; k++) c[k] = d.hot[(size_t)k * N + env];
+      for (int k = 0; k < BG_NHOT; k++) c[k] = *bg_hot(d, env, k);
       s_c34[0][l] = c[3]; s_c34[1][l] = c[4];
       DeckT dk; static_cast<Deck0&>(dk) = bg_load_deck0(d, env);
       const uint32_t prod = d.prod_view ? d.prod_view[env] : 0u;
@@ -83,7 +83,7 @@
       s_ndst[l] = e.d_ready > 0 ? 1u : 0u;
       if (e.d_ready > 0) {
 #pragma unroll
-        for (int k = 0; k < BG_NDECK; k++) s_nd[k][l] = d.ndeck[((size_t)e.d_head * BG_NDECK + k) * N + env];
+        for (int k = 0; k < BG_NDECK; k++) s_nd[k][l] = *bg_ndeck(d, env, e.d_head, k);
       }
       ShopRegs sr; sr.valid = false;
       const uint64_t mask = bg_action_mask(d, env, e, sr);
@@ -129,7 +129,7 @@
         abase[s] = 0; athr[s] = 100u;
         prow[s] = (size_t)(env0 + l);
         if (l < n_live) {
-          const uint32_t cap = (d.hot[(size_t)7 * N + (size_t)(env0 + l)].w >> 16) & 0xffu;
+          const uint32_t cap = (bg_hot(d, env0 + l, 7)->w >> 16) & 0xffu;
           if (cap > 0u && cap < 100u) athr[s] = cap;
         }
       } else {
@@ -189,7 +189,7 @@
           const uint32_t nds = bg_lds_ld(&s_ndst[l]);
           if ((nds & 0xffu) == 2u) {
 #pragma unroll
-            for (int k = 0; k < BG_NDECK; k++) ndv[s][k] = *(const __attribute__((address_space(1))) bg_u32x4*)&d.ndeck[((size_t)(nds >> 8) * BG_NDECK + k) * N + env];
+            for (int k = 0; k < BG_NDECK; k++) ndv[s][k] = *(const __attribute__((address_space(1))) bg_u32x4*)bg_ndeck(d, env, (int)(nds >> 8), k);
             bg_lds_st(&s_ndst[l], 0u);
             ndp[s] = true;
           }
@@ -418,7 +418,7 @@
           BG_PROBE_BEGIN();
           uint4 c[BG_NHOT];
 #pragma unroll
-          for (int k = 0; k < BG_NHOT; k++) if (k != 3 && k != 4) c[k] = d.hot[(size_t)k * N + env];
+          for (int k = 0; k < BG_NHOT; k++) if (k != 3 && k != 4) c[k] = *bg_hot(d, env, k);
           c[3] = s_c34[0][l]; c[4] = s_c34[1][l];
           DeckT dk; static_cast<Deck0&>(dk) = bg_load_deck0(d, env);
           RngWin w;
@@ -449,7 +449,7 @@
           BG_PROBE(26);
           bg_pack(e, c);
 #pragma unroll
-          for (int k = 0; k < BG_NHOT; k++) if (k != 3 && k != 4) d.hot[(size_t)k * N + env] = c[k];
+          for (int k = 0; k < BG_NHOT; k++) if (k != 3 && k != 4) *bg_hot(d, env, k) = c[k];
           s_c34[0][l] = c[3]; s_c34[1][l] = c[4];
           s_mask[l] = mask;
           if (o.hand_type >= 0) { n_plays++; ssum += o.final_score; }
@@ -466,8 +466,8 @@
   BG_PROBE_FLUSH(d);
   __syncthreads();
   for (int l = tid; l < n_live; l += (NOW + NSV) * BG_BLOCK) {
-    d.hot[(size_t)3 * N + env0 + l] = s_c34[0][l];
-    d.hot[(size_t)4 * N + env0 + l] = s_c34[1][l];
+    *bg_hot(d, env0 + l, 3) = s_c34[0][l];
+    *bg_hot(d, env0 + l, 4) = s_c34[1][l];
   }
   if (a.stats) bg_stats_flush(a.stats, L.s_stats, tid);
   if constexpr (kE3Tl) if (tid == 0 && d.dbg) atomicAdd(&d.dbg[31], wall_clock64() - e3_k0);
diff --git a/balatro_gym_amd/csrc/bg_lib.hip b/balatro_gym_amd/csrc/bg_lib.hip
--- a/balatro_gym_amd/csrc/bg_lib.hip
+++ b/balatro_gym_amd/csrc/bg_lib.hip
@@ -352,9 +352,9 @@
   int env = blockIdx.x * BG_BLOCK + threadIdx.x;
   if (env >= d.N) return;
   size_t N = d.N;
-  uint32_t w5 = ((const uint32_t*)&d.hot[(size_t)5 * N + env])[3];
-  uint32_t w6 = ((const uint32_t*)&d.hot[(size_t)6 * N + env])[3];
-  uint2 w7 = *((const uint2*)&d.hot[(size_t)7 * N + env]);
+  uint32_t w5 = ((const uint32_t*)bg_hot(d, env, 5))[3];
+  uint32_t w6 = ((const uint32_t*)bg_hot(d, env, 6))[3];
+  uint2 w7 = *((const uint2*)bg_hot(d, env, 7));
   uint32_t prod = d.prod_in[env];
   int d_cons = bg_b(w5, 3), g_cons = bg_b(w6, 3), s_cur = bg_b(w7.y, 0), s_cons = bg_b(w7.y, 1);
   int d_ready = (int)((prod - (uint32_t)d_cons) & 0xffu);
@@ -415,7 +415,7 @@
         if (!have && my < count) {
           env = (int)d.wl[my];
           mt = bg_deckmt(d, env);
-          const uint32_t w5 = ((const uint32_t*)&d.hot[(size_t)5 * N + env])[3];
+          const uint32_t w5 = ((const uint32_t*)bg_hot(d, env, 5))[3];
           prod = d.prod_out[env];
           d_head = bg_b(w5, 2);
           d_ready = (int)((prod - (uint32_t)bg_b(w5, 3)) & 0xffu);
@@ -447,7 +447,7 @@
 #pragma unroll
         for (int b = 0; b < 16; b++) { int i2 = k * 16 + b; if (i2 < 52) wv[b >> 2] |= (uint32_t)sdeck[i2][tid] << (8 * (b & 3)); }
         bg_cp_u32x4 nv; nv.x = wv[0]; nv.y = wv[1]; nv.z = wv[2]; nv.w = wv[3];
-        __builtin_nontemporal_store(nv, (bg_cp_u32x4*)&d.ndeck[((size_t)slot * BG_NDECK + k) * N + env]);
+        __builtin_nontemporal_store(nv, (bg_cp_u32x4*)bg_ndeck(d, env, slot, k));
       }
       d_ready++; made++;
       need = d_ready < d.KD && made < cap;
@@ -503,7 +503,7 @@
   constexpr int NR = (BG_MT_N + 63) / 64;
   for (uint32_t item = lo + blockIdx.x; item < count; item += gridDim.x) {
     const int env = (int)d.wl[2 * N + item];
-    const uint32_t w6 = ((const uint32_t*)&d.hot[(size_t)6 * N + env])[3];
+    const uint32_t w6 = ((const uint32_t*)bg_hot(d, env, 6))[3];
     const uint32_t prod = d.prod_out[env];
     const int g_cur = bg_b(w6, 2), g_cons = bg_b(w6, 3);
     int g_valid = (int)(((prod >> 16) - (uint32_t)g_cons) & 0xffu);
@@ -558,7 +558,7 @@
   if (mask_in && !mask_in[env]) return;
   Env e;
   bg_load_env(d, env, e);
-  uint4 t0 = d.tmpl[env], t1 = d.tmpl[(size_t)d.N + env];
+  uint4 t0 = *bg_tmpl(d, env, 0), t1 = *bg_tmpl(d, env, 1);
   if (t0.y & 0x80000000u) { e.njokers = (int)bg_b(t0.y, 1); e.jokers = (uint64_t)t0.x | ((uint64_t)(t0.y & 0xffu) << 32); }
   if (t0.y & 0x40000000u) e.money = (int32_t)t0.z;
   if (t0.y & 0x20000000u) e.ante = (int)bg_b(t0.y, 2);
@@ -581,13 +581,13 @@
   if (env >= d.N) return;
   if (mask_in && !mask_in[env]) return;
 #pragma unroll
-  for (int k = 0; k < BG_NDECK; k++) d.deck[(size_t)k * d.N + env] = decks[(size_t)env * BG_NDECK + k];
+  for (int k = 0; k < BG_NDECK; k++) *bg_deck(d, env, k) = decks[(size_t)env * BG_NDECK + k];
 }
 __global__ __launch_bounds__(BG_BLOCK) void bg_set_cap_kernel(BgDev d, const int32_t* __restrict__ caps, int scalar, const uint8_t* __restrict__ mask_in) {
   int env = blockIdx.x * BG_BLOCK + threadIdx.x;
   if (env >= d.N) return;
   if (mask_in && !mask_in[env]) return;
-  uint32_t* w = ((uint32_t*)&d.hot[(size_t)7 * d.N + env]) + 3;
+  uint32_t* w = ((uint32_t*)bg_hot(d, env, 7)) + 3;
   const int cap = caps ? caps[env] : scalar;
   *w = (*w & 0xffffu) | ((uint32_t)(cap & 0xff) << 16);
 }
@@ -803,11 +803,11 @@
   size_t N = (size_t)n_envs;
   BG_GUARD(h);
   hipError_t e = hipSuccess;
-  if (e == hipSuccess) e = bg_alloc(h, &d.hot, BG_NHOT * N);
-  if (e == hipSuccess) e = bg_alloc(h, &d.deck, BG_NDECK * N);
-  if (e == hipSuccess) e = bg_alloc(h, &d.cold, BG_NCOLD * N);
-  if (e == hipSuccess) e = bg_alloc(h, &d.tmpl, BG_NTMPL * N);
-  if (e == hipSuccess) e = bg_alloc(h, &d.ndeck, (size_t)d.KD * BG_NDECK * N);
+  if (e == hipSuccess) e = bg_alloc(h, &d.hot, bg_hot_chunks(N));
+  if (e == hipSuccess) e = bg_alloc(h, &d.deck, bg_deck_chunks(N));
+  if (e == hipSuccess) e = bg_alloc(h, &d.cold, bg_cold_chunks(N));
+  if (e == hipSuccess) e = bg_alloc(h, &d.tmpl, bg_tmpl_chunks(N));
+  if (e == hipSuccess) e = bg_alloc(h, &d.ndeck, bg_ndeck_chunks(N, (size_t)d.KD));
   if (e == hipSuccess) e = bg_alloc(h, &d.gblk, (size_t)d.KG * BG_MTS * N);
   if (e == hipSuccess) e = bg_alloc(h, &d.sblk, (size_t)d.KS * BG_SLOT_WORDS * N);
   if (e == hipSuccess) e = bg_alloc(h, &d.sovf, (size_t)BG_MTS * N);
@@ -846,7 +846,7 @@
   d.jtab = h->d_jtab;
   hipLaunchKernelGGL(bg_tables_build_kernel, dim3(1), dim3(256), 0, 0, h->d_jtab);
   if (hipGetLastError() != hipSuccess || hipDeviceSynchronize() != hipSuccess) { g_create_err = "bg_create: table kernel failed"; bg_destroy(h); return BG_E_HIP; }
-  h->h_tmpl.assign(BG_NTMPL * N, make_uint4(0, 0, 0, 0));
+  h->h_tmpl.assign(bg_tmpl_chunks(N), make_uint4(0, 0, 0, 0));
   h->h_cap.assign(N, (uint8_t)(max_ante > 0 && max_ante < 256 ? max_ante : 0));
   if (max_ante < 0 || max_ante > 255) { g_create_err = "bg_create: max_ante must be in [0, 255]"; bg_destroy(h); return BG_E_ARG; }
   if (max_ante > 0) {
@@ -1439,8 +1439,8 @@
   size_t N = h->dev.N;
   for (size_t i = 0; i < N; i++) {
     if (mask_host && !mask_host[i]) continue;
-    uint4& t0 = h->h_tmpl[i];
-    uint4& t1 = h->h_tmpl[N + i];
+    uint4& t0 = h->h_tmpl[bg_tmpl_at(N, i, 0)];
+    uint4& t1 = h->h_tmpl[bg_tmpl_at(N, i, 1)];
     uint32_t fl = t0.y >> 24;
     uint32_t j4 = t0.y & 0xffu, nj = (t0.y >> 8) & 0xffu, an = (t0.y >> 16) & 0xffu;
     if (jokers_host && njokers_host) {
@@ -1466,7 +1466,7 @@
     }
     t0.y = j4 | (nj << 8) | (an << 16) | (fl << 24);
   }
-  BG_HIP(hipMemcpyAsync(h->dev.tmpl, h->h_tmpl.data(), BG_NTMPL * N * sizeof(uint4), hipMemcpyHostToDevice, s));
+  BG_HIP(hipMemcpyAsync(h->dev.tmpl, h->h_tmpl.data(), h->h_tmpl.size() * sizeof(uint4), hipMemcpyHostToDevice, s));
   if (apply_now) {
     if (mask_host) BG_HIP(hipMemcpyAsync(h->d_mask, mask_host, N, hipMemcpyHostToDevice, s));
     { const int rcw = bg_wait_refill(h, s, 0); if (rcw) return rcw; }
@@ -1487,7 +1487,7 @@
   for (size_t i = 0; i < N; i++) {
     if (mask_host && !mask_host[i]) continue;
     int n = n_host[i];
-    if (n < 0) { h->h_tmpl[N + i].z = 0; continue; }
+    if (n < 0) { h->h_tmpl[bg_tmpl_at(N, i, 1)].z = 0; continue; }
     if (n > 2) { h->err = "bg_inject_consumables: an env holds at most consumable_slots = 2"; return BG_E_ARG; }
     uint32_t v = 0x80000000u | (uint32_t)n;
     for (int k = 0; k < n; k++) {
@@ -1497,9 +1497,9 @@
       if (other && !h->dev.cstate) { h->err = "bg_inject_consumables: tarot / spectral cards need BG_FLAG_CARD_STATES"; return BG_E_ARG; }
       v |= (uint32_t)id << (8 * (k + 1));
     }
-    h->h_tmpl[N + i].z = v;
-  }
-  BG_HIP(hipMemcpyAsync(h->dev.tmpl, h->h_tmpl.data(), BG_NTMPL * N * sizeof(uint4), hipMemcpyHostToDevice, s));
+    h->h_tmpl[bg_tmpl_at(N, i, 1)].z = v;
+  }
+  BG_HIP(hipMemcpyAsync(h->dev.tmpl, h->h_tmpl.data(), h->h_tmpl.size() * sizeof(uint4), hipMemcpyHostToDevice, s));
   if (apply_now) {
     if (mask_host) BG_HIP(hipMemcpyAsync(h->d_mask, mask_host, N, hipMemcpyHostToDevice, s));
     { const int rcw = bg_wait_refill(h, s, 0); if (rcw) return rcw; }
@@ -1511,16 +1511,24 @@
   return 0;
 }
 
-struct BgSlice { void* base; size_t rows; size_t elem; };
+struct BgSlice { void* base; size_t rows; size_t elem; size_t env_stride, row_stride; };
+static BgSlice bg_slice1(void* base, size_t bytes) { return {base, 1, bytes, bytes, bytes}; }
 static void bg_slices(bg_handle* h, std::vector<BgSlice>& v) {
   BgDev& d = h->dev;
-  v.push_back({d.hot, BG_NHOT, 16}); v.push_back({d.deck, BG_NDECK, 16}); v.push_back({d.cold, BG_NCOLD, 16});
-  v.push_back({d.tmpl, BG_NTMPL, 16}); v.push_back({d.ndeck, (size_t)d.KD * BG_NDECK, 16});
-  v.push_back({d.gblk, 1, (size_t)d.KG * BG_MTS * 4}); v.push_back({d.sblk, 1, (size_t)d.KS * BG_SLOT_WORDS * 4}); v.push_back({d.sovf, 1, (size_t)BG_MTS * 4});
-  v.push_back({d.deckmt, 1, (size_t)BG_MTS * 4}); v.push_back({d.shopgenmt, 1, (size_t)BG_MTS * 4});
-  v.push_back({d.sseed, 1, BG_SSEED * 4}); v.push_back({d.smeta, 1, 4});
-  v.push_back({bg_prod_latest(h), 1, 4});
-  if (d.cstate) { v.push_back({d.cstate, BG_NCST, 16}); v.push_back({d.ctmpl, BG_NCST, 16}); v.push_back({d.cardmt, 1, (size_t)BG_MTS * 4}); v.push_back({d.sealmt, 1, (size_t)BG_MTS * 4}); }
+  const size_t N = (size_t)d.N, KD = (size_t)d.KD;
+  v.push_back({d.hot, BG_NHOT, 16, 16 * (bg_hot_at(N, 1, 0) - bg_hot_at(N, 0, 0)), 16 * (bg_hot_at(N, 0, 1) - bg_hot_at(N, 0, 0))});
+  v.push_back({d.deck, BG_NDECK, 16, 16 * (bg_deck_at(N, 1, 0) - bg_deck_at(N, 0, 0)), 16 * (bg_deck_at(N, 0, 1) - bg_deck_at(N, 0, 0))});
+  v.push_back({d.cold, BG_NCOLD, 16, 16 * (bg_cold_at(N, 1, 0) - bg_cold_at(N, 0, 0)), 16 * (bg_cold_at(N, 0, 1) - bg_cold_at(N, 0, 0))});
+  v.push_back({d.tmpl, BG_NTMPL, 16, 16 * (bg_tmpl_at(N, 1, 0) - bg_tmpl_at(N, 0, 0)), 16 * (bg_tmpl_at(N, 0, 1) - bg_tmpl_at(N, 0, 0))});
+  v.push_back({d.ndeck, KD * BG_NDECK, 16, 16 * (bg_ndeck_at(N, KD, 1, 0, 0) - bg_ndeck_at(N, KD, 0, 0, 0)), 16 * (bg_ndeck_at(N, KD, 0, 0, 1) - bg_ndeck_at(N, KD, 0, 0, 0))});
+  v.push_back(bg_slice1(d.gblk, (size_t)d.KG * BG_MTS * 4)); v.push_back(bg_slice1(d.sblk, (size_t)d.KS * BG_SLOT_WORDS * 4)); v.push_back(bg_slice1(d.sovf, (size_t)BG_MTS * 4));
+  v.push_back(bg_slice1(d.deckmt, (size_t)BG_MTS * 4)); v.push_back(bg_slice1(d.shopgenmt, (size_t)BG_MTS * 4));
+  v.push_back(bg_slice1(d.sseed, BG_SSEED * 4)); v.push_back(bg_slice1(d.smeta, 4));
+  v.push_back(bg_slice1(bg_prod_latest(h), 4));
+  if (d.cstate) {
+    v.push_back({d.cstate, BG_NCST, 16, 16, 16 * N}); v.push_back({d.ctmpl, BG_NCST, 16, 16, 16 * N});
+    v.push_back(bg_slice1(d.cardmt, (size_t)BG_MTS * 4)); v.push_back(bg_slice1(d.sealmt, (size_t)BG_MTS * 4));
+  }
 }
 uint64_t bg_state_blob_bytes(const bg_handle* h) {
   if (!h) return 0;
@@ -1559,7 +1567,7 @@
   bg_slices(h, v);
   size_t N = h->dev.N;
   for (auto& s : v) {
-    BG_HIP(hipMemcpy2D(out, s.elem, (uint8_t*)s.base + (size_t)env_index * s.elem, N * s.elem, s.elem, s.rows, hipMemcpyDeviceToHost));
+    BG_HIP(hipMemcpy2D(out, s.elem, (uint8_t*)s.base + (size_t)env_index * s.env_stride, s.row_stride, s.elem, s.rows, hipMemcpyDeviceToHost));
     out += s.rows * s.elem;
   }
   return 0;
@@ -1586,9 +1594,9 @@
   bg_slices(h, v);
   size_t N = h->dev.N;
   for (auto& s : v) {
-    BG_HIP(hipMemcpy2D((uint8_t*)s.base + (size_t)env_index * s.elem, N * s.elem, in, s.elem, s.elem, s.rows, hipMemcpyHostToDevice));
+    BG_HIP(hipMemcpy2D((uint8_t*)s.base + (size_t)env_index * s.env_stride, s.row_stride, in, s.elem, s.elem, s.rows, hipMemcpyHostToDevice));
     if (s.base == (void*)h->dev.tmpl)
-      for (size_t r = 0; r < s.rows; r++) memcpy(&h->h_tmpl[r * N + (size_t)env_index], in + r * s.elem, sizeof(uint4));
+      for (size_t r = 0; r < s.rows; r++) memcpy(&h->h_tmpl[bg_tmpl_at(N, (size_t)env_index, (int)r)], in + r * s.elem, sizeof(uint4));
     if (s.base == (void*)h->dev.hot) { uint4 c7; memcpy(&c7, in + 7 * s.elem, sizeof(uint4)); h->h_cap[env_index] = (uint8_t)((c7.w >> 16) & 0xffu); }
     in += s.rows * s.elem;
   }
@@ -1643,7 +1651,7 @@
     if (mask_host && !mask_host[i]) continue;
     const int c = per_env_host ? per_env_host[i] : max_ante;
     if (c < 0 || c > 255) { h->err = "bg_set_max_ante: every cap must be in [0, 255] (0 = none)"; return BG_E_ARG; }
-    const uint32_t ty = h->h_tmpl[i].y;
+    const uint32_t ty = h->h_tmpl[bg_tmpl_at(N, i, 0)].y;
     if (c > 0 && ((ty >> 24) & 0x20u) && (int)((ty >> 16) & 0xffu) > c) { h->err = "bg_set_max_ante: a cap below the env's template ante (bg_inject)"; return BG_E_ARG; }
   }
   for (size_t i = 0; i < N; i++)
diff --git a/balatro_gym_amd/csrc/bg_step.h b/balatro_gym_amd/csrc/bg_step.h
--- a/balatro_gym_amd/csrc/bg_step.h
+++ b/balatro_gym_amd/csrc/bg_step.h
@@ -14,13 +14,11 @@
 struct ShopRegs { uint4 c3, c4, c5, c6; bool valid; };
 __device__ __forceinline__ void bg_shop_load(const BgDev& d, int env, ShopRegs& sr) {
   if (sr.valid) return;
-  size_t N = d.N;
-  sr.c3 = bg_ld16a(&d.cold[3 * N + env]); sr.c4 = bg_ld16a(&d.cold[4 * N + env]); sr.c5 = bg_ld16a(&d.cold[5 * N + env]); sr.c6 = bg_ld16a(&d.cold[6 * N + env]);
+  sr.c3 = bg_ld16a(bg_cold(d, env, 3)); sr.c4 = bg_ld16a(bg_cold(d, env, 4)); sr.c5 = bg_ld16a(bg_cold(d, env, 5)); sr.c6 = bg_ld16a(bg_cold(d, env, 6));
   sr.valid = true;
 }
 __device__ __forceinline__ void bg_shop_store(const BgDev& d, int env, const ShopRegs& sr) {
-  size_t N = d.N;
-  d.cold[3 * N + env] = sr.c3; d.cold[4 * N + env] = sr.c4; d.cold[5 * N + env] = sr.c5; d.cold[6 * N + env] = sr.c6;
+  *bg_cold(d, env, 3) = sr.c3; *bg_cold(d, env, 4) = sr.c4; *bg_cold(d, env, 5) = sr.c5; *bg_cold(d, env, 6) = sr.c6;
 }
 __device__ __forceinline__ void bg_shop_unpack(const ShopRegs& sr, int32_t cost[9], uint32_t tp[9]) {
   cost[0] = sr.c3.x; cost[1] = sr.c3.y; cost[2] = sr.c3.z; cost[3] = sr.c3.w;
@@ -67,7 +65,7 @@
 typedef __attribute__((address_space(3))) const bg_pv_u32x4 lds_cu4;
 template <class DK>
 __device__ __forceinline__ void bg_env_reset(const BgDev& d, int env, Env& e, DK& dk, const uint4* pre = nullptr, lds_cu4* pv = nullptr, int pv_stride = 0) {
-  const uint4 t0 = d.tmpl[env], t1 = d.tmpl[(size_t)d.N + env];
+  const uint4 t0 = *bg_tmpl(d, env, 0), t1 = *bg_tmpl(d, env, 1);
   e.ante = 1; e.round = 1; e.phase = 2; e.chips_needed = 300; e.chips_scored = 0; e.round_chips = 0; e.money = 4;
   e.hand = 0; e.nhand = 0; e.sel = 0; e.nsel = 0; e.hands_left = 4; e.discards_left = 3; e.hand_size = 8;
   e.njokers = 0; e.jokers = 0; e.ncons = 0; e.cons0 = 0; e.cons1 = 0; e.n_magic = 0; e.n_minim = 0;
@@ -79,15 +77,15 @@
   e.levels = 0x111111111111ull;
   e.excess = 0;
 #pragma unroll
-  for (int k = 0; k < 3; k++) d.cold[(size_t)k * d.N + env] = make_uint4(0, 0, 0, 0);
+  for (int k = 0; k < 3; k++) *bg_cold(d, env, k) = make_uint4(0, 0, 0, 0);
   if (e.d_ready <= 0) atomicOr(d.err, BG_DEVERR_DECKRING);
   else {
 #pragma unroll
     for (int k = 0; k < BG_NDECK; k++) {
       uint4 c;
       if (pv) { const bg_pv_u32x4 v = pv[k * pv_stride]; c = make_uint4(v.x, v.y, v.z, v.w); }
-      else c = pre ? pre[k] : d.ndeck[((size_t)e.d_head * BG_NDECK + k) * d.N + env];
-      d.deck[(size_t)k * d.N + env] = c;
+      else c = pre ? pre[k] : *bg_ndeck(d, env, e.d_head, k);
+      *bg_deck(d, env, k) = c;
       bg_deck_set(dk, k, c);
     }
     e.d_head = (e.d_head + 1 == d.KD) ? 0 : e.d_head + 1;
@@ -749,7 +747,7 @@
   e.chips_scored += final_score;
   e.hp_total++; e.hp_ante++;
   if (final_score > e.best_hand) e.best_hand = final_score;
-  atomicAdd(((uint32_t*)&d.cold[(size_t)(ht >> 2) * d.N + env]) + (ht & 3), 1u);
+  atomicAdd(((uint32_t*)bg_cold(d, env, ht >> 2)) + (ht & 3), 1u);
   if (e.boss_type) {
     e.boss_types |= 1u << ht;
     e.bflags &= ~BG_BF_FIRST_HAND;
@@ -1144,7 +1142,7 @@
 #pragma unroll
         for (int k = 0; k < BG_NDECK; k++) {
           const uint4 c4 = make_uint4(w.lds[(4 * k) * BG_BLOCK], w.lds[(4 * k + 1) * BG_BLOCK], w.lds[(4 * k + 2) * BG_BLOCK], w.lds[(4 * k + 3) * BG_BLOCK]);
-          d.deck[(size_t)k * d.N + env] = c4;
+          *bg_deck(d, env, k) = c4;
           bg_deck_set(mdk, k, c4);
         }
         e.boss_cards = played;
```

Measured after the change: 8.278 billion (median of 6 runs). 1.7% higher.
